# MisEty/RTG-SLAM

Hardware: AMD Instinct MI355X
Metric: hot_path_units_per_sec (higher is better)
Workload: dtype f32; 1 GPU; `value` counts UNITS, not SLAM frames (the SLAM frame rate by the reference's definition is `slam_frames_per_sec`, from the `slam_sequence` leg of --full).  One UNIT per step = 1 ICP track (3 levels x 5 GN iters, 1200x680, on a second HIP stream) + 1 map-optimisation iteration (raster fwd + masked L1 colour / gated depth loss + attach regulariser + raster bwd + fused Adam) over 1200000 random Gaus; gaussians=1200000, mode=single, parallelism=1 GPU

## Files before the change

include/rtgs_debug.h:

```cpp
#ifndef RTGS_DEBUG_H
#define RTGS_DEBUG_H
#include "rtgs_raster.h"
#ifdef __cplusplus
extern "C" {
#endif

void rtgs_raster_set_counters(void* counters);
void rtgs_raster_set_counters_ctx(rtgs_ctx* ctx, void* counters);

void rtgs_raster_set_profiling(int enable);
void rtgs_raster_set_profiling_ctx(rtgs_ctx* ctx, int enable);

void rtgs_raster_set_near_slice(int mode, int budget_per_tile);
void rtgs_raster_set_near_slice_ctx(rtgs_ctx* ctx, int mode, int budget_per_tile);

void rtgs_raster_force_sort_path(int enable);
void rtgs_raster_force_sort_path_ctx(rtgs_ctx* ctx, int enable);
int rtgs_raster_last_timings(float* ms12_host);
int rtgs_raster_last_timings_ctx(rtgs_ctx* ctx, float* ms12_host);

void rtgs_raster_set_bwd_walk_ctx(rtgs_ctx* ctx, int mode);
void rtgs_raster_set_onepass_ctx(rtgs_ctx* ctx, int on);
void rtgs_raster_set_fused_sort_ctx(rtgs_ctx* ctx, int on);
int rtgs_raster_fused_sort_stats_ctx(rtgs_ctx* ctx, int64_t* out18);
void rtgs_raster_set_tile_gather_ctx(rtgs_ctx* ctx, int mode);
int rtgs_raster_tile_gather_stats_ctx(rtgs_ctx* ctx, int64_t* out6);
void rtgs_raster_set_bwd_debug(int bits);
void rtgs_raster_set_bwd_stamps(void* dev);
void rtgs_raster_set_fwd_stamps(void* dev);
#define RTGS_ICP_STAMP_LAUNCHES 16
#define RTGS_ICP_STAMP_WGS 256
void rtgs_icp_set_stamps(void* dev);
void rtgs_tsdf_set_dense(int on);

#ifdef __cplusplus
}
#endif
#endif
```

rtg_slam_amd/csrc/map_ops.hip:

```cpp
#include "../../include/rtgs_raster.h"
#include <hip/hip_runtime.h>
#include <math.h>
#include <stdint.h>
#include "adam_common.h"
#include "activate_common.h"


namespace rtgs {

__global__ void __launch_bounds__(256) activate8_fwd_kernel(const float4* __restrict__ raw8, int64_t n,
                                                            float* __restrict__ opacity, float* __restrict__ scales,
                                                            float4* __restrict__ rots, float* __restrict__ normal) {
  for (int64_t i = (int64_t)blockIdx.x * blockDim.x + threadIdx.x; i < n; i += (int64_t)gridDim.x * blockDim.x)
    activate8_row_store(raw8[2 * i], raw8[2 * i + 1], i, opacity, scales, rots, normal);
}

__global__ void __launch_bounds__(256) activate8_bwd_kernel(const float4* __restrict__ raw8, int64_t n,
                                                            const float* __restrict__ g_op, const float* __restrict__ g_sc,
                                                            const float4* __restrict__ g_rot, const float* __restrict__ g_nrm,
                                                            const uint8_t* __restrict__ row_state,
                                                            float4* __restrict__ g_raw8) {
  for (int64_t i = (int64_t)blockIdx.x * blockDim.x + threadIdx.x; i < n; i += (int64_t)gridDim.x * blockDim.x) {
    if (row_state) {
      const uint8_t s = row_state[i];
      if (s == 0) continue;
      if (s == 2) { g_raw8[2 * i] = g_raw8[2 * i + 1] = make_float4(0.f, 0.f, 0.f, 0.f); continue; }
    }
    float4 lo, hi;
    activate8_bwd_row(raw8[2 * i], raw8[2 * i + 1], g_op[i], g_sc[i * 3], g_sc[i * 3 + 1], g_sc[i * 3 + 2], g_rot[i],
                      g_nrm[i * 3], g_nrm[i * 3 + 1], g_nrm[i * 3 + 2], lo, hi);
    g_raw8[2 * i] = lo;
    g_raw8[2 * i + 1] = hi;
  }
}

}

extern "C" int rtgs_map_activate8_forward(const float* raw8, int64_t n, float* opacity, float* scales, float* rotations,
                                          float* normal, void* stream) {
  if (n < 0 || (n > 0 && (!raw8 || !opacity || !scales || !rotations || !normal))) return -1;
  if (n == 0) return 0;
  int64_t blocks = (n + 255) / 256;
  if (blocks > 8192) blocks = 8192;
  hipLaunchKernelGGL(rtgs::activate8_fwd_kernel, dim3((unsigned)blocks), dim3(256), 0, (hipStream_t)stream,
                     (const float4*)raw8, n, opacity, scales, (float4*)rotations, normal);
  return hipGetLastError() == hipSuccess ? 0 : -2;
}

extern "C" int rtgs_map_activate8_backward(const float* raw8, int64_t n, const float* g_opacity, const float* g_scales,
                                           const float* g_rotations, const float* g_normal, float* g_raw8, void* stream) {
  if (n < 0 || (n > 0 && (!raw8 || !g_opacity || !g_scales || !g_rotations || !g_normal || !g_raw8))) return -1;
  if (n == 0) return 0;
  int64_t blocks = (n + 255) / 256;
  if (blocks > 8192) blocks = 8192;
  hipLaunchKernelGGL(rtgs::activate8_bwd_kernel, dim3((unsigned)blocks), dim3(256), 0, (hipStream_t)stream,
                     (const float4*)raw8, n, g_opacity, g_scales, (const float4*)g_rotations, g_normal,
                     (const uint8_t*)nullptr, (float4*)g_raw8);
  return hipGetLastError() == hipSuccess ? 0 : -2;
// ... 461 lines not shown
    const float4 t = *reinterpret_cast<const float4*>(p + i); v[0] = t.x; v[1] = t.y; v[2] = t.z; v[3] = t.w;
  }
  __device__ __forceinline__ void store(float* p, int64_t i) const { *reinterpret_cast<float4*>(p + i) = make_float4(v[0], v[1], v[2], v[3]); }
};
template <int V>
__device__ __forceinline__ void load_flags(const uint8_t* __restrict__ rmask, const int32_t* __restrict__ didx, int64_t i, bool (&m)[V],
                                           bool (&hit)[V]) {
  if constexpr (V == 4) {
    const uint32_t mm = rmask ? *reinterpret_cast<const uint32_t*>(rmask + i) : 0x01010101u;
    const int4 d = *reinterpret_cast<const int4*>(didx + i);
    m[0] = (mm & 0xffu) != 0; m[1] = (mm & 0xff00u) != 0; m[2] = (mm & 0xff0000u) != 0; m[3] = (mm & 0xff000000u) != 0;
    hit[0] = d.x != -1; hit[1] = d.y != -1; hit[2] = d.z != -1; hit[3] = d.w != -1;
  } else {
    m[0] = !rmask || rmask[i] != 0;
    hit[0] = didx[i] != -1;
  }
}

template <int V>
__global__ void __launch_bounds__(256) slam_loss_sums_kernel(const float* __restrict__ color, const float* __restrict__ depth,
                                                             const int32_t* __restrict__ didx, const float* __restrict__ gt_c,
                                                             const float* __restrict__ gt_d, const uint8_t* __restrict__ rmask,
                                                             int64_t hw, float depth_thr, float* __restrict__ sums) {
  float s_c = 0.f, s_d = 0.f, s_m = 0.f, s_n = 0.f;
  for (int64_t i = ((int64_t)blockIdx.x * blockDim.x + threadIdx.x) * V; i < hw; i += (int64_t)gridDim.x * blockDim.x * V) {
    bool m[V], hit[V];
    load_flags<V>(rmask, didx, i, m, hit);
    PixVec<V> c0, c1, c2, t0, t1, t2, dp, gd;
    c0.load(color, i); c1.load(color + hw, i); c2.load(color + 2 * hw, i);
    t0.load(gt_c, i); t1.load(gt_c + hw, i); t2.load(gt_c + 2 * hw, i);
    dp.load(depth, i); gd.load(gt_d, i);
#pragma unroll
    for (int k = 0; k < V; ++k) {
      if (!m[k]) continue;
      s_n += 1.f;
      s_c += fabsf(c0.v[k] - t0.v[k]) + fabsf(c1.v[k] - t1.v[k]) + fabsf(c2.v[k] - t2.v[k]);
      const float g = gd.v[k], e = dp.v[k] - g;
      if (hit[k] && g > 0.f && e < depth_thr) { s_d += fabsf(e); s_m += 1.f; }
    }
  }
  s_c = wave_sum_shfl(s_c); s_d = wave_sum_shfl(s_d); s_m = wave_sum_shfl(s_m); s_n = wave_sum_shfl(s_n);
  __shared__ float sh[4][4];
  const int lane = threadIdx.x & 63, w = threadIdx.x >> 6;
  if (lane == 0) { sh[0][w] = s_c; sh[1][w] = s_d; sh[2][w] = s_m; sh[3][w] = s_n; }
  __syncthreads();
  if (threadIdx.x < 4) {
    const float t = sh[threadIdx.x][0] + sh[threadIdx.x][1] + sh[threadIdx.x][2] + sh[threadIdx.x][3];
    unsafeAtomicAdd(&sums[threadIdx.x], t);
  }
}

__device__ __forceinline__ uint32_t sign_code(float d) { return d > 0.f ? 1u : (d < 0.f ? 2u : 0u); }

template <int V>
__global__ void __launch_bounds__(256) slam_loss_sums_signs_kernel(const float* __restrict__ color, const float* __restrict__ depth,
                                                                   const int32_t* __restrict__ didx, const float* __restrict__ gt_c,
                                                                   const float* __restrict__ gt_d, const uint8_t* __restrict__ rmask,
                                                                   int64_t hw, float depth_thr,
                                                                   float* __restrict__ sums, uint8_t* __restrict__ signs) {
  float s_c = 0.f, s_d = 0.f, s_m = 0.f, s_n = 0.f;
  for (int64_t i = ((int64_t)blockIdx.x * blockDim.x + threadIdx.x) * V; i < hw; i += (int64_t)gridDim.x * blockDim.x * V) {
    bool m[V], hit[V];
    load_flags<V>(rmask, didx, i, m, hit);
    PixVec<V> c0, c1, c2, t0, t1, t2, dp, gd;
    c0.load(color, i); c1.load(color + hw, i); c2.load(color + 2 * hw, i);
    t0.load(gt_c, i); t1.load(gt_c + hw, i); t2.load(gt_c + 2 * hw, i);
    dp.load(depth, i); gd.load(gt_d, i);
    uint32_t packed = 0u;
#pragma unroll
    for (int k = 0; k < V; ++k) {
      if (!m[k]) continue;
      const float d0 = c0.v[k] - t0.v[k], d1 = c1.v[k] - t1.v[k], d2 = c2.v[k] - t2.v[k];
      s_n += 1.f;
      s_c += fabsf(d0) + fabsf(d1) + fabsf(d2);
      uint32_t code = sign_code(d0) | (sign_code(d1) << 2) | (sign_code(d2) << 4);
      const float g = gd.v[k], e = dp.v[k] - g;
      if (hit[k] && g > 0.f && e < depth_thr) { s_d += fabsf(e); s_m += 1.f; code |= sign_code(e) << 6; }
      packed |= code << (8 * k);
    }
    if constexpr (V == 4) *reinterpret_cast<uint32_t*>(signs + i) = packed;
    else signs[i] = (uint8_t)packed;
  }
  s_c = wave_sum_shfl(s_c); s_d = wave_sum_shfl(s_d); s_m = wave_sum_shfl(s_m); s_n = wave_sum_shfl(s_n);
  __shared__ float sh[4][4];
  const int lane = threadIdx.x & 63, w = threadIdx.x >> 6;
  if (lane == 0) { sh[0][w] = s_c; sh[1][w] = s_d; sh[2][w] = s_m; sh[3][w] = s_n; }
  __syncthreads();
  if (threadIdx.x < 4) {
    const float t = sh[threadIdx.x][0] + sh[threadIdx.x][1] + sh[threadIdx.x][2] + sh[threadIdx.x][3];
    unsafeAtomicAdd(&sums[threadIdx.x], t);
  }
}

__global__ void slam_loss_values_kernel(const float* __restrict__ sums, float cw, float dw, float* __restrict__ loss4) {
  const float inv_c = 1.f / (3.f * fmaxf(sums[3], 1.f));
  const float inv_m = 1.f / fmaxf(sums[2], 1.f);
  const float lc = sums[0] * inv_c, ld = sums[1] * inv_m;
  loss4[1] = lc; loss4[2] = ld; loss4[3] = 0.f;
  loss4[0] = dw * ld + cw * lc;
}

struct SsimWin { float g[11]; };
constexpr int SS_R = 5, SS_T = 16 + 2 * SS_R;

__global__ void __launch_bounds__(256) ssim_fwd_kernel(const float* __restrict__ x1, const float* __restrict__ x2, int H, int W,
                                                       SsimWin win, float* __restrict__ dmaps, float* __restrict__ sums) {
  __shared__ float s_a[SS_T * SS_T], s_b[SS_T * SS_T];
  __shared__ float s_h[5][SS_T * 16];
  const int lx = threadIdx.x & 15, ly = threadIdx.x >> 4;
  const int px = blockIdx.x * 16 + lx, py = blockIdx.y * 16 + ly;
  const size_t HW = (size_t)H * W;
  float ssum = 0.f;
  for (int c = 0; c < 3; ++c) {
    __syncthreads();
// ... 133 lines not shown
}

}

extern "C" size_t rtgs_slam_loss_signs_offset(int32_t H, int32_t W, int32_t with_ssim) {
  const size_t front = 8 * sizeof(float) + (with_ssim ? (size_t)9 * (size_t)H * (size_t)W * sizeof(float) : 0);
  return (front + 15) & ~(size_t)15;
}
extern "C" size_t rtgs_slam_loss_scratch_bytes(int32_t H, int32_t W, int32_t with_ssim) {
  return rtgs_slam_loss_signs_offset(H, W, with_ssim) + (((size_t)H * (size_t)W + 15) & ~(size_t)15);
}

static void ssim_window(rtgs::SsimWin& win) {
  float gf[11], totf = 0.f;
  for (int i = 0; i < 11; ++i) { gf[i] = (float)exp(-(double)((i - 5) * (i - 5)) / (2.0 * 1.5 * 1.5)); totf += gf[i]; }
  for (int i = 0; i < 11; ++i) win.g[i] = gf[i] / totf;
}

extern "C" int rtgs_slam_loss_sums(const float* color, const float* depth, const int32_t* depth_index, const float* gt_color,
                                   const float* gt_depth, int32_t H, int32_t W, const rtgs_loss_cfg* cfg, void* scratch,
                                   void* stream) {
  if (!color || !depth || !depth_index || !gt_color || !gt_depth || !cfg || !scratch || H <= 0 || W <= 0) return -1;
  hipStream_t st = (hipStream_t)stream;
  const int64_t hw = (int64_t)H * W;
  float* sums = (float*)scratch;
  const bool ssim = cfg->render_mask == nullptr && cfg->ssim_weight != 0.f;
  if (!cfg->sums_zeroed && hipMemsetAsync(sums, 0, 8 * sizeof(float), st) != hipSuccess) return -2;
  int64_t blocks = (hw + 255) / 256;
  if (blocks > 192) blocks = 192;
  if (rtgs::loss_vec4_ok(hw, color, depth, depth_index, gt_color, gt_depth, cfg->render_mask, nullptr, nullptr))
    hipLaunchKernelGGL(rtgs::slam_loss_sums_kernel<4>, dim3((unsigned)blocks), dim3(256), 0, st, color, depth, depth_index,
                       gt_color, gt_depth, cfg->render_mask, hw, cfg->add_depth_thres, sums);
  else
    hipLaunchKernelGGL(rtgs::slam_loss_sums_kernel<1>, dim3((unsigned)blocks), dim3(256), 0, st, color, depth, depth_index,
                       gt_color, gt_depth, cfg->render_mask, hw, cfg->add_depth_thres, sums);
  if (ssim) {
    rtgs::SsimWin win;
    ssim_window(win);
    hipLaunchKernelGGL(rtgs::ssim_fwd_kernel, dim3((W + 15) / 16, (H + 15) / 16), dim3(256), 0, st, color, gt_color, H, W, win,
                       sums + 8, sums);
  }
  return hipGetLastError() == hipSuccess ? 0 : -2;
}

extern "C" int rtgs_slam_loss_values(const rtgs_loss_cfg* cfg, const void* scratch, float* loss_out4, void* stream) {
  if (!cfg || !scratch || !loss_out4 || (cfg->render_mask == nullptr && cfg->ssim_weight != 0.f)) return -1;
  hipLaunchKernelGGL(rtgs::slam_loss_values_kernel, dim3(1), dim3(1), 0, (hipStream_t)stream, (const float*)scratch,
                     cfg->color_weight, cfg->depth_weight, loss_out4);
  return hipGetLastError() == hipSuccess ? 0 : -2;
}
extern "C" int rtgs_slam_loss_sums_signs(const float* color, const float* depth, const int32_t* depth_index,
                                         const float* gt_color, const float* gt_depth, int32_t H, int32_t W,
                                         const rtgs_loss_cfg* cfg, void* scratch, float* loss_out4, void* stream) {
  if (!color || !depth || !depth_index || !gt_color || !gt_depth || !cfg || !scratch || H <= 0 || W <= 0) return -1;
  if (cfg->render_mask == nullptr && cfg->ssim_weight != 0.f) return -1;
  hipStream_t st = (hipStream_t)stream;
  const int64_t hw = (int64_t)H * W;
  float* sums = (float*)scratch;
  uint8_t* signs = (uint8_t*)scratch + rtgs_slam_loss_signs_offset(H, W, cfg->render_mask == nullptr);
  if (!cfg->sums_zeroed && hipMemsetAsync(sums, 0, 8 * sizeof(float), st) != hipSuccess) return -2;
  int64_t blocks = (hw + 255) / 256;
  if (blocks > 192) blocks = 192;
  if (rtgs::loss_vec4_ok(hw, color, depth, depth_index, gt_color, gt_depth, cfg->render_mask, nullptr, nullptr) &&
      ((uintptr_t)signs & 3u) == 0)
    hipLaunchKernelGGL(rtgs::slam_loss_sums_signs_kernel<4>, dim3((unsigned)blocks), dim3(256), 0, st, color, depth, depth_index,
                       gt_color, gt_depth, cfg->render_mask, hw, cfg->add_depth_thres, sums, signs);
  else
    hipLaunchKernelGGL(rtgs::slam_loss_sums_signs_kernel<1>, dim3((unsigned)blocks), dim3(256), 0, st, color, depth, depth_index,
                       gt_color, gt_depth, cfg->render_mask, hw, cfg->add_depth_thres, sums, signs);
  if (loss_out4) return rtgs_slam_loss_values(cfg, scratch, loss_out4, stream);
  return hipGetLastError() == hipSuccess ? 0 : -2;
}

extern "C" int rtgs_slam_loss_grads(const float* color, const float* depth, const int32_t* depth_index, const float* gt_color,
                                    const float* gt_depth, int32_t H, int32_t W, const rtgs_loss_cfg* cfg, void* scratch,
                                    float* loss_out4, float* g_color, float* g_depth, void* stream) {
  if (!color || !depth || !depth_index || !gt_color || !gt_depth || !cfg || !scratch || !loss_out4 || !g_color || !g_depth ||
      H <= 0 || W <= 0)
    return -1;
  hipStream_t st = (hipStream_t)stream;
  const int64_t hw = (int64_t)H * W;
  float* sums = (float*)scratch;
  const bool ssim = cfg->render_mask == nullptr && cfg->ssim_weight != 0.f;
  int64_t blocks = (hw + 255) / 256;
  if (blocks > 1024) blocks = 1024;
  if (rtgs::loss_vec4_ok(hw, color, depth, depth_index, gt_color, gt_depth, cfg->render_mask, g_color, g_depth)) {
    blocks = (hw / 4 + 255) / 256;
    if (blocks > 1024) blocks = 1024;
    hipLaunchKernelGGL(rtgs::slam_loss_grads_kernel<4>, dim3((unsigned)blocks), dim3(256), 0, st, color, depth, depth_index,
                       gt_color, gt_depth, cfg->render_mask, hw, cfg->color_weight, cfg->depth_weight,
                       ssim ? cfg->ssim_weight : 0.f, cfg->add_depth_thres, (const float*)sums, loss_out4, g_color, g_depth);
  } else {
    hipLaunchKernelGGL(rtgs::slam_loss_grads_kernel<1>, dim3((unsigned)blocks), dim3(256), 0, st, color, depth, depth_index,
                       gt_color, gt_depth, cfg->render_mask, hw, cfg->color_weight, cfg->depth_weight,
                       ssim ? cfg->ssim_weight : 0.f, cfg->add_depth_thres, (const float*)sums, loss_out4, g_color, g_depth);
  }
  if (ssim) {
    rtgs::SsimWin win;
    ssim_window(win);
    hipLaunchKernelGGL(rtgs::ssim_bwd_kernel, dim3((W + 15) / 16, (H + 15) / 16), dim3(256), 0, st, color, gt_color, H, W, win,
                       (const float*)(sums + 8), -cfg->ssim_weight / (3.f * (float)hw), g_color);
  }
  return hipGetLastError() == hipSuccess ? 0 : -2;
}

extern "C" int rtgs_slam_loss(const float* color, const float* depth, const int32_t* depth_index, const float* gt_color,
                              const float* gt_depth, int32_t H, int32_t W, const rtgs_loss_cfg* cfg, void* scratch,
                              float* loss_out4, float* g_color, float* g_depth, void* stream) {
  int rc = rtgs_slam_loss_sums(color, depth, depth_index, gt_color, gt_depth, H, W, cfg, scratch, stream);
  if (rc != 0) return rc;
  return rtgs_slam_loss_grads(color, depth, depth_index, gt_color, gt_depth, H, W, cfg, scratch, loss_out4, g_color, g_depth,
                              stream);
}


namespace rtgs {

__device__ __forceinline__ bool normal_pixel(const float* __restrict__ normal_w, const int32_t* __restrict__ didx,
                                             const float* __restrict__ gtn, const uint8_t* __restrict__ mask, int64_t i,
                                             int& owner, float (&n)[3], float (&g)[3]) {
  owner = didx[i];
  if (owner < 0 || (mask && mask[i] == 0)) return false;
// ... 104 lines not shown
```

rtg_slam_amd/csrc/map_step.hip:

```cpp
#include <hip/hip_runtime.h>

#include "../../include/rtgs_raster.h"

static int map_step_front(rtgs_ctx* ctx, const rtgs_map_step_args* a, int64_t* num_rendered_host, int32_t fwd_flags,
                          void* stream, bool walk_only = false) {
  if (!a || !num_rendered_host || !a->settings) return RTGS_E_INVALID;
  const int32_t P = a->P, M = a->sh_coeffs;
  if (P <= 0 || M != 16 || a->step < 1) return RTGS_E_INVALID;
  if (!a->xyz || !a->shs || !a->raw8 || !a->tile_mask || !a->gt_color || !a->gt_depth) return RTGS_E_INVALID;
  const int32_t H = a->settings->image_height, W = a->settings->image_width;
  int rc = 0;
  if (!a->activated_valid) {
    rc = rtgs_map_activate8_forward(a->raw8, P, a->opacity, a->scales, a->rotations, a->normal, stream);
    if (rc != 0) return RTGS_E_HIP;
  }
  if (!a->loss_scratch || !a->loss4) return RTGS_E_INVALID;
  rtgs_raster_set_aux_zero_ctx(ctx, a->loss_scratch);
  rc = rtgs_raster_forward_ctx(ctx, a->settings, P, M, a->xyz, a->opacity, a->shs, a->scales, a->rotations, a->normal,
                           a->tile_mask, a->out_color, a->out_depth, a->out_color_index, a->out_depth_index,
                           a->out_color_weight, a->out_depth_weight, a->out_T, a->out_radii, a->geom_resize,
                           a->geom_user, a->binning_resize, a->binning_user, a->image_resize, a->image_user,
                           num_rendered_host, fwd_flags, stream);
  if (rc != RTGS_OK) return rc;
  void* bufs[3];
  if (rtgs_raster_last_buffers_ctx(ctx, bufs) != RTGS_OK) return RTGS_E_ALLOC;
  void *geom = bufs[0], *bin = bufs[1], *img = bufs[2];
  rtgs_loss_cfg lcfg = a->loss;
  lcfg.sums_zeroed = P > 0 ? 1 : 0;
  const bool ssim_off = a->loss.render_mask != nullptr || a->loss.ssim_weight == 0.f;
  const bool signs = walk_only && ssim_off && rtgs_raster_signs_ok_ctx(ctx, geom) != 0;
  rtgs_raster_note_loss_path_ctx(ctx, signs ? 1 : 0);
  if (signs)
    rc = rtgs_slam_loss_sums_signs(a->out_color, a->out_depth, a->out_depth_index, a->gt_color, a->gt_depth, H, W, &lcfg,
                                   a->loss_scratch, nullptr, stream);
  else
    rc = rtgs_slam_loss(a->out_color, a->out_depth, a->out_depth_index, a->gt_color, a->gt_depth, H, W, &lcfg,
                        a->loss_scratch, a->loss4, a->dL_dcolor, a->dL_ddepth, stream);
  if (rc != 0) return RTGS_E_HIP;
  int32_t t0 = 0, t1 = P;
  if (a->train_begin != 0 || a->train_end != 0) { t0 = a->train_begin; t1 = a->train_end; }
  if (t0 < 0 || t1 > P || t1 < t0) return RTGS_E_INVALID;
  if (t1 == t0)
    return signs && rtgs_slam_loss_values(&lcfg, a->loss_scratch, a->loss4, stream) != 0 ? RTGS_E_HIP : RTGS_OK;
  if (signs) {
    const rtgs_loss_signs ls{reinterpret_cast<const uint8_t*>(a->loss_scratch) + rtgs_slam_loss_signs_offset(H, W, a->loss.render_mask == nullptr),
                             reinterpret_cast<const float*>(a->loss_scratch), a->loss.color_weight, a->loss.depth_weight, a->loss4};
    return rtgs_raster_backward_walk_signs_ctx(ctx, a->settings, P, M, *num_rendered_host, a->xyz, a->opacity, a->shs, a->scales,
                                               a->rotations, a->normal, geom, bin, img, a->out_color, a->out_T, a->out_depth_index,
                                               &ls, a->grad_scratch, a->row_state, t0, t1, stream);
  }
  rc = (walk_only ? rtgs_raster_backward_walk_ctx : rtgs_raster_backward_range_ctx)(
      ctx, a->settings, P, M, *num_rendered_host, a->xyz, a->opacity, a->shs, a->scales, a->rotations, a->normal, geom, bin, img,
      a->out_color, a->out_T, a->out_depth_index, a->dL_dcolor, a->dL_ddepth, a->d_xyz, a->d_opacity, a->d_shs, a->d_scales,
      a->d_rotations, a->d_normal, a->grad_scratch, a->row_state, t0, t1, stream);
  if (rc != RTGS_OK) return rc;
  if (a->normal_weight > 0.f && a->gt_normal) {
    rc = rtgs_slam_normal_loss_range(a->normal, a->out_depth_index, a->gt_normal, a->loss.render_mask, H, W, a->normal_weight,
                                     reinterpret_cast<float*>(a->loss_scratch) + 5, a->loss4, a->d_normal, a->row_state,
                                     rtgs_raster_spec_fail_ptr_ctx(ctx), t0, t1, stream);
    if (rc != 0) return RTGS_E_HIP;
  }
  return RTGS_OK;
}

extern "C" int rtgs_slam_map_step_front_ctx(rtgs_ctx* ctx, const rtgs_map_step_args* a, int64_t* num_rendered_host,
                                            void* stream) {
  return map_step_front(ctx, a, num_rendered_host, 0, stream);
}

extern "C" int rtgs_slam_map_step_front(const rtgs_map_step_args* a, int64_t* num_rendered_host, void* stream) {
  return rtgs_slam_map_step_front_ctx(nullptr, a, num_rendered_host, stream);
}

static int map_step_once(rtgs_ctx* ctx, const rtgs_map_step_args* a, int64_t* num_rendered_host, bool speculate, void* stream) {
  const bool fused = a->tail_mode == 0 && !(a->normal_weight > 0.f && a->gt_normal);
  rtgs_raster_set_map_epoch_ctx(ctx, speculate ? a->map_epoch : 0u);
  int rc = map_step_front(ctx, a, num_rendered_host, speculate ? RTGS_FWD_SPECULATE : 0, stream, fused);
  if (rc != RTGS_OK) return rc;
  if ((a->train_begin != 0 || a->train_end != 0) && a->train_end == a->train_begin) return RTGS_OK;
  if (fused) {
    void* bufs[3];
    if (rtgs_raster_last_buffers_ctx(ctx, bufs) != RTGS_OK) return RTGS_E_ALLOC;
    return rtgs_map_fused_tail_marked(a->settings, a, bufs[0], bufs[2], rtgs_raster_spec_fail_ptr_ctx(ctx), a->live_counts,
                                      rtgs_raster_last_listed_ctx(ctx), rtgs_raster_cull_marks_ctx(ctx), stream);
  }
  const int32_t P = a->P;
  int32_t t0 = 0, t1 = P;
  if (a->train_begin != 0 || a->train_end != 0) { t0 = a->train_begin; t1 = a->train_end; }
  const size_t o = (size_t)t0;
  const rtgs_activated act{a->opacity + o, a->scales + 3 * o, a->rotations + 4 * o, a->normal + 3 * o};
  uint8_t* const marks = rtgs_raster_cull_marks_ctx(ctx);
  rc = rtgs_map_tail_rows_marked(a->xyz + 3 * o, a->shs + 48 * o, a->raw8 + 8 * o, a->d_opacity + o, a->d_scales + 3 * o,
                          a->d_rotations + 4 * o, a->d_normal + 3 * o, a->d_xyz + 3 * o, a->d_shs + 48 * o, a->d_raw8 + 8 * o,
// ... 39 lines not shown
```

rtg_slam_amd/csrc/raster_api.hip:

```cpp
#include "../../include/rtgs_raster.h"
#include "../../include/rtgs_debug.h"
#include "raster_common.h"
#include "raster_launch.h"
#include <vector>

#include <rocprim/device/device_radix_sort.hpp>
#include <rocprim/device/device_scan.hpp>
#include <math.h>
#include <new>
#include <stdlib.h>
#include <string.h>

enum { EV_F0 = 0, EV_PRE, EV_SL_BIN, EV_SL_BLEND, EV_SCAN, EV_BIN0, EV_EMIT, EV_SORT, EV_RANGES, EV_BLEND0, EV_BLEND, EV_B0,
       EV_BWALK, EV_BBLEND, EV_BPRE, EV_N };
struct rtgs_ctx {
  int64_t stats[8] = {0};
  struct Switches {
    int slice_mode = 2;
    int slice_budget = 384;
    int bwd_walk = 0;
    bool onepass = true;
    bool fused_sort = true;
    bool speculation = true;
    bool plain_onepass = true;
    bool cull_cache = true, cull_check = false;
    bool loss_signs = true;
    int tile_gather = 1;
  } sw;
  int64_t gather_stats[4] = {0, 0, 0, 0};
  bool gather_blocked = false;
  int64_t loss_path_stats[2] = {0, 0};
  int64_t slice_stats[4] = {0};
  unsigned long long* counters = nullptr;
  uint32_t last_listed = 0;
  uint32_t* fsort_cls = nullptr;
  int32_t fsort_cap = 0, fsort_tiles = 0;
  bool prof = false;
  bool force_sort_path = false;
  bool ev_init = false;
  hipEvent_t ev[EV_N];
  bool ev_set[EV_N] = {false};
  uint32_t* info_host = nullptr;
  uint32_t seq = 0;
  const void* hint_geom = nullptr;
  bool hint_slice_lists = true, hint_main_lists = true;
  int hint_walk = -2;
  void *last_geom = nullptr, *last_bin = nullptr, *last_img = nullptr;
  uint32_t* aux_zero = nullptr;
  bool ask_first = false;
  struct Plan {
    bool valid = false;
    int32_t P = 0, H = 0, W = 0;
    int kind = -1;
    int slice_mode = 0, slice_budget = 0;
    uint32_t R = 0, R1 = 0, longest = 0, slots = 0, n_fin = 0;
    uint32_t R_hi = 0, longest_hi = 0, slots_hi = 0;
    uint32_t slice_longest_hi = 0;
    void note_slice(uint32_t l) { slice_longest_hi = l > slice_longest_hi - slice_longest_hi / 16 ? l : slice_longest_hi - slice_longest_hi / 16; }
    void note(uint32_t r, uint32_t l, uint32_t s) {
      R = r; longest = l; slots = s;
      R_hi = r > R_hi - R_hi / 16 ? r : R_hi - R_hi / 16;
      longest_hi = l > longest_hi - longest_hi / 16 ? l : longest_hi - longest_hi / 16;
      slots_hi = s > slots_hi - slots_hi / 16 ? s : slots_hi - slots_hi / 16;
    }
  } plan;
  struct Spec {
    bool pending = false;
    int kind = -1;
    bool gathered = false;
    uint32_t seq = 0, capR = 0, capL = 0, capS = 0;
    const void* geom = nullptr;
    const uint32_t* fail_dev = nullptr;
    void* stream = nullptr;
    int32_t ntiles = 0;
    int64_t G_total = 0, B_total = 0, I_total = 0;
  } spec;
  int64_t spec_stats[3] = {0, 0, 0};
  Plan plan_plain;
  Plan plan_plain0;
  int64_t plain_stats[2] = {0, 0};
  struct CullKey {
    const void *geom, *view, *means, *scales, *rots, *out_radii, *stream;
    uint64_t geom_bytes, epoch;
    int32_t P, H, W, kind, slice_mode, slice_budget;
    float fx, fy, cx, cy, tanfovx, tanfovy, scale_modifier, color_sigma;
  };
  struct CullCache {
    bool armed = false;
    CullKey key = {};
    uint8_t* marks = nullptr;
    uint64_t next_epoch = 0;
    int64_t stats[4] = {0, 0, 0, 0};
    char* scratch = nullptr;
    size_t scratch_bytes = 0;
    unsigned long long* mismatches = nullptr;
  } cull;
};

namespace rtgs {

static rtgs_ctx* default_ctx() {
  static rtgs_ctx* c = [] {
    rtgs_ctx* n = new rtgs_ctx();
    if (const char* e = getenv("RTGS_NEAR_SLICE")) n->sw.slice_mode = atoi(e);
    if (const char* e = getenv("RTGS_NEAR_SLICE_BUDGET")) { const int b = atoi(e); if (b > 0) n->sw.slice_budget = b; }
    if (const char* e = getenv("RTGS_SPECULATE")) n->sw.speculation = atoi(e) != 0;
    if (const char* e = getenv("RTGS_BIN_ONEPASS")) n->sw.onepass = atoi(e) != 0;
    if (const char* e = getenv("RTGS_FWD_SORT")) n->sw.fused_sort = atoi(e) != 0;
    if (const char* e = getenv("RTGS_PLAIN_ONEPASS")) n->sw.plain_onepass = atoi(e) != 0;
    if (const char* e = getenv("RTGS_BWD_WALK")) { const int m = atoi(e); n->sw.bwd_walk = (m >= 1 && m <= 4) ? m : 0; }
    if (const char* e = getenv("RTGS_CULL_CACHE")) n->sw.cull_cache = atoi(e) != 0;
    if (const char* e = getenv("RTGS_CULL_CACHE_CHECK")) n->sw.cull_check = atoi(e) != 0;
    if (const char* e = getenv("RTGS_LOSS_SIGNS")) n->sw.loss_signs = atoi(e) != 0;
    if (const char* e = getenv("RTGS_TILE_GATHER")) { const int m = atoi(e); n->sw.tile_gather = (m >= 0 && m <= 2) ? m : 1; }
    return n;
  }();
  return c;
}
static inline rtgs_ctx* use(rtgs_ctx* c) { return c ? c : default_ctx(); }

static void prof_mark(rtgs_ctx* c, int which, hipStream_t st) {
  if (!c->prof) return;
  if (!c->ev_init) {
    for (int i = 0; i < EV_N; ++i) (void)hipEventCreate(&c->ev[i]);
    c->ev_init = true;
  }
  (void)hipEventRecord(c->ev[which], st);
  c->ev_set[which] = true;
}

static int bits_for(uint32_t n) {
  int b = 0;
  while ((1ull << b) < (unsigned long long)n) ++b;
  return b < 1 ? 1 : b;
}

static int wait_published_words(uint32_t* info_host, uint32_t seq, hipStream_t st, uint32_t (&pub)[7]) {
  volatile uint32_t* h = info_host;
  auto snapshot_ok = [&]() -> bool {
    if (h[7] != seq) return false;
    __atomic_thread_fence(__ATOMIC_ACQUIRE);
    uint32_t w[7];
    for (int k = 0; k < 7; ++k) w[k] = h[k];
    if (h[8] != host_checksum(seq, w)) return false;
    for (int k = 0; k < 7; ++k) pub[k] = w[k];
    return true;
  };
  for (long spin = 0; spin < 4000000L; ++spin) {
    if (snapshot_ok()) return RTGS_OK;
    __builtin_ia32_pause();
  }
  if (hipStreamSynchronize(st) != hipSuccess) return RTGS_E_HIP;
  return snapshot_ok() ? RTGS_OK : RTGS_E_HIP;
}

static uint32_t sort_class_cap(uint32_t longest) {
  const uint64_t want = (uint64_t)longest + longest / 4 + 16;
  const uint32_t classes[5] = {256u, 1024u, 3072u, 8192u, 16384u};
  for (uint32_t c : classes) if (want <= c) return c;
  return 16384u;
}

__global__ void bwd_info_kernel(BwdInfo* dst, SplatGrad* slot_grads, uint32_t slots, uint32_t use_slots) {
  dst->slot_grads = slot_grads; dst->slots = slots; dst->use_slots = use_slots;
}

static int large_map_min() {
  static const int v = [] { const char* e = getenv("RTGS_LARGE_MAP_MIN"); const int x = e ? atoi(e) : 100000; return x > 0 ? x : 100000; }();
  return v;
}

static GeomLayout geom_layout(int32_t P, int gx, int gy, int budget) {
  GeomLayout L{};
  size_t off = 0;
  const size_t Pn = (size_t)(P > 0 ? P : 1);
  L.splats = off; off = align_up(off + Pn * sizeof(Splat));
  L.tiles_touched = off; off = align_up(off + Pn * sizeof(uint32_t));
  L.offsets = off; off = align_up(off + Pn * sizeof(uint32_t));
  L.radii = off; off = align_up(off + Pn * sizeof(int32_t));
  L.clamped = off; off = align_up(off + Pn);
  L.sat = off; off = align_up(off + (size_t)(gx + 1) * (gy + 1) * sizeof(int32_t));
  {
    const size_t nt = (size_t)gx * gy;
    L.zero_begin = L.tile_count = off;
    off += nt * sizeof(uint32_t);
    L.tile_count1 = off; off += nt * sizeof(uint32_t);
    L.ranges1_bwd = off; off += nt * sizeof(uint2);
    L.slice_ctr = off; off += 8 * sizeof(uint32_t);
    L.slot_count = off; off += Pn * sizeof(uint32_t);
    L.zero_end = off; off = align_up(off);
    L.cursor = off; off = align_up(off + nt * sizeof(uint32_t));
    L.info = off; off = align_up(off + 4 * sizeof(uint32_t));
    L.block_counts = off; off = align_up(off + bin_block_counts_bytes((int)Pn, gx * gy));
    L.zbin = off; off = align_up(off + Pn);
    L.cursor1 = off; off = align_up(off + nt * sizeof(uint32_t));
    L.ranges1 = off; off = align_up(off + nt * sizeof(uint2));
    L.mask2 = off; off = align_up(off + nt * sizeof(int32_t));
    L.uv = off; off = align_up(off + Pn * sizeof(float2));
    L.slice_hist = off; off += 2 * SLICE_BINS * sizeof(uint32_t);
    L.slice_cover = off; off = align_up(off + SLICE_BINS * sizeof(unsigned long long));
    L.cull_marks = off; off = align_up(off + Pn + 16);
    L.cull_view = off; off = align_up(off + 16 * sizeof(float));
    L.slice_cap = nt * (size_t)(budget > 0 ? budget : 1);
    L.slice_max_list = L.slice_cap < 65536 ? L.slice_cap : 65536;
// ... 71 lines not shown
  p.cy = s->cy > 0.f ? s->cy : 0.5f * (float)(p.H - 1);
  p.scale_modifier = s->scale_modifier;
  p.opaque_thr = s->opaque_threshold; p.depth_thr = s->depth_threshold; p.normal_thr = s->normal_threshold;
  p.color_sigma = s->color_sigma; p.T_thr = s->T_threshold;
  p.view = s->viewmatrix; p.campos = s->campos; p.bg = s->bg;
  p.spec_fail = nullptr;
  return RTGS_OK;
}

#define HIP_TRY(expr)                         \
  do {                                        \
    hipError_t e_ = (expr);                   \
    if (e_ != hipSuccess) return RTGS_E_HIP;  \
  } while (0)

static int dbg_sync(const rtgs_raster_settings* s, hipStream_t st) {
  if (s->debug) {
    HIP_TRY(hipStreamSynchronize(st));
    HIP_TRY(hipGetLastError());
  }
  return RTGS_OK;
}
#define DBG(s, st)                              \
  do {                                          \
    int r_ = dbg_sync(s, st);                   \
    if (r_ != RTGS_OK) return r_;               \
  } while (0)

struct FwdCall {
  rtgs_ctx* c;
  const rtgs_raster_settings* s;
  RasterParams p;
  hipStream_t st;
  int32_t flags;
  bool want_bwd, slice_auto;
  const float *means3D, *opacities, *shs, *scales, *rotations, *normal_w;
  const int32_t* tile_mask;
  float *out_color, *out_depth, *out_cw, *out_dw, *out_T;
  int32_t *out_cidx, *out_didx, *out_radii;
  rtgs_resize_fn geom_resize, binning_resize, image_resize;
  void *geom_user, *binning_user, *image_user;
  int64_t* num_rendered_host;
  GeomLayout G;
  ImgLayout I;
  char *geom, *img;
  uint32_t *tiles_touched, *offsets, *tile_count, *cursor, *info, *zero_words, *tile_count1, *slice_hist, *slice_ctr, *list1;
  Splat* splats; int32_t *radii, *sat, *mask2; uint8_t *clamped, *zbin; uint16_t* block_counts;
  uint2 *ranges, *ranges1, *ranges1_bwd; unsigned long long* slice_cover; float2* uv;
  uint32_t *n_contrib, *depth_pos, *tile_last, *tile_mode;
  int zero_n, ntiles;
  int fwd_walk;
  TileCache tcache;
  uint32_t seg1;
  uint32_t* aux_zero;
  uint64_t cull_epoch;
  bool cull_was_armed;
  uint32_t* info_host;
  uint32_t pub[7];
};

static inline void next_seq(rtgs_ctx* c) { if (++c->seq == 0u) c->seq = 1u; }
static inline int wait_published(FwdCall& f) { return wait_published_words(f.info_host, f.c->seq, f.st, f.pub); }

static void record_stats(rtgs_ctx* c, int64_t rendered, int ntiles, int64_t geom_bytes, int64_t bin_bytes, int64_t img_bytes,
                         bool tile_path, int64_t longest) {
  c->stats[0] = rendered; c->stats[1] = 32 + bits_for((uint32_t)ntiles); c->stats[2] = ntiles;
  c->stats[3] = geom_bytes; c->stats[4] = bin_bytes; c->stats[5] = img_bytes;
  c->stats[6] = tile_path ? 1 : 0; c->stats[7] = longest;
}

static void note_plan(rtgs_ctx::Plan& pl, const FwdCall& f, bool same, int kind, bool usable, int64_t R, uint32_t longest,
                      uint32_t slots) {
  same = same && pl.valid && pl.H == f.p.H && pl.W == f.p.W;
  pl.kind = kind;
  pl.valid = kind >= 0 && usable && R <= 0xffffffffll;
  pl.P = f.p.P; pl.H = f.p.H; pl.W = f.p.W; pl.slice_mode = f.c->sw.slice_mode; pl.slice_budget = f.c->sw.slice_budget;
  if (!same || !pl.valid) { pl.R_hi = pl.longest_hi = pl.slots_hi = 0; pl.slice_longest_hi = 0; }
  pl.note((uint32_t)R, longest, slots);
}

static SliceSel slice_sel(const FwdCall& f) {
  return SliceSel{1, f.zbin, f.slice_hist, (uint32_t)f.G.slice_cap, (uint32_t)f.G.slice_max_list, f.slice_ctr, nullptr, nullptr,
                  f.slice_cover, (uint32_t)f.ntiles * (uint32_t)(TILE * TILE), f.slice_auto ? 1 : 0};
}

static void preprocess_all(const FwdCall& f, const int32_t* sat, bool clear) {
  launch_preprocess_fwd(f.p, f.means3D, f.opacities, f.shs, f.scales, f.rotations, f.normal_w, sat, f.splats, f.tiles_touched,
                        f.radii, f.clamped, f.out_radii, clear ? f.zero_words : nullptr, clear ? f.zero_n : 0, nullptr, f.st);
}
static void shade(const FwdCall& f, const RasterParams& p, SliceList work, const SliceSel& sel, size_t max_list,
                  RowBands rb = RowBands{nullptr, nullptr, 0u}) {
  launch_preprocess_shade(p, f.means3D, f.opacities, f.shs, f.scales, f.rotations, f.normal_w, f.splats, f.radii, f.clamped,
                          f.uv, work, sel, max_list, f.st, rb);
}
static void blend(const FwdCall& f, const RasterParams& p, const uint2* ranges, const uint32_t* list, SlicePass pass,
                  uint32_t seg, FusedSort fs = FusedSort{nullptr, nullptr, nullptr, nullptr, nullptr},
                  TileGather tg = TileGather{nullptr, nullptr, 0u, nullptr, nullptr, nullptr}) {
  launch_blend_fwd(p, ranges, list, f.splats, f.out_color, f.out_depth, f.out_cidx, f.out_didx, f.out_cw, f.out_dw, f.out_T,
                   f.n_contrib, f.c->counters, pass, f.tile_mode, f.depth_pos, f.tile_last, f.fwd_walk, f.aux_zero, f.tcache,
                   seg, f.st, fs, tg);
}

static bool tile_gather_chosen(FwdCall& f, const rtgs_ctx::Plan& pl) {
  rtgs_ctx* const c = f.c; const GeomLayout& G = f.G;
  if (c->sw.tile_gather == 0 || !f.seg1 || !(c->sw.fused_sort && blend_fwd_fuses_sort() && blend_fwd_gathers())) return false;
  const size_t cap1 = (size_t)f.ntiles * G.slice_seg > G.slice_cap ? (size_t)f.ntiles * G.slice_seg : G.slice_cap;
  if (f.p.gx > 255 || f.p.gy > GATHER_ROWS_MAX || G.slice_max_list > 65536 ||
      (size_t)f.p.gy * G.slice_max_list * sizeof(uint32_t) > cap1 * sizeof(uint64_t)) { ++c->gather_stats[3]; return false; }
  const bool forced = c->sw.tile_gather == 2;
  if (c->gather_blocked && pl.slice_longest_hi <= (uint32_t)FSORT_CAP) c->gather_blocked = false;
  if (c->gather_blocked) { ++c->gather_stats[2]; return false; }
  if (!forced && c->last_listed > (uint32_t)G.slice_max_list) { ++c->gather_stats[1]; return false; }
  if (!forced && pl.slice_longest_hi > (uint32_t)(FSORT_CAP - FSORT_CAP / 8)) { ++c->gather_stats[2]; return false; }
  ++c->gather_stats[0];
  return true;
}

static int scan_slots(const FwdCall& f) {
  size_t tb = f.G.scan_temp_bytes;
  HIP_TRY(rocprim::exclusive_scan(f.geom + f.G.scan_temp, tb, f.tiles_touched, f.offsets, 0u, (size_t)f.p.P,
                                  rocprim::plus<uint32_t>(), f.st));
  return RTGS_OK;
}

static int fsort_class_words(FwdCall& f, uint32_t*& cls) {
  rtgs_ctx* const c = f.c;
  cls = nullptr;
  if (c->counters) {
    if (c->fsort_cap < f.ntiles) {
      if (c->fsort_cls) (void)hipFree(c->fsort_cls);
      c->fsort_cls = nullptr; c->fsort_cap = 0;
      HIP_TRY(hipMalloc((void**)&c->fsort_cls, (size_t)f.ntiles * sizeof(uint32_t)));
      c->fsort_cap = f.ntiles;
    }
    HIP_TRY(hipMemsetAsync(c->fsort_cls, 0xff, (size_t)f.ntiles * sizeof(uint32_t), f.st));
    c->fsort_tiles = f.ntiles;
    cls = c->fsort_cls;
  }
  return RTGS_OK;
}
static int sort_slice_lists(FwdCall& f, FusedSort& fs1) {
  rtgs_ctx* const c = f.c;
  const unsigned long long* bucket1 = (const unsigned long long*)(f.geom + f.G.bucket1);
  const uint32_t* cnt = f.seg1 ? f.tile_count1 : nullptr;
  if (!(c->sw.fused_sort && blend_fwd_fuses_sort())) {
    launch_bin_tilesort(f.ntiles, (uint32_t)SLICE_MAX_LIST, f.ranges1, bucket1, f.list1, nullptr, f.st, cnt, f.seg1,
                        f.seg1 ? f.ranges1 : nullptr);
    return RTGS_OK;
  }
  launch_bin_tilesort_long(f.ntiles, f.ranges1, bucket1, f.list1, nullptr, f.st, cnt, f.seg1);
  uint32_t* cls = nullptr;
  const int rc = fsort_class_words(f, cls);
  if (rc != RTGS_OK) return rc;
  fs1 = FusedSort{bucket1, cnt, f.seg1 ? f.ranges1 : nullptr, f.list1, cls};
  return RTGS_OK;
}

static int slice_pass1(FwdCall& f, uint32_t* guard, bool gather = false) {
  const RasterParams& p = f.p; const GeomLayout& G = f.G;
  const SliceSel sel1 = slice_sel(f);
  const SliceList work{(const uint32_t*)(f.geom + G.slice_ids), f.slice_ctr + 2};
  unsigned long long* const bucket1 = (unsigned long long*)(f.geom + G.bucket1);
  if (gather) {
    const RowBands rb{f.tile_count, (uint32_t*)bucket1, (uint32_t)G.slice_max_list};
    shade(f, p, work, sel1, G.slice_max_list, rb);
    uint32_t* cls = nullptr;
    const int rcc = fsort_class_words(f, cls);
    if (rcc != RTGS_OK) return rcc;
    DBG(f.s, f.st);
    prof_mark(f.c, EV_SL_BIN, f.st);
    blend(f, p, f.ranges1, f.list1, SlicePass{1, f.tile_mask, f.mask2, f.ranges1_bwd, f.ranges}, f.seg1,
          FusedSort{bucket1, f.tile_count1, f.ranges1, f.list1, cls},
          TileGather{rb.count, rb.entries, rb.stride, work.ids, f.radii, f.tile_count1});
    prof_mark(f.c, EV_SL_BLEND, f.st);
    launch_slice_publish(f.ntiles, f.tile_mask, f.mask2, f.info + 2, f.slice_ctr, f.info_host, f.c->seq, guard, f.st, f.tile_count1);
    DBG(f.s, f.st);
    return RTGS_OK;
  }
  shade(f, p, work, sel1, G.slice_max_list);
  if (f.seg1) {
    launch_bin_place(p, f.splats, f.radii, f.tile_mask, f.tile_count1, bucket1, f.seg1, nullptr, sel1, work, G.slice_max_list, f.st);
  } else {
    uint16_t* const block_counts1 = (uint16_t*)(f.geom + G.block_counts1);
    uint32_t* const cursor1 = (uint32_t*)(f.geom + G.cursor1);
    if (launch_bin_count(p, f.splats, f.radii, f.tile_mask, f.tile_count1, block_counts1, sel1, work, G.slice_max_list, f.st) != 0)
      return RTGS_E_HIP;
    launch_bin_tilescan(f.ntiles, f.tile_count1, f.ranges1, cursor1, f.info + 2, nullptr, nullptr, nullptr, nullptr, nullptr, 0u,
                        SpecCaps{nullptr, 0u, 0u, 0u, nullptr}, f.st);
    launch_bin_scatter(p, f.splats, f.radii, f.tile_mask, block_counts1, cursor1, bucket1, sel1, work, G.slice_max_list, f.st);
  }
  FusedSort fs1{nullptr, nullptr, nullptr, nullptr, nullptr};
  const int rc = sort_slice_lists(f, fs1);
  if (rc != RTGS_OK) return rc;
  DBG(f.s, f.st);
  prof_mark(f.c, EV_SL_BIN, f.st);
  blend(f, p, f.ranges1, f.list1, SlicePass{1, f.tile_mask, f.mask2, f.ranges1_bwd, f.ranges}, f.seg1, fs1);
  prof_mark(f.c, EV_SL_BLEND, f.st);
  launch_slice_publish(f.ntiles, f.tile_mask, f.mask2, f.info + 2, f.slice_ctr, f.info_host, f.c->seq, guard, f.st,
                       f.seg1 ? f.tile_count1 : nullptr);
  DBG(f.s, f.st);
  return RTGS_OK;
}

static int cull_self_check(FwdCall& f, uint32_t* fail) {
  rtgs_ctx::CullCache& cc = f.c->cull;
  const int32_t P = f.p.P; const size_t Pn = (size_t)P;
  const size_t o_tt = 0, o_rad = align_up(o_tt + Pn * 4), o_orad = align_up(o_rad + Pn * 4), o_zb = align_up(o_orad + Pn * 4),
               o_uv = align_up(o_zb + Pn), o_hist = align_up(o_uv + Pn * 8), need = align_up(o_hist + CULL_HIST_WORDS * 4);
  if (cc.scratch_bytes < need) {
    if (cc.scratch) (void)hipFree(cc.scratch);
    cc.scratch = nullptr; cc.scratch_bytes = 0;
    HIP_TRY(hipMalloc((void**)&cc.scratch, need));
    cc.scratch_bytes = need;
  }
  if (!cc.mismatches) {
    HIP_TRY(hipMalloc((void**)&cc.mismatches, sizeof(unsigned long long)));
    HIP_TRY(hipMemset(cc.mismatches, 0, sizeof(unsigned long long)));
  }
  char* sc = cc.scratch;
  HIP_TRY(hipMemcpyAsync(sc + o_uv, f.uv, Pn * 8, hipMemcpyDeviceToDevice, f.st));
  launch_preprocess_cull(f.p, f.means3D, f.scales, f.rotations, (uint32_t*)(sc + o_tt), (int32_t*)(sc + o_rad),
                         f.out_radii ? (int32_t*)(sc + o_orad) : nullptr, nullptr, 0, (uint8_t*)(sc + o_zb),
                         (float2*)(sc + o_uv), (uint32_t*)(sc + o_hist), f.st);
  launch_slice_hist(P, (const uint8_t*)(sc + o_zb), (const uint32_t*)(sc + o_tt), (const int32_t*)(sc + o_rad),
                    (uint32_t*)(sc + o_hist), (unsigned long long*)(sc + o_hist + 2 * SLICE_BINS * 4), f.st);
  launch_cull_check(P, f.tiles_touched, (const uint32_t*)(sc + o_tt), f.radii, (const int32_t*)(sc + o_rad), f.out_radii,
                    (const int32_t*)(sc + o_orad), f.zbin, (const uint8_t*)(sc + o_zb), f.uv, (const float2*)(sc + o_uv),
                    f.slice_hist, (const uint32_t*)(sc + o_hist), fail + 1, cc.mismatches, f.st);
  return RTGS_OK;
}

static int cull_stage(FwdCall& f, int kind, bool usable, uint32_t* fail, const BwdInfoInit& bi) {
  rtgs_ctx* const c = f.c; const RasterParams& p = f.p;
  rtgs_ctx::CullCache& cc = c->cull;
  rtgs_ctx::CullKey key;
  memset(&key, 0, sizeof(key));
  key.geom = f.geom; key.view = f.s->viewmatrix; key.means = f.means3D; key.scales = f.scales; key.rots = f.rotations;
  key.out_radii = f.out_radii; key.stream = (void*)f.st; key.geom_bytes = (uint64_t)f.G.total; key.epoch = f.cull_epoch;
  key.P = p.P; key.H = p.H; key.W = p.W; key.kind = kind; key.slice_mode = c->sw.slice_mode; key.slice_budget = c->sw.slice_budget;
  key.fx = p.fx; key.fy = p.fy; key.cx = p.cx; key.cy = p.cy; key.tanfovx = p.tanfovx; key.tanfovy = p.tanfovy;
  key.scale_modifier = p.scale_modifier; key.color_sigma = p.color_sigma;
  usable = usable && c->sw.cull_cache && f.cull_epoch != 0;
  uint8_t* const marks = (uint8_t*)(f.geom + f.G.cull_marks);
  float* const view_copy = (float*)(f.geom + f.G.cull_view);
  if (usable && f.cull_was_armed && memcmp(&key, &cc.key, sizeof(key)) == 0) {
    launch_recull_rows(p, f.means3D, f.scales, f.rotations, f.tiles_touched, f.radii, f.out_radii, f.zero_words, f.zero_n, f.zbin,
                       f.uv, f.slice_hist, f.slice_cover, marks, view_copy, (int)(fail - f.zero_words), bi, f.st);
    cc.armed = true;
    ++cc.stats[0]; --cc.stats[2];
    return c->sw.cull_check ? cull_self_check(f, fail) : RTGS_OK;
  }
  launch_preprocess_cull(p, f.means3D, f.scales, f.rotations, f.tiles_touched, f.radii, f.out_radii, f.zero_words, f.zero_n,
// ... 37 lines not shown
  f.tcache = f.want_bwd ? TileCache{(float4*)(img + I.tile_recs), (uint16_t*)(img + I.tile_masks), (float2*)(img + I.depth_aux)}
                        : TileCache{nullptr, nullptr, nullptr};
  f.fwd_walk = c->sw.bwd_walk == 0 || c->sw.bwd_walk == 3 ? 2 : (c->sw.bwd_walk == 4 ? -1 : c->sw.bwd_walk - 1);
  f.seg1 = c->sw.onepass ? (uint32_t)G.slice_seg : 0u;
  f.slice_auto = c->sw.slice_mode == 2;
  if (!c->info_host) {
    HIP_TRY(hipHostMalloc((void**)&c->info_host, HOST_WORDS * sizeof(uint32_t), hipHostMallocCoherent));
    memset(c->info_host, 0, HOST_WORDS * sizeof(uint32_t));
  }
  f.info_host = c->info_host;
  for (uint32_t& w : f.pub) w = 0;
  return RTGS_OK;
}

enum SpecOutcome { SPEC_RETURNED, SPEC_NOT_ELIGIBLE, SPEC_REDO };

static int forward_speculative(FwdCall& f, bool sort_path, bool sliced, SpecOutcome& outcome) {
  rtgs_ctx* const c = f.c;
  const RasterParams& p = f.p; const GeomLayout& G = f.G; const ImgLayout& I = f.I;
  const int32_t P = p.P; const int ntiles = f.ntiles; hipStream_t st = f.st;
  int rc;
  outcome = SPEC_RETURNED;
  rtgs_ctx::Plan& pp = sliced ? c->plan_plain : c->plan_plain0;
  const bool immediate = !(f.flags & RTGS_FWD_SPECULATE) && !f.want_bwd && c->sw.speculation && c->sw.plain_onepass && c->sw.onepass &&
                         P > 0 && !sort_path && !f.s->debug && pp.valid && (sliced ? (pp.kind == 2 && G.slice_seg) : pp.kind == 0) &&
                         pp.H == p.H && pp.W == p.W && pp.slice_mode == c->sw.slice_mode && pp.slice_budget == c->sw.slice_budget;
  const rtgs_ctx::Plan& pl = immediate ? pp : c->plan;
  const bool eligible = immediate ||
                        ((f.flags & RTGS_FWD_SPECULATE) && c->sw.speculation && f.want_bwd && P > 0 && !sort_path && !f.s->debug &&
                         pl.valid && pl.P == P && pl.H == p.H && pl.W == p.W && pl.slice_mode == c->sw.slice_mode &&
                         pl.slice_budget == c->sw.slice_budget && (pl.kind == 0 ? !sliced : (pl.kind == 1 || pl.kind == 2) && sliced));
  const uint32_t capR = pl.R_hi + pl.R_hi / 8u + 8192u, capL = sort_class_cap(pl.longest_hi),
                 capS = immediate ? 0u : pl.slots_hi + pl.slots_hi / 8u + 8192u;
  if (!(eligible && (pl.kind == 1 || capS <= SLOTS_MAX))) {
    if (f.flags & RTGS_FWD_SPECULATE) ++c->spec_stats[2];
    outcome = SPEC_NOT_ELIGIBLE;
    return RTGS_OK;
  }
  uint32_t* const fail = f.slice_ctr + 6;
  next_seq(c);
  const uint32_t sl = (uint32_t)G.slice_cap <= SLOTS_MAX ? (uint32_t)G.slice_cap : 0u;
  const uint32_t seg2 = (pl.kind != 1 && c->sw.onepass && ((pl.kind == 2 && G.slice_seg) || (immediate && pl.kind == 0))) ? capL : 0u;
  const bool seg_main = seg2 != 0u;
  const BinLayout B = pl.kind == 1 ? bin_layout(0, ntiles, false, (size_t)sl)
                                   : bin_layout(seg2 ? (int64_t)ntiles * (int64_t)seg2 : (int64_t)capR, ntiles, false, (size_t)capS);
  char* bin = (char*)f.binning_resize(f.binning_user, B.total);
  if (!bin) return RTGS_E_ALLOC;
  c->last_bin = bin;
  BwdInfo* const bwd_info = (BwdInfo*)(f.img + I.bwd_info);
  SplatGrad* const slot_grads = (SplatGrad*)(bin + B.slot_grads);
  if (pl.kind == 1) {
    if ((rc = cull_stage(f, pl.kind, !immediate, fail, BwdInfoInit{bwd_info, slot_grads, sl, sl ? 1u : 0u})) != RTGS_OK) return rc;
    prof_mark(c, EV_PRE, st);
    launch_slice_compact(P, slice_sel(f), (uint32_t*)(f.geom + G.slice_ids), f.slice_ctr + 2, f.tiles_touched, f.offsets,
                         f.slice_ctr + 4, nullptr, 0u, nullptr, st);
    c->spec.gathered = tile_gather_chosen(f, pl);
    if ((rc = slice_pass1(f, fail, c->spec.gathered)) != RTGS_OK) return rc;
    prof_mark(c, EV_BLEND0, st); prof_mark(c, EV_BLEND, st);
    c->hint_slice_lists = true; c->hint_main_lists = false;
    c->slice_stats[0] = 1; c->slice_stats[1] = pl.R1; c->slice_stats[2] = pl.n_fin; c->slice_stats[3] = 0;
  } else {
    unsigned long long* const keys_a = (unsigned long long*)(bin + B.keys_a);
    uint32_t* const vals_b = (uint32_t*)(bin + B.vals_b);
    RasterParams pg = p;
    pg.spec_fail = fail;
    SliceList vl{nullptr, nullptr};
    if (pl.kind == 2) {
      if ((rc = cull_stage(f, pl.kind, !immediate, fail, BwdInfoInit{bwd_info, slot_grads, capS, immediate ? 0u : 1u})) != RTGS_OK)
        return rc;
      prof_mark(c, EV_PRE, st);
      const SliceSel sel1 = slice_sel(f);
      vl = SliceList{(const uint32_t*)(f.geom + G.vis_ids), f.slice_ctr + 4};
      launch_visible_compact(P, f.zbin, (uint32_t*)(f.geom + G.vis_ids), f.slice_ctr + 4, f.tiles_touched, f.offsets, f.slice_ctr + 5,
                             fail, st, &sel1, (int32_t*)(f.slice_ctr + 3), fail);
      shade(f, pg, vl, sel1, (size_t)P);
    } else {
      preprocess_all(f, nullptr, true);
      if (!immediate && (rc = scan_slots(f)) != RTGS_OK) return rc;
      prof_mark(c, EV_PRE, st);
    }
    const SliceSel sel2{0, nullptr, nullptr, 0u, 0u, f.slice_ctr, nullptr, f.uv, nullptr, 0u, 0};
    const int32_t* const still_declined = pl.kind == 2 ? (const int32_t*)(f.slice_ctr + 3) : nullptr;
    if (seg2) {
      if (pl.kind != 2)
        hipLaunchKernelGGL(bwd_info_kernel, dim3(1), dim3(1), 0, st, bwd_info, slot_grads, capS, immediate ? 0u : 1u);
      launch_bin_place(pg, f.splats, f.radii, f.tile_mask, f.tile_count, keys_a, seg2, fail, sel2, vl, (size_t)P, st);
      prof_mark(c, EV_SCAN, st); prof_mark(c, EV_BIN0, st); prof_mark(c, EV_EMIT, st);
      const BinFinish fin{f.tile_count, ntiles, f.info, f.info_host, f.slice_ctr + 5, nullptr, f.slice_ctr + 4, c->seq,
                          SpecCaps{fail, 0xffffffffu, capL, immediate ? 0xffffffffu : capS, still_declined}};
      launch_bin_tilesort(ntiles, capL, f.ranges, keys_a, vals_b, fail, st, f.tile_count, seg2, f.ranges, &fin);
    } else {
      uint16_t* const counts = vl.ids ? (uint16_t*)(f.geom + G.block_counts_vis) : f.block_counts;
      if (launch_bin_count(pg, f.splats, f.radii, f.tile_mask, f.tile_count, counts, sel2, vl, (size_t)P, st) != 0)
        return RTGS_E_HIP;
      const SpecCaps caps{fail, capR, capL, immediate ? 0xffffffffu : capS, still_declined};
      launch_bin_tilescan(ntiles, f.tile_count, f.ranges, f.cursor, f.info, f.info_host, nullptr, nullptr,
                          vl.ids ? f.slice_ctr + 5 : f.offsets + (P - 1), vl.ids ? nullptr : f.tiles_touched + (P - 1), c->seq,
                          caps, st);
      prof_mark(c, EV_SCAN, st);
      if (pl.kind != 2) hipLaunchKernelGGL(bwd_info_kernel, dim3(1), dim3(1), 0, st, bwd_info, slot_grads, capS, 1u);
      prof_mark(c, EV_BIN0, st);
      launch_bin_scatter(pg, f.splats, f.radii, f.tile_mask, counts, f.cursor, keys_a, sel2, vl, (size_t)P, st);
      prof_mark(c, EV_EMIT, st);
      launch_bin_tilesort(ntiles, capL, f.ranges, keys_a, vals_b, fail, st);
    }
    prof_mark(c, EV_SORT, st);
    prof_mark(c, EV_BLEND0, st);
    blend(f, pg, f.ranges, vals_b, SlicePass{0, nullptr, nullptr, nullptr, nullptr}, seg2);
    prof_mark(c, EV_BLEND, st);
    c->hint_slice_lists = false; c->hint_main_lists = true;
// ... 200 lines not shown

const char* rtgs_version(void) { return "rtgs-hip 0.2.0 (gfx950)"; }

rtgs_ctx* rtgs_ctx_create(void) {
  rtgs_ctx* c = new (std::nothrow) rtgs_ctx();
  if (c) c->sw = default_ctx()->sw;
  return c;
}
void rtgs_ctx_destroy(rtgs_ctx* c) {
  if (!c || c == default_ctx()) return;
  if (c->ev_init) for (int i = 0; i < EV_N; ++i) (void)hipEventDestroy(c->ev[i]);
  if (c->info_host) (void)hipHostFree(c->info_host);
  if (c->cull.scratch) (void)hipFree(c->cull.scratch);
  if (c->cull.mismatches) (void)hipFree(c->cull.mismatches);
  if (c->fsort_cls) (void)hipFree(c->fsort_cls);
  delete c;
}

size_t rtgs_raster_geom_bytes_ctx(rtgs_ctx* c, int32_t P, int32_t H, int32_t W) {
  return geom_layout(P, (W + TILE - 1) / TILE, (H + TILE - 1) / TILE, use(c)->sw.slice_budget).total;
}
size_t rtgs_raster_geom_bytes(int32_t P, int32_t H, int32_t W) { return rtgs_raster_geom_bytes_ctx(nullptr, P, H, W); }
size_t rtgs_raster_binning_bytes(int64_t R, int32_t H, int32_t W) {
  const int gx = (W + TILE - 1) / TILE, gy = (H + TILE - 1) / TILE;
  return bin_layout(R, gx * gy, true, 0).total;
}
size_t rtgs_raster_image_bytes(int32_t H, int32_t W) {
  const int gx = (W + TILE - 1) / TILE, gy = (H + TILE - 1) / TILE;
  return img_layout(H, W, gx * gy).total;
}
size_t rtgs_raster_backward_scratch_bytes(int32_t P) {
  const size_t n = (size_t)(P > 0 ? P : 1);
  return align_up(n * sizeof(SplatGrad)) + align_up(n);
}

int rtgs_raster_last_stats_ctx(rtgs_ctx* c, int64_t* out) {
  if (!out) return RTGS_E_INVALID;
  memcpy(out, use(c)->stats, sizeof(use(c)->stats));
  return RTGS_OK;
}
void rtgs_raster_set_counters_ctx(rtgs_ctx* c, void* counters) { use(c)->counters = (unsigned long long*)counters; }

int rtgs_raster_forward_ctx(rtgs_ctx* ctx, const rtgs_raster_settings* s, int32_t P, int32_t M, const float* means3D,
                            const float* opacities, const float* shs, const float* scales, const float* rotations,
                            const float* normal_w, const int32_t* tile_mask, float* out_color, float* out_depth,
                            int32_t* out_cidx, int32_t* out_didx, float* out_cw, float* out_dw, float* out_T,
                            int32_t* out_radii, rtgs_resize_fn geom_resize, void* geom_user,
                            rtgs_resize_fn binning_resize, void* binning_user, rtgs_resize_fn image_resize,
                            void* image_user, int64_t* num_rendered_host, int32_t flags, void* stream) {
  rtgs_ctx* c = use(ctx);
  FwdCall f;
  f.c = c;
  f.aux_zero = c->aux_zero; c->aux_zero = nullptr;
  f.cull_epoch = c->cull.next_epoch; c->cull.next_epoch = 0;
  f.cull_was_armed = c->cull.armed; c->cull.armed = false;
  if (f.cull_was_armed) ++c->cull.stats[2];
  int rc = make_params(s, P, M, f.p);
  if (rc != RTGS_OK) return rc;
  if (P > 0 && (!means3D || !opacities || !shs || !scales || !rotations || !normal_w)) return RTGS_E_INVALID;
  if (!tile_mask || !out_color || !out_depth || !out_cidx || !out_didx || !out_cw || !out_dw || !out_T)
    return RTGS_E_INVALID;
  if (!geom_resize || !binning_resize || !image_resize || !num_rendered_host) return RTGS_E_INVALID;
  f.s = s; f.st = (hipStream_t)stream; f.flags = flags; f.want_bwd = !(flags & RTGS_FWD_NO_BACKWARD);
  f.means3D = means3D; f.opacities = opacities; f.shs = shs; f.scales = scales; f.rotations = rotations; f.normal_w = normal_w;
  f.tile_mask = tile_mask;
  f.out_color = out_color; f.out_depth = out_depth; f.out_cidx = out_cidx; f.out_didx = out_didx; f.out_cw = out_cw;
  f.out_dw = out_dw; f.out_T = out_T; f.out_radii = out_radii;
  f.geom_resize = geom_resize; f.geom_user = geom_user; f.binning_resize = binning_resize; f.binning_user = binning_user;
  f.image_resize = image_resize; f.image_user = image_user; f.num_rendered_host = num_rendered_host;
  if ((rc = forward_setup(f)) != RTGS_OK) return rc;
  if (c->spec.pending) return RTGS_E_INVALID;
  c->spec.geom = nullptr; c->spec.fail_dev = nullptr;
  const bool sort_path = (size_t)f.ntiles > bin_lds_limit_tiles() || c->force_sort_path;
  const bool sliced = !sort_path && P > 0 && (c->sw.slice_mode == 1 || (f.slice_auto && P >= large_map_min() && f.ntiles >= 256));
  SpecOutcome outcome;
  rc = forward_speculative(f, sort_path, sliced, outcome);
  if (outcome == SPEC_RETURNED) return rc;
  return forward_classic(f, sort_path, sliced);
}

static int backward_impl(rtgs_ctx* ctx, const rtgs_raster_settings* s, int32_t P, int32_t M, int64_t R, const float* means3D,
                         const float* opacities, const float* shs, const float* scales, const float* rotations,
                         const float* normal_w, void* geom_buffer, void* binning_buffer,
                         const void* image_buffer, const float* out_color, const float* out_T,
                         const int32_t* out_didx,
                         const float* dL_dcolor, const float* dL_ddepth, float* dL_dmeans3D, float* dL_dopacities,
                         float* dL_dshs, float* dL_dscales, float* dL_drotations, float* dL_dnormal_w,
                         void* grad_scratch, uint8_t* row_state, int32_t train_begin, int32_t train_end, void* stream,
                         bool walk_only = false, const rtgs_loss_signs* lsg = nullptr) {
  rtgs_ctx* c = use(ctx);
  RasterParams p;
  int rc = make_params(s, P, M, p);
  if (rc != RTGS_OK) return rc;
  if (P == 0) return RTGS_OK;
  if (c->spec.geom == geom_buffer && c->spec.fail_dev) p.spec_fail = c->spec.fail_dev;
  if (!means3D || !opacities || !shs || !scales || !rotations || !normal_w || !geom_buffer || !binning_buffer ||
      !image_buffer || !out_color || !out_T || !out_didx || (!lsg && (!dL_dcolor || !dL_ddepth)) || !grad_scratch || R < 0)
    return RTGS_E_INVALID;
  if (lsg && (!walk_only || !lsg->signs || !lsg->sums || c->hint_geom != geom_buffer || c->hint_walk != 2)) return RTGS_E_INVALID;
  const LossSigns lsd = lsg ? LossSigns{lsg->signs, lsg->sums, lsg->color_weight, lsg->depth_weight, lsg->loss_out4}
                            : LossSigns{nullptr, nullptr, 0.f, 0.f, nullptr};
  int entry_launches = 0;
  if (!walk_only && (!dL_dmeans3D || !dL_dopacities || !dL_dshs || !dL_dscales || !dL_drotations || !dL_dnormal_w)) return RTGS_E_INVALID;
  hipStream_t st = (hipStream_t)stream;
  const int ntiles = p.gx * p.gy;
  const GeomLayout G = geom_layout(P, p.gx, p.gy, 1);
  const BinLayout B = bin_layout(R, ntiles, false, 0);
  const ImgLayout I = img_layout(p.H, p.W, ntiles);
  const char* geom = (const char*)geom_buffer;
  const char* bin = (const char*)binning_buffer;
  const char* img = (const char*)image_buffer;
  SplatGrad* grads = (SplatGrad*)grad_scratch;
  for (int i = EV_B0; i < EV_N; ++i) c->ev_set[i] = false;
  prof_mark(c, EV_B0, st);
  uint8_t* touched = (uint8_t*)grad_scratch + align_up((size_t)P * sizeof(SplatGrad));
  if (!row_state) HIP_TRY(hipMemsetAsync(grads, 0, rtgs_raster_backward_scratch_bytes(P), st));
  const BwdInfo* binfo = (const BwdInfo*)(img + I.bwd_info);
  const uint32_t* gbase = (const uint32_t*)(geom + G.offsets);
  const int32_t* radii = (const int32_t*)(geom + G.radii);
  uint32_t* slot_count = (uint32_t*)(geom + G.slot_count);
  const uint32_t* tile_mode = (const uint32_t*)(img + I.tile_mode);
  if (R > 0) {
    const bool hinted = c->hint_geom == geom_buffer;
    const int which = !hinted ? 7 : (c->hint_walk == 2 ? 4 : (c->hint_walk == -1 ? 3 : (c->hint_walk == 0 ? 1 : 2)));
    if (train_begin < 0 || train_end > P || train_end < train_begin) return RTGS_E_INVALID;
    const uint32_t t0 = (uint32_t)train_begin, tn = (uint32_t)(train_end - train_begin);
    const uint32_t* depth_pos = (const uint32_t*)(img + I.depth_pos);
    for (int set = 0; set < 2; ++set) {
      if (hinted && !(set == 0 ? c->hint_slice_lists : c->hint_main_lists)) continue;
      const uint2* rg = set == 0 ? (const uint2*)(geom + G.ranges1_bwd) : (const uint2*)(img + I.ranges);
      const uint32_t* pl = set == 0 ? (const uint32_t*)(geom + G.list1) : (const uint32_t*)(bin + B.vals_b);
      if (which & 3)
        launch_blend_bwd(p, rg, pl, (const Splat*)(geom + G.splats), out_color, out_T, (const uint32_t*)(img + I.n_contrib),
                         out_didx, dL_dcolor, dL_ddepth, gbase, slot_count, binfo, grads, touched, tile_mode, which & 3, t0, tn, st);
      if (which & 4) ++entry_launches;
      if (which & 4)
        launch_blend_bwd_entry(p, rg, pl, (const Splat*)(geom + G.splats), out_color, (const uint32_t*)(img + I.n_contrib),
                               out_didx, depth_pos, (const uint32_t*)(img + I.tile_last), dL_dcolor, dL_ddepth, gbase, slot_count, binfo, grads,
                               touched, tile_mode, t0, tn,
                               TileCache{(float4*)(img + I.tile_recs), (uint16_t*)(img + I.tile_masks), (float2*)(img + I.depth_aux)},
                               set == 0 ? (uint32_t)(BLOCK / 4) : (uint32_t)BLOCK,
                               st, lsg ? &lsd : nullptr);
    }
    prof_mark(c, EV_BWALK, st);
    if (!walk_only) launch_grad_reduce(P, touched, gbase, slot_count, binfo, grads, p.spec_fail, st);
    DBG(s, st);
  }
// ... 51 lines not shown
                       image_buffer, out_color, out_T, out_didx, dL_dcolor, dL_ddepth, dL_dmeans3D, dL_dopacities,
                       dL_dshs, dL_dscales, dL_drotations, dL_dnormal_w, grad_scratch, row_state, train_begin, train_end, stream);
}

int rtgs_raster_backward_walk_ctx(rtgs_ctx* ctx, const rtgs_raster_settings* s, int32_t P, int32_t M, int64_t R,
                                   const float* means3D, const float* opacities, const float* shs, const float* scales,
                                   const float* rotations, const float* normal_w, void* geom_buffer,
                                   void* binning_buffer, const void* image_buffer, const float* out_color,
                                   const float* out_T, const int32_t* out_didx, const float* dL_dcolor,
                                   const float* dL_ddepth, float* dL_dmeans3D, float* dL_dopacities, float* dL_dshs,
                                   float* dL_dscales, float* dL_drotations, float* dL_dnormal_w, void* grad_scratch,
                                   uint8_t* row_state, int32_t train_begin, int32_t train_end, void* stream) {
  return backward_impl(ctx, s, P, M, R, means3D, opacities, shs, scales, rotations, normal_w, geom_buffer, binning_buffer,
                       image_buffer, out_color, out_T, out_didx, dL_dcolor, dL_ddepth, dL_dmeans3D, dL_dopacities,
                       dL_dshs, dL_dscales, dL_drotations, dL_dnormal_w, grad_scratch, row_state, train_begin, train_end, stream, true);
}

int rtgs_raster_backward_walk_signs_ctx(rtgs_ctx* ctx, const rtgs_raster_settings* s, int32_t P, int32_t M, int64_t R,
                                        const float* means3D, const float* opacities, const float* shs, const float* scales,
                                        const float* rotations, const float* normal_w, void* geom_buffer, void* binning_buffer,
                                        const void* image_buffer, const float* out_color, const float* out_T,
                                        const int32_t* out_didx, const rtgs_loss_signs* loss, void* grad_scratch,
                                        uint8_t* row_state, int32_t train_begin, int32_t train_end, void* stream) {
  if (!loss || (P > 0 && !row_state)) return RTGS_E_INVALID;
  return backward_impl(ctx, s, P, M, R, means3D, opacities, shs, scales, rotations, normal_w, geom_buffer, binning_buffer,
                       image_buffer, out_color, out_T, out_didx, nullptr, nullptr, nullptr, nullptr, nullptr, nullptr, nullptr,
                       nullptr, grad_scratch, row_state, train_begin, train_end, stream, true, loss);
}
int rtgs_raster_signs_ok_ctx(rtgs_ctx* ctx, const void* geom_buffer) {
  rtgs_ctx* c = use(ctx);
  return c->sw.loss_signs && geom_buffer && c->hint_geom == geom_buffer && c->hint_walk == 2 ? 1 : 0;
}
void rtgs_raster_set_loss_signs_ctx(rtgs_ctx* ctx, int enable) { use(ctx)->sw.loss_signs = enable != 0; }
int rtgs_raster_loss_signs_stats_ctx(rtgs_ctx* ctx, int64_t* out2) {
  if (!out2) return RTGS_E_INVALID;
  memcpy(out2, use(ctx)->loss_path_stats, sizeof(use(ctx)->loss_path_stats));
  return RTGS_OK;
}
void rtgs_raster_note_loss_path_ctx(rtgs_ctx* ctx, int signs) { ++use(ctx)->loss_path_stats[signs ? 0 : 1]; }

void rtgs_raster_set_profiling_ctx(rtgs_ctx* c, int enable) { use(c)->prof = enable != 0; }
void rtgs_raster_set_near_slice_ctx(rtgs_ctx* c, int mode, int budget_per_tile) {
  use(c)->sw.slice_mode = mode;
  if (budget_per_tile > 0) use(c)->sw.slice_budget = budget_per_tile;
}
int rtgs_raster_last_slice_stats_ctx(rtgs_ctx* c, int64_t* out) {
  if (!out) return RTGS_E_INVALID;
  memcpy(out, use(c)->slice_stats, sizeof(use(c)->slice_stats));
  return RTGS_OK;
}
void rtgs_raster_force_sort_path_ctx(rtgs_ctx* c, int enable) { use(c)->force_sort_path = enable != 0; }
int rtgs_raster_forward_verify_ctx(rtgs_ctx* ctx, int64_t* num_rendered_host) {
  rtgs_ctx* c = use(ctx);
  if (!c->spec.pending) return 0;
  c->spec.pending = false;
  uint32_t pub[7] = {0, 0, 0, 0, 0, 0, 0};
  const int rc = wait_published_words(c->info_host, c->spec.seq, (hipStream_t)c->spec.stream, pub);
  if (rc != RTGS_OK) { c->plan.valid = false; return rc; }
  rtgs_ctx::Plan& pl = c->plan;
  bool ok;
  if (c->spec.kind == 1) {
    const uint32_t n_left = pub[2];
    ok = n_left == 0u && pub[5] == 0u;
    if (pub[5] != 0u) ++c->cull.stats[3];
    pl.R1 = pub[4]; pl.n_fin = pub[3]; pl.R = 0; pl.longest = 0;
    pl.note_slice(pub[1]);
    if (c->spec.gathered && pub[1] > (uint32_t)FSORT_CAP) c->gather_blocked = true;
    c->last_listed = pub[0];
    c->slice_stats[1] = pub[4]; c->slice_stats[2] = pub[3]; c->slice_stats[3] = n_left;
  } else {
    ok = pub[0] <= c->spec.capR && pub[1] <= c->spec.capL && pub[5] <= c->spec.capS && (c->spec.kind != 2 || (int32_t)pub[6] < 0) &&
         pub[4] == 0u;
    if (pub[4] != 0u) ++c->cull.stats[3];
    pl.note(pub[0], pub[1], pub[5]); pl.R1 = 0;
    c->last_listed = pub[2];
  }
  record_stats(c, (int64_t)pl.R + (int64_t)pl.R1, c->spec.ntiles, c->spec.G_total, c->spec.B_total, c->spec.I_total, true,
               (int64_t)pl.longest);
  if (num_rendered_host) *num_rendered_host = c->stats[0] > 0 ? c->stats[0] : 1;
  if (!ok) { pl.valid = false; ++c->spec_stats[1]; }
  return ok ? 0 : 1;
}
const uint32_t* rtgs_raster_spec_fail_ptr_ctx(rtgs_ctx* ctx) {
  rtgs_ctx* c = use(ctx);
  return c->spec.pending ? c->spec.fail_dev : nullptr;
}
void rtgs_raster_set_speculation_ctx(rtgs_ctx* ctx, int enable) {
  rtgs_ctx* c = use(ctx);
  c->sw.speculation = enable != 0;
  c->plan = rtgs_ctx::Plan();
}
int rtgs_raster_speculation_stats_ctx(rtgs_ctx* ctx, int64_t* out3) {
  if (!out3) return RTGS_E_INVALID;
  memcpy(out3, use(ctx)->spec_stats, sizeof(use(ctx)->spec_stats));
  return RTGS_OK;
}
int rtgs_raster_plain_stats_ctx(rtgs_ctx* ctx, int64_t* out2) {
  if (!out2) return RTGS_E_INVALID;
  memcpy(out2, use(ctx)->plain_stats, sizeof(use(ctx)->plain_stats));
  return RTGS_OK;
}
void rtgs_raster_set_plain_onepass_ctx(rtgs_ctx* ctx, int enable) {
  rtgs_ctx* c = use(ctx);
  c->sw.plain_onepass = enable != 0;
  c->plan_plain = rtgs_ctx::Plan();
  c->plan_plain0 = rtgs_ctx::Plan();
}
uint32_t rtgs_raster_last_listed_ctx(rtgs_ctx* c) { return use(c)->last_listed; }
void rtgs_raster_set_cull_cache_ctx(rtgs_ctx* ctx, int enable) {
  rtgs_ctx* c = use(ctx);
  c->sw.cull_cache = enable != 0;
  c->cull.armed = false;
}
void rtgs_raster_set_cull_cache_check_ctx(rtgs_ctx* ctx, int enable) { use(ctx)->sw.cull_check = enable != 0; }
void rtgs_raster_set_map_epoch_ctx(rtgs_ctx* ctx, uint64_t epoch) { use(ctx)->cull.next_epoch = epoch; }
uint8_t* rtgs_raster_cull_marks_ctx(rtgs_ctx* ctx) {
  rtgs_ctx* c = use(ctx);
  return c->cull.armed ? c->cull.marks : nullptr;
}
int rtgs_raster_cull_cache_stats_ctx(rtgs_ctx* ctx, int64_t* out5) {
  rtgs_ctx* c = use(ctx);
  if (!out5) return RTGS_E_INVALID;
  memcpy(out5, c->cull.stats, sizeof(c->cull.stats));
  unsigned long long bad = 0;
  if (c->cull.mismatches) HIP_TRY(hipMemcpy(&bad, c->cull.mismatches, sizeof(bad), hipMemcpyDeviceToHost));
  out5[4] = (int64_t)bad;
  return RTGS_OK;
}
void rtgs_raster_set_bwd_debug(int bits) { rtgs::set_bwd_debug(bits); }
void rtgs_raster_set_bwd_stamps(void* dev) { rtgs::set_bwd_stamps(dev); }
void rtgs_raster_set_fwd_stamps(void* dev) { rtgs::set_fwd_stamps(dev); }
void rtgs_raster_set_onepass_ctx(rtgs_ctx* c, int on) { use(c)->sw.onepass = on != 0; use(c)->plan.valid = false; }
void rtgs_raster_set_fused_sort_ctx(rtgs_ctx* c, int on) { use(c)->sw.fused_sort = on != 0; use(c)->plan.valid = false; }
int rtgs_raster_fused_sort_stats_ctx(rtgs_ctx* ctx, int64_t* out18) {
  rtgs_ctx* c = use(ctx);
  if (!out18) return RTGS_E_INVALID;
  for (int k = 0; k < 3 * FSORT_CLASSES; ++k) out18[k] = 0;
  if (!c->fsort_cls || c->fsort_tiles <= 0) return RTGS_OK;
  std::vector<uint32_t> w((size_t)c->fsort_tiles);
  HIP_TRY(hipMemcpy(w.data(), c->fsort_cls, w.size() * sizeof(uint32_t), hipMemcpyDeviceToHost));
  for (uint32_t v : w) {
    if (v == 0xffffffffu) continue;
    const int cls = (int)(v >> 28);
    const int64_t len = (int64_t)(v & 0x0fffffffu);
    if (cls >= FSORT_CLASSES) continue;
    int64_t* o = out18 + 3 * cls;
    o[1] = o[0] == 0 ? len : (len < o[1] ? len : o[1]);
    o[2] = len > o[2] ? len : o[2];
    ++o[0];
  }
  return RTGS_OK;
}
void rtgs_raster_set_tile_gather_ctx(rtgs_ctx* c, int mode) {
  use(c)->sw.tile_gather = (mode >= 0 && mode <= 2) ? mode : 1; use(c)->plan.valid = false; use(c)->gather_blocked = false;
}
int rtgs_raster_tile_gather_stats_ctx(rtgs_ctx* ctx, int64_t* out6) {
  if (!out6) return RTGS_E_INVALID;
  memcpy(out6, use(ctx)->gather_stats, sizeof(use(ctx)->gather_stats));
  out6[4] = GATHER_CHUNK; out6[5] = GATHER_CAND;
  return RTGS_OK;
}
void rtgs_raster_set_bwd_walk_ctx(rtgs_ctx* c, int mode) { use(c)->sw.bwd_walk = (mode >= 1 && mode <= 4) ? mode : 0; }
void rtgs_raster_set_aux_zero_ctx(rtgs_ctx* ctx, void* eight_words) { use(ctx)->aux_zero = (uint32_t*)eight_words; }
int rtgs_raster_last_buffers_ctx(rtgs_ctx* ctx, void** out3) {
  rtgs_ctx* c = use(ctx);
  if (!out3 || !c->last_geom || !c->last_bin || !c->last_img) return RTGS_E_INVALID;
  out3[0] = c->last_geom; out3[1] = c->last_bin; out3[2] = c->last_img;
  return RTGS_OK;
}
int rtgs_raster_backward_buffers(int32_t P, int32_t H, int32_t W, size_t* out) {
  if (!out || P < 0 || H <= 0 || W <= 0) return RTGS_E_INVALID;
  const int gx = (W + TILE - 1) / TILE, gy = (H + TILE - 1) / TILE;
  const GeomLayout G = geom_layout(P, gx, gy, 1);
  const ImgLayout I = img_layout(H, W, gx * gy);
  out[0] = G.clamped; out[1] = G.offsets; out[2] = G.slot_count; out[3] = I.bwd_info;
  out[4] = align_up((size_t)(P > 0 ? P : 1) * sizeof(SplatGrad)); out[5] = G.radii; out[6] = G.cull_marks; out[7] = 0;
  return RTGS_OK;
}
int rtgs_raster_image_offsets(int32_t H, int32_t W, size_t* out) {
  if (!out || H <= 0 || W <= 0) return RTGS_E_INVALID;
  const int gx = (W + TILE - 1) / TILE, gy = (H + TILE - 1) / TILE;
  const ImgLayout I = img_layout(H, W, gx * gy);
  out[0] = I.ranges; out[1] = I.n_contrib; out[2] = I.bwd_info; out[3] = I.tile_mode; out[4] = I.total; out[5] = I.depth_pos;
  return RTGS_OK;
}

int rtgs_raster_last_timings_ctx(rtgs_ctx* ctx, float* ms) {
  rtgs_ctx* c = use(ctx);
  if (!ms) return RTGS_E_INVALID;
  for (int i = 0; i < 12; ++i) ms[i] = -1.f;
  if (!c->ev_init) return RTGS_OK;
  const int pre_end = c->ev_set[EV_SL_BLEND] ? EV_SL_BLEND : EV_PRE;
  const int pairs[11][2] = {{EV_F0, EV_PRE}, {pre_end, EV_SCAN}, {EV_BIN0, EV_EMIT}, {EV_EMIT, EV_SORT},
                            {EV_SORT, EV_RANGES}, {EV_BLEND0, EV_BLEND}, {EV_B0, EV_BWALK}, {EV_BBLEND, EV_BPRE},
                            {EV_PRE, EV_SL_BIN}, {EV_SL_BIN, EV_SL_BLEND}, {EV_BWALK, EV_BBLEND}};
  for (int i = 0; i < 11; ++i) {
    const int a = pairs[i][0], b = pairs[i][1];
    if (!c->ev_set[a] || !c->ev_set[b]) continue;
    if (hipEventSynchronize(c->ev[b]) != hipSuccess) return RTGS_E_HIP;
    float t = 0.f;
    if (hipEventElapsedTime(&t, c->ev[a], c->ev[b]) == hipSuccess) ms[i] = t;
  }
  return RTGS_OK;
}

int rtgs_raster_forward(const rtgs_raster_settings* s, int32_t P, int32_t M, const float* means3D,
                        const float* opacities, const float* shs, const float* scales, const float* rotations,
                        const float* normal_w, const int32_t* tile_mask, float* out_color, float* out_depth,
// ... 42 lines not shown
```

rtg_slam_amd/csrc/raster_common.h:

```cpp
#pragma once
#include <hip/hip_runtime.h>
#include <stdint.h>
#include <stddef.h>

namespace rtgs {

constexpr int TILE = 16;
constexpr int BLOCK = TILE * TILE;
constexpr int WAVE = 64;
#ifndef RTGS_BWD_BATCH
#define RTGS_BWD_BATCH 128
#endif
constexpr int BATCH = RTGS_BWD_BATCH;

struct __attribute__((aligned(16))) Splat {
  float u, v;
  float ca, cb, cc;
  float o;
  float r, g, b;
  float nx, ny, nz;
  float pd;
  float z;
  float hx, hy;
};
// ... 256 lines not shown

#define RTGS_SH_C0 0.28209479177387814f
#define RTGS_SH_C1 0.4886025119029199f
#define RTGS_SH_C2_0 1.0925484305920792f
#define RTGS_SH_C2_1 -1.0925484305920792f
#define RTGS_SH_C2_2 0.31539156525252005f
#define RTGS_SH_C2_3 -1.0925484305920792f
#define RTGS_SH_C2_4 0.5462742152960396f
#define RTGS_SH_C3_0 -0.5900435899266435f
#define RTGS_SH_C3_1 2.890611442640554f
#define RTGS_SH_C3_2 -0.4570457994644658f
#define RTGS_SH_C3_3 0.3731763325901154f
#define RTGS_SH_C3_4 -0.4570457994644658f
#define RTGS_SH_C3_5 1.445305721320277f
#define RTGS_SH_C3_6 -0.5900435899266435f

__device__ __forceinline__ uint32_t wave_max_u32(uint32_t x) {
  const auto r = __builtin_amdgcn_permlane32_swap(x, x, false, false);
  x = max(r[0], r[1]);
  const auto q = __builtin_amdgcn_permlane16_swap(x, x, false, false);
  x = max(q[0], q[1]);
  x = max(x, (uint32_t)__builtin_amdgcn_update_dpp(0, (int)x, 0x128, 0xf, 0xf, false));
  x = max(x, (uint32_t)__builtin_amdgcn_update_dpp(0, (int)x, 0x124, 0xf, 0xf, false));
  x = max(x, (uint32_t)__builtin_amdgcn_update_dpp(0, (int)x, 0x122, 0xf, 0xf, false));
  x = max(x, (uint32_t)__builtin_amdgcn_update_dpp(0, (int)x, 0x121, 0xf, 0xf, false));
  return x;
}

__device__ __forceinline__ float splat_power(float ca, float cb, float cc, float dx, float dy) {
  float q = __fmaf_rn(ca * dx, dx, (cc * dy) * dy);
  return __fmaf_rn(-0.5f, q, -(cb * dx) * dy);
}

__device__ __forceinline__ float splat_exp(float x) {
  return __builtin_amdgcn_exp2f(__fmul_rn(x, 1.4426950408889634f));
}

constexpr int HOST_WORDS = 16;
__host__ __device__ __forceinline__ uint32_t host_checksum(uint32_t seq, const uint32_t (&w)[7]) {
  uint32_t h = seq * 2654435761u;
#pragma unroll
  for (int k = 0; k < 7; ++k) h = (h ^ w[k]) * 16777619u;
  return h;
}
__device__ __forceinline__ void publish_to_host(uint32_t* host, const uint32_t (&w)[7], uint32_t seq) {
#pragma unroll
  for (int k = 0; k < 7; ++k) host[k] = w[k];
  host[8] = host_checksum(seq, w);
  __builtin_amdgcn_fence(__ATOMIC_RELEASE, "");
  asm volatile("s_waitcnt vmcnt(0)" ::: "memory");
  __hip_atomic_store(&host[7], seq, __ATOMIC_RELAXED, __HIP_MEMORY_SCOPE_SYSTEM);
}

__device__ __forceinline__ int slice_cut(const SliceSel& sel) {
  __shared__ uint32_t s_wsum[2][BLOCK / 64];
  const int tid = threadIdx.x, lane = tid & 63, w = tid >> 6;
  uint32_t incl = sel.hist[tid], incl_n = sel.hist[SLICE_BINS + tid];
#pragma unroll
  for (int off = 1; off < 64; off <<= 1) {
    const uint32_t o = (uint32_t)__shfl_up((int)incl, off), on = (uint32_t)__shfl_up((int)incl_n, off);
    if (lane >= off) { incl += o; incl_n += on; }
  }
  if (lane == 63) { s_wsum[0][w] = incl; s_wsum[1][w] = incl_n; }
  __syncthreads();
  unsigned long long cum = incl, cum_n = incl_n;
  for (int k = 0; k < w; ++k) { cum += s_wsum[0][k]; cum_n += s_wsum[1][k]; }
  const int n_ok = __syncthreads_count(cum <= (unsigned long long)sel.cap && cum_n <= (unsigned long long)sel.max_list);
  const int cut = n_ok - 1;
  if (!sel.decide || cut < 0) return cut;
  __shared__ float s_dec[3][BLOCK / 64];
  float cov = tid <= cut ? (float)sel.cover[tid] : 0.f;
  float ins = tid <= cut ? (float)sel.hist[tid] : 0.f;
  float tot = (float)sel.hist[tid];
#pragma unroll
  for (int off = 32; off > 0; off >>= 1) { cov += __shfl_xor(cov, off); ins += __shfl_xor(ins, off); tot += __shfl_xor(tot, off); }
  if (lane == 0) { s_dec[0][w] = cov; s_dec[1][w] = ins; s_dec[2][w] = tot; }
  __syncthreads();
  cov = (s_dec[0][0] + s_dec[0][1]) + (s_dec[0][2] + s_dec[0][3]);
  ins = (s_dec[1][0] + s_dec[1][1]) + (s_dec[1][2] + s_dec[1][3]);
  tot = (s_dec[2][0] + s_dec[2][1]) + (s_dec[2][2] + s_dec[2][3]);
  const bool use = cov >= SLICE_MIN_COVER * (float)sel.npix && tot >= SLICE_MIN_RATIO * ins;
  return use ? cut : -1;
}

}
```

rtg_slam_amd/csrc/raster_fwd.hip:

```cpp
#include "raster_common.h"
#include "raster_launch.h"
#include "raster_tilesort.h"
#include <stdlib.h>

namespace rtgs {

constexpr int SAT_LDS = 12288;
__global__ void __launch_bounds__(256) mask_sat_kernel(const int32_t* __restrict__ mask, int gx, int gy,
                                                       int32_t* __restrict__ sat) {
  __shared__ int32_t s_sat[SAT_LDS];
  const int sw = gx + 1, n = (gy + 1) * sw;
  int32_t* const w = n <= SAT_LDS ? s_sat : sat;
  for (int i = threadIdx.x; i < n; i += blockDim.x) {
    int y = i / sw, x = i % sw;
    w[i] = (y == 0 || x == 0) ? 0 : (mask[(y - 1) * gx + (x - 1)] != 0);
  }
  __syncthreads();
  for (int y = 1 + threadIdx.x; y <= gy; y += blockDim.x) {
    int acc = 0;
    for (int x = 1; x <= gx; ++x) { acc += w[y * sw + x]; w[y * sw + x] = acc; }
  }
  __syncthreads();
  for (int x = 1 + threadIdx.x; x <= gx; x += blockDim.x) {
    int acc = 0;
// ... 35 lines not shown
  const float S01 = M00 * M10 + M01 * M11 + M02 * M12;
  const float S02 = M00 * M20 + M01 * M21 + M02 * M22;
  const float S11 = M10 * M10 + M11 * M11 + M12 * M12;
  const float S12 = M10 * M20 + M11 * M21 + M12 * M22;
  const float S22 = M20 * M20 + M21 * M21 + M22 * M22;

  const float limx = 1.3f * p.tanfovx, limy = 1.3f * p.tanfovy;
  const float txtz = pcx / pcz, tytz = pcy / pcz;
  const float tx = fminf(limx, fmaxf(-limx, txtz)) * pcz;
  const float ty = fminf(limy, fmaxf(-limy, tytz)) * pcz;
  const float iz = 1.f / pcz;
  const float J00 = p.fx * iz, J02 = -p.fx * tx * iz * iz;
  const float J11 = p.fy * iz, J12 = -p.fy * ty * iz * iz;
  const float T00 = J00 * V[0] + J02 * V[2], T01 = J00 * V[4] + J02 * V[6], T02 = J00 * V[8] + J02 * V[10];
  const float T10 = J11 * V[1] + J12 * V[2], T11 = J11 * V[5] + J12 * V[6], T12 = J11 * V[9] + J12 * V[10];
  const float a0 = S00 * T00 + S01 * T01 + S02 * T02;
  const float a1 = S01 * T00 + S11 * T01 + S12 * T02;
  const float a2 = S02 * T00 + S12 * T01 + S22 * T02;
  const float b0 = S00 * T10 + S01 * T11 + S02 * T12;
  const float b1 = S01 * T10 + S11 * T11 + S12 * T12;
  const float b2 = S02 * T10 + S12 * T11 + S22 * T12;
  const float ca = T00 * a0 + T01 * a1 + T02 * a2 + 0.3f;
  const float cb = T00 * b0 + T01 * b1 + T02 * b2;
  const float cc = T10 * b0 + T11 * b1 + T12 * b2 + 0.3f;
  const float det = ca * cc - cb * cb;
  if (det == 0.f) return false;
  const float idet = 1.f / det;
  const float mid = 0.5f * (ca + cc);
  const float lam = mid + sqrtf(fmaxf(0.1f, mid * mid - det));
  const int radius = (int)ceilf(p.color_sigma * sqrtf(lam));
  const float u = p.fx * pcx / pcz + p.cx;
  const float v = p.fy * pcy / pcz + p.cy;
  int touched = 0;
  if constexpr (RECT) {
    int x0, y0, x1, y1;
    tile_rect_of(u, v, radius, p.gx, p.gy, x0, y0, x1, y1);
    if ((x1 - x0) * (y1 - y0) == 0) return false;
    const int sw = p.gx + 1;
    touched = sat ? sat[y1 * sw + x1] - sat[y0 * sw + x1] - sat[y1 * sw + x0] + sat[y0 * sw + x0]
                  : (x1 - x0) * (y1 - y0);
  }
  o.mx = mx; o.my = my; o.mz = mz; o.pcx = pcx; o.pcy = pcy; o.pcz = pcz;
  o.ca = ca; o.cb = cb; o.cc = cc; o.idet = idet; o.u = u; o.v = v; o.radius = radius; o.touched = touched;
  return true;
}
__device__ __forceinline__ void cull_store(const CullGeom& g, int i, uint32_t* __restrict__ tiles_touched,
                                           int32_t* __restrict__ radii, int32_t* __restrict__ out_radii,
                                           uint8_t* __restrict__ zbin, float2* __restrict__ uv) {
  radii[i] = g.radius;
  if (out_radii) out_radii[i] = g.radius;
  tiles_touched[i] = (uint32_t)g.touched;
  zbin[i] = (uint8_t)slice_bin_of(g.pcz);
  uv[i] = make_float2(g.u, g.v);
}

template <int MODE>
__global__ void __launch_bounds__(256) preprocess_fwd_kernel(
    RasterParams p, const float* __restrict__ means, const float* __restrict__ opac,
    const float* __restrict__ shs, const float* __restrict__ scales, const float* __restrict__ rots,
    const float* __restrict__ normal_w, const int32_t* __restrict__ sat,
    Splat* __restrict__ splats, uint32_t* __restrict__ tiles_touched, int32_t* __restrict__ radii,
    uint8_t* __restrict__ clamped, int32_t* __restrict__ out_radii, uint32_t* __restrict__ zero_words, int zero_n,
    uint8_t* __restrict__ zbin, float2* __restrict__ uv, SliceList list, SliceSel sel,
    uint32_t* __restrict__ zero2, int zero2_n, RowBands rb) {
#pragma clang fp contract(off)
  int i = blockIdx.x * blockDim.x + threadIdx.x;
  if constexpr (MODE != 2) {
    for (int t = i; t < zero_n; t += gridDim.x * blockDim.x) zero_words[t] = 0u;
    for (int t = i; t < zero2_n; t += gridDim.x * blockDim.x) zero2[t] = 0u;
    if (i >= p.P) return;
    tiles_touched[i] = 0;
    radii[i] = 0;
    if (out_radii) out_radii[i] = 0;
    if (zbin) zbin[i] = 255;
  } else {
    if (spec_failed(p.spec_fail)) return;
    if (list.ids) {
      const int n_list = (int)*list.count;
      if (rb.count) {
        if ((int)(blockIdx.x * blockDim.x) >= n_list) return;
        __shared__ uint32_t s_rows[GATHER_ROWS_MAX], s_rbase[GATHER_ROWS_MAX];
        for (int y = threadIdx.x; y < GATHER_ROWS_MAX; y += blockDim.x) s_rows[y] = 0u;
        __syncthreads();
        int x0 = 0, y0 = 0, x1 = 0, y1 = 0;
        if (i < n_list) {
          const int id = (int)list.ids[i];
          const int rad = radii[id];
          if (rad > 0 && opac[id] >= 1.f / 255.f) {
            const float2 c = uv[id];
            tile_rect_of(c.x, c.y, rad, p.gx, p.gy, x0, y0, x1, y1);
            if ((x1 - x0) * (y1 - y0) <= 0) y1 = y0;
          }
        }
        for (int y = y0; y < y1; ++y) atomicAdd(&s_rows[y], 1u);
        __syncthreads();
        for (int y = threadIdx.x; y < p.gy; y += blockDim.x) {
          const uint32_t c = s_rows[y];
          s_rbase[y] = c ? atomicAdd(&rb.count[y], c) : 0u;
          s_rows[y] = 0u;
        }
        __syncthreads();
        const uint32_t word = (uint32_t)x0 | ((uint32_t)x1 << 8) | ((uint32_t)i << 16);
        for (int y = y0; y < y1; ++y) {
          const uint32_t slot = s_rbase[y] + atomicAdd(&s_rows[y], 1u);
          if (slot < rb.stride) rb.entries[(size_t)y * rb.stride + slot] = word;
        }
      }
      if (i >= n_list) return;
      i = (int)list.ids[i];
    } else {
      if (sel.ctr && sel.ctr[0] == 0u) return;
      const int cut = slice_cut(sel);
      if (i >= p.P) return;
      const int zb = (int)sel.zbin[i];
      if (zb == 255 || zb <= cut) return;
      if (sel.sat) {
        const float2 c = uv[i];
        int x0, y0, x1, y1;
        tile_rect_of(c.x, c.y, radii[i], p.gx, p.gy, x0, y0, x1, y1);
        if (sat_count(sel.sat, p.gx, x0, y0, x1, y1) == 0) return;
      }
    }
  }

  CullGeom cg;
  if (!cull_geom<MODE != 2>(p, means, scales, rots, sat, i, cg)) return;
  const float* V = p.view;
  const float mx = cg.mx, my = cg.my, mz = cg.mz, pcx = cg.pcx, pcy = cg.pcy, pcz = cg.pcz;
  const float ca = cg.ca, cb = cg.cb, cc = cg.cc, idet = cg.idet;
  float u = cg.u, v = cg.v;
  int radius = cg.radius;
  const int touched = cg.touched;
  if constexpr (MODE == 2) {
    const float2 t = uv[i];
    u = t.x; v = t.y; radius = radii[i];
  }
  if constexpr (MODE == 1) {
    cull_store(cg, i, tiles_touched, radii, out_radii, zbin, uv);
    return;
  }

  float dxw = mx - p.campos[0], dyw = my - p.campos[1], dzw = mz - p.campos[2];
  const float il = 1.f / sqrtf(dxw * dxw + dyw * dyw + dzw * dzw);
  dxw *= il; dyw *= il; dzw *= il;
  float shv[48];
  if (p.M == 16) {
    const float4* sh4 = reinterpret_cast<const float4*>(shs + (size_t)i * 48);
#pragma unroll
    for (int q = 0; q < 12; ++q) {
      const float4 t = sh4[q];
      shv[4 * q] = t.x; shv[4 * q + 1] = t.y; shv[4 * q + 2] = t.z; shv[4 * q + 3] = t.w;
    }
  } else {
    const float* shp = shs + (size_t)i * p.M * 3;
#pragma unroll
    for (int q = 0; q < 48; ++q) shv[q] = (q < p.M * 3) ? shp[q] : 0.f;
  }
  const float* sh = shv;
  float col[3];
#pragma unroll
  for (int c = 0; c < 3; ++c) {
    float r = RTGS_SH_C0 * sh[c];
    if (p.deg > 0) {
      r = r - RTGS_SH_C1 * dyw * sh[3 + c] + RTGS_SH_C1 * dzw * sh[6 + c] - RTGS_SH_C1 * dxw * sh[9 + c];
      if (p.deg > 1) {
        const float xx = dxw * dxw, yy = dyw * dyw, zz = dzw * dzw, xy = dxw * dyw, yz = dyw * dzw, xz = dxw * dzw;
        r = r + RTGS_SH_C2_0 * xy * sh[12 + c] + RTGS_SH_C2_1 * yz * sh[15 + c] +
            RTGS_SH_C2_2 * (2.f * zz - xx - yy) * sh[18 + c] + RTGS_SH_C2_3 * xz * sh[21 + c] +
            RTGS_SH_C2_4 * (xx - yy) * sh[24 + c];
        if (p.deg > 2) {
          r = r + RTGS_SH_C3_0 * dyw * (3.f * xx - yy) * sh[27 + c] + RTGS_SH_C3_1 * xy * dzw * sh[30 + c] +
              RTGS_SH_C3_2 * dyw * (4.f * zz - xx - yy) * sh[33 + c] +
              RTGS_SH_C3_3 * dzw * (2.f * zz - 3.f * xx - 3.f * yy) * sh[36 + c] +
              RTGS_SH_C3_4 * dxw * (4.f * zz - xx - yy) * sh[39 + c] + RTGS_SH_C3_5 * dzw * (xx - yy) * sh[42 + c] +
              RTGS_SH_C3_6 * dxw * (xx - 3.f * yy) * sh[45 + c];
        }
      }
    }
    col[c] = r + 0.5f;
  }
  uint8_t cl = 0;
#pragma unroll
  for (int c = 0; c < 3; ++c) {
    if (col[c] < 0.f) { cl |= (uint8_t)(1u << c); col[c] = 0.f; }
  }

  const float nwx = normal_w[3 * i], nwy = normal_w[3 * i + 1], nwz = normal_w[3 * i + 2];
  const float ncx = V[0] * nwx + V[4] * nwy + V[8] * nwz;
  const float ncy = V[1] * nwx + V[5] * nwy + V[9] * nwz;
  const float ncz = V[2] * nwx + V[6] * nwy + V[10] * nwz;

  Splat s;
  s.u = u; s.v = v;
  s.ca = cc * idet; s.cb = -cb * idet; s.cc = ca * idet;
  s.o = opac[i];
  s.r = col[0]; s.g = col[1]; s.b = col[2];
  s.nx = ncx; s.ny = ncy; s.nz = ncz;
  s.pd = ncx * pcx + ncy * pcy + ncz * pcz;
  s.z = pcz;
  {
    const float thr = 2.f * __logf(255.f * fmaxf(opac[i], 1e-12f));
    const float m = fmaxf(thr, 0.f) * 1.01f;
    s.hx = sqrtf(m * ca) + 0.5f;
    s.hy = sqrtf(m * cc) + 0.5f;
  }
  float4* dst = reinterpret_cast<float4*>(splats + i);
  const float4* src = reinterpret_cast<const float4*>(&s);
  dst[0] = src[0]; dst[1] = src[1]; dst[2] = src[2]; dst[3] = src[3];
  clamped[i] = cl;
  if constexpr (MODE == 0) {
    radii[i] = radius;
    if (out_radii) out_radii[i] = radius;
    tiles_touched[i] = (uint32_t)touched;
    if (zbin) zbin[i] = (uint8_t)slice_bin_of(pcz);
  }
}

__global__ void __launch_bounds__(256) emit_keys_kernel(
    RasterParams p, const Splat* __restrict__ splats, const int32_t* __restrict__ radii,
    const uint32_t* __restrict__ offsets, const int32_t* __restrict__ mask,
    uint64_t* __restrict__ keys, uint32_t* __restrict__ vals) {
  const int i = blockIdx.x * blockDim.x + threadIdx.x;
  if (i >= p.P) return;
  const int radius = radii[i];
  if (radius <= 0) return;
  uint32_t off = (i == 0) ? 0u : offsets[i - 1];
  const uint32_t end = offsets[i];
  if (off == end) return;
  const float u = splats[i].u, v = splats[i].v;
  const uint32_t zbits = __float_as_uint(splats[i].z);
  int x0, y0, x1, y1;
  tile_rect_of(u, v, radius, p.gx, p.gy, x0, y0, x1, y1);
  for (int y = y0; y < y1; ++y)
    for (int x = x0; x < x1; ++x) {
      const int t = y * p.gx + x;
      if (mask[t] != 0) {
        keys[off] = ((uint64_t)(uint32_t)t << 32) | zbits;
        vals[off] = (uint32_t)i;
        ++off;
      }
    }
}

__global__ void __launch_bounds__(256) tile_ranges_kernel(int64_t R, const uint64_t* __restrict__ keys,
                                                          uint2* __restrict__ ranges) {
  const int64_t i = (int64_t)blockIdx.x * blockDim.x + threadIdx.x;
  if (i >= R) return;
  const uint32_t t = (uint32_t)(keys[i] >> 32);
  if (i == 0) ranges[t].x = 0;
  else {
    const uint32_t tp = (uint32_t)(keys[i - 1] >> 32);
    if (tp != t) { ranges[tp].y = (uint32_t)i; ranges[t].x = (uint32_t)i; }
  }
  if (i == R - 1) ranges[t].y = (uint32_t)R;
}

constexpr int FWD_BATCH = BLOCK;
constexpr int FWD_CHUNKS = FWD_BATCH / 32;

typedef float f4v __attribute__((ext_vector_type(4)));
typedef float f2v __attribute__((ext_vector_type(2)));

template <bool STAMP, bool COUNT, bool ASMW, bool FSORT, bool GATHER>
__device__ __forceinline__ void blend_fwd_body(
    RasterParams p, const uint2* __restrict__ ranges, const uint32_t* __restrict__ point_list,
    const Splat* __restrict__ splats, float* __restrict__ out_color, float* __restrict__ out_depth,
    int32_t* __restrict__ out_cidx, int32_t* __restrict__ out_didx, float* __restrict__ out_cw,
// ... 466 lines not shown
__global__ void __launch_bounds__(256, OCC) blend_fwd_gather_kernel(
    RasterParams p, const uint2* __restrict__ ranges, const uint32_t* __restrict__ point_list,
    const Splat* __restrict__ splats, float* __restrict__ out_color, float* __restrict__ out_depth,
    int32_t* __restrict__ out_cidx, int32_t* __restrict__ out_didx, float* __restrict__ out_cw,
    float* __restrict__ out_dw, float* __restrict__ out_T, uint32_t* __restrict__ n_contrib,
    unsigned long long* __restrict__ counters, SlicePass sp, uint32_t* __restrict__ tile_mode,
    uint32_t* __restrict__ depth_pos, uint32_t* __restrict__ tile_last, int walk, uint32_t* __restrict__ aux_zero,
    TileCache tc, unsigned long long* __restrict__ stamps, uint32_t seg, FusedSort fs, TileGather tg) {
  blend_fwd_body<false, COUNT, true, true, true>(
      p, ranges, point_list, splats, out_color, out_depth, out_cidx, out_didx, out_cw, out_dw, out_T, n_contrib, counters, sp, tile_mode,
      depth_pos, tile_last, walk, aux_zero, tc, stamps, seg, fs, tg);
}


static int g_f1_occ = [] { const char* e = getenv("RTGS_F1_OCC"); const int v = e ? atoi(e) : 6; return v == 5 ? 5 : 6; }();
static int g_f1_asm = [] { const char* e = getenv("RTGS_F1_ASM"); return e ? atoi(e) : 1; }();
static unsigned long long* g_fwd_stamps = nullptr;
void set_fwd_stamps(void* dev) { g_fwd_stamps = (unsigned long long*)dev; }

void launch_mask_sat(const int32_t* mask, int gx, int gy, int32_t* sat, hipStream_t st) {
  hipLaunchKernelGGL(mask_sat_kernel, dim3(1), dim3(256), 0, st, mask, gx, gy, sat);
}
void launch_preprocess_fwd(const RasterParams& p, const float* means, const float* opac, const float* shs,
                           const float* scales, const float* rots, const float* normal_w, const int32_t* sat,
                           Splat* splats, uint32_t* tiles_touched, int32_t* radii, uint8_t* clamped,
                           int32_t* out_radii, uint32_t* zero_words, int zero_n, uint8_t* zbin, hipStream_t st) {
  if (p.P == 0) return;
  hipLaunchKernelGGL(preprocess_fwd_kernel<0>, dim3((p.P + 255) / 256), dim3(256), 0, st, p, means, opac, shs, scales,
                     rots, normal_w, sat, splats, tiles_touched, radii, clamped, out_radii, zero_words, zero_n, zbin,
                     (float2*)nullptr, SliceList{nullptr, nullptr}, SliceSel{0, nullptr, nullptr, 0u, 0u, nullptr, nullptr, nullptr},
                     (uint32_t*)nullptr, 0, RowBands{nullptr, nullptr, 0u});
}
void launch_preprocess_cull(const RasterParams& p, const float* means, const float* scales, const float* rots,
                            uint32_t* tiles_touched, int32_t* radii, int32_t* out_radii, uint32_t* zero_words, int zero_n,
                            uint8_t* zbin, float2* uv, uint32_t* hist_words, hipStream_t st) {
  if (p.P == 0) return;
  hipLaunchKernelGGL(preprocess_fwd_kernel<1>, dim3((p.P + 255) / 256), dim3(256), 0, st, p, means, (const float*)nullptr,
                     (const float*)nullptr, scales, rots, (const float*)nullptr, (const int32_t*)nullptr, (Splat*)nullptr,
                     tiles_touched, radii, (uint8_t*)nullptr, out_radii, zero_words, zero_n, zbin, uv,
                     SliceList{nullptr, nullptr}, SliceSel{0, nullptr, nullptr, 0u, 0u, nullptr, nullptr, nullptr},
                     hist_words, hist_words ? CULL_HIST_WORDS : 0, RowBands{nullptr, nullptr, 0u});
}
void launch_preprocess_shade(const RasterParams& p, const float* means, const float* opac, const float* shs,
                             const float* scales, const float* rots, const float* normal_w, Splat* splats,
                             int32_t* radii, uint8_t* clamped, float2* uv, SliceList list, SliceSel sel, size_t max_items,
                             hipStream_t st, RowBands rb) {
  if (p.P == 0) return;
  const size_t n = list.ids ? (max_items < (size_t)p.P ? max_items : (size_t)p.P) : (size_t)p.P;
  hipLaunchKernelGGL(preprocess_fwd_kernel<2>, dim3((unsigned)((n + 255) / 256)), dim3(256), 0, st, p, means, opac, shs,
                     scales, rots, normal_w, (const int32_t*)nullptr, splats, (uint32_t*)nullptr, radii, clamped,
                     (int32_t*)nullptr, (uint32_t*)nullptr, 0, (uint8_t*)nullptr, uv, list, sel, (uint32_t*)nullptr, 0,
                     list.ids ? rb : RowBands{nullptr, nullptr, 0u});
}
constexpr int RECULL_ROWS = 1024;
struct RecullArgs {
  RasterParams p;
  const float *means, *scales, *rots;
  uint32_t* tiles_touched; int32_t* radii; int32_t* out_radii; uint8_t* zbin; float2* uv;
  uint32_t* hist; unsigned long long* cover;
  uint8_t* marks;
  const float* view_copy;
  uint32_t* zero_words; int zero_n;
  int fail_idx;
  BwdInfoInit bi;
};
__global__ void __launch_bounds__(256) recull_rows_kernel(RecullArgs a) {
  __shared__ uint32_t s_h[SLICE_BINS], s_c[SLICE_BINS], s_r[SLICE_BINS];
  __shared__ uint16_t s_list[RECULL_ROWS];
  __shared__ uint32_t s_n;
  const int tid = threadIdx.x;
  const bool differs = tid < 16 && __float_as_uint(a.p.view[tid]) != __float_as_uint(a.view_copy[tid]);
  s_h[tid] = 0; s_c[tid] = 0; s_r[tid] = 0;
  if (tid == 0) s_n = 0;
  const uint32_t moved = __syncthreads_or(differs ? 1 : 0) ? 1u : 0u;
  if (a.bi.dst && blockIdx.x == 0 && tid == 0) {
    a.bi.dst->slot_grads = a.bi.slot_grads; a.bi.dst->slots = a.bi.slots; a.bi.dst->use_slots = a.bi.use_slots;
  }
  {
    const int nv = a.zero_n >> 2, stride = (int)gridDim.x * 256;
    uint4* z4 = reinterpret_cast<uint4*>(a.zero_words);
    for (int t = (int)blockIdx.x * 256 + tid; t < nv; t += stride) {
      uint4 w = make_uint4(0u, 0u, 0u, 0u);
      const int d = a.fail_idx - 4 * t;
      if (d >= -1 && d < 4) {
        if (d == 0 || d == -1) w.x = moved;
        if (d == 1 || d == 0) w.y = moved;
        if (d == 2 || d == 1) w.z = moved;
        if (d == 3 || d == 2) w.w = moved;
      }
      z4[t] = w;
    }
    for (int t = 4 * nv + (int)blockIdx.x * 256 + tid; t < a.zero_n; t += stride)
      a.zero_words[t] = (t == a.fail_idx || t == a.fail_idx + 1) ? moved : 0u;
  }
  if (moved) return;
  const int P = a.p.P;
  const int row0 = (int)blockIdx.x * RECULL_ROWS + tid * 4;
  if (row0 < P) {
    uint32_t* m4 = reinterpret_cast<uint32_t*>(a.marks + row0);
    const uint32_t m = *m4;
    if (m != 0u) {
      uint32_t bits = 0;
#pragma unroll
      for (int k = 0; k < 4; ++k) bits |= (((m >> (8 * k)) & 0xffu) != 0u ? 1u : 0u) << k;
      uint32_t at = atomicAdd(&s_n, (uint32_t)__popc(bits));
      while (bits) {
// ... 44 lines not shown
}

struct CullCheckArgs {
  int P;
  const uint32_t *tt_a, *tt_b; const int32_t *rad_a, *rad_b, *orad_a, *orad_b; const uint8_t *zb_a, *zb_b;
  const uint2 *uv_a, *uv_b; const uint32_t *hist_a, *hist_b;
  const uint32_t* skip;
  unsigned long long* mismatches;
};
__global__ void __launch_bounds__(256) cull_check_kernel(CullCheckArgs a) {
  if (*a.skip != 0u) return;
  uint32_t bad = 0;
  const int stride = (int)gridDim.x * 256;
  for (int i = (int)blockIdx.x * 256 + (int)threadIdx.x; i < a.P; i += stride) {
    bad += a.tt_a[i] != a.tt_b[i]; bad += a.rad_a[i] != a.rad_b[i]; bad += a.zb_a[i] != a.zb_b[i];
    if (a.orad_a) bad += a.orad_a[i] != a.orad_b[i];
    const uint2 x = a.uv_a[i], y = a.uv_b[i];
    bad += x.x != y.x; bad += x.y != y.y;
  }
  if (blockIdx.x == 0)
    for (int t = (int)threadIdx.x; t < CULL_HIST_WORDS; t += 256) bad += a.hist_a[t] != a.hist_b[t];
#pragma unroll
  for (int off = 32; off > 0; off >>= 1) bad += (uint32_t)__shfl_xor((int)bad, off);
  if ((threadIdx.x & 63) == 0 && bad) atomicAdd(a.mismatches, (unsigned long long)bad);
}
void launch_cull_check(int P, const uint32_t* tt_a, const uint32_t* tt_b, const int32_t* rad_a, const int32_t* rad_b,
                       const int32_t* orad_a, const int32_t* orad_b, const uint8_t* zb_a, const uint8_t* zb_b,
                       const float2* uv_a, const float2* uv_b, const uint32_t* hist_a, const uint32_t* hist_b,
                       const uint32_t* skip, unsigned long long* mismatches, hipStream_t st) {
  if (P == 0) return;
  int blocks = (P + 255) / 256;
  if (blocks > 1024) blocks = 1024;
  const CullCheckArgs a{P, tt_a, tt_b, rad_a, rad_b, orad_a, orad_b, zb_a, zb_b, (const uint2*)uv_a, (const uint2*)uv_b,
                        hist_a, hist_b, skip, mismatches};
  hipLaunchKernelGGL(cull_check_kernel, dim3(blocks), dim3(256), 0, st, a);
}

void launch_emit_keys(const RasterParams& p, const Splat* splats, const int32_t* radii, const uint32_t* offsets,
                      const int32_t* mask, uint64_t* keys, uint32_t* vals, hipStream_t st) {
  if (p.P == 0) return;
  hipLaunchKernelGGL(emit_keys_kernel, dim3((p.P + 255) / 256), dim3(256), 0, st, p, splats, radii, offsets, mask,
                     keys, vals);
}
void launch_tile_ranges(int64_t R, const uint64_t* keys, uint2* ranges, hipStream_t st) {
  if (R == 0) return;
  hipLaunchKernelGGL(tile_ranges_kernel, dim3((unsigned)((R + 255) / 256)), dim3(256), 0, st, R, keys, ranges);
}
__global__ void __launch_bounds__(256) slice_publish_kernel(int ntiles, const int32_t* __restrict__ user_mask,
                                                            const int32_t* __restrict__ mask2,
                                                            const uint32_t* __restrict__ r1, uint32_t* __restrict__ ctr,
                                                            uint32_t* __restrict__ host, uint32_t seq,
                                                            uint32_t* __restrict__ spec_fail,
                                                            const uint32_t* __restrict__ seg_count) {
  int left = 0, fin = 0, inst = 0, lmax = 0;
  constexpr int PUB_IT = 16;
  if (ntiles <= 256 * PUB_IT) {
    int32_t um[PUB_IT], m2[PUB_IT];
    uint32_t sc[PUB_IT];
    const uint32_t* const sc_src = seg_count ? seg_count : reinterpret_cast<const uint32_t*>(mask2);
#pragma unroll
    for (int j = 0; j < PUB_IT; ++j) {
      const int t = max(min((int)threadIdx.x + 256 * j, ntiles - 1), 0);
      um[j] = user_mask[t];
      m2[j] = mask2[t];
      sc[j] = sc_src[t];
    }
#pragma unroll
    for (int j = 0; j < PUB_IT; ++j) {
      const bool in = (int)threadIdx.x + 256 * j < ntiles;
      const bool on = in && um[j] != 0, l = in && m2[j] != 0;
      left += l ? 1 : 0;
      fin += (on && !l) ? 1 : 0;
      inst += (in && seg_count) ? (int)sc[j] : 0;
      lmax = max(lmax, (in && seg_count) ? (int)sc[j] : 0);
    }
  } else {
    for (int t = threadIdx.x; t < ntiles; t += 256) {
      const bool on = user_mask[t] != 0, l = mask2[t] != 0;
      left += l ? 1 : 0;
      fin += (on && !l) ? 1 : 0;
      if (seg_count) { inst += (int)seg_count[t]; lmax = max(lmax, (int)seg_count[t]); }
    }
  }
  __shared__ int s_l[4], s_f[4], s_i[4], s_m[4];
#pragma unroll
  for (int off = 32; off > 0; off >>= 1) {
    left += __shfl_xor(left, off); fin += __shfl_xor(fin, off); inst += __shfl_xor(inst, off); lmax = max(lmax, __shfl_xor(lmax, off));
  }
  if ((threadIdx.x & 63) == 0) { s_l[threadIdx.x >> 6] = left; s_f[threadIdx.x >> 6] = fin; s_i[threadIdx.x >> 6] = inst; s_m[threadIdx.x >> 6] = lmax; }
  __syncthreads();
  if (threadIdx.x == 0) {
    const uint32_t L = (uint32_t)(s_l[0] + s_l[1] + s_l[2] + s_l[3]), F = (uint32_t)(s_f[0] + s_f[1] + s_f[2] + s_f[3]);
    ctr[0] = L; ctr[1] = F;
    if (spec_fail) *spec_fail = (L != 0u || *spec_fail != 0u) ? 1u : 0u;
    const uint32_t R1 = seg_count ? (uint32_t)(s_i[0] + s_i[1] + s_i[2] + s_i[3]) : r1[0];
    const uint32_t LM = (uint32_t)max(max(s_m[0], s_m[1]), max(s_m[2], s_m[3]));
    const uint32_t w[7] = {ctr[2], LM, L, F, R1, ctr[7], 0u};
    publish_to_host(host, w, seq);
  }
}
void launch_slice_publish(int ntiles, const int32_t* user_mask, const int32_t* mask2, const uint32_t* r1, uint32_t* ctr,
                          uint32_t* host, uint32_t seq, uint32_t* spec_fail, hipStream_t st, const uint32_t* seg_count) {
  hipLaunchKernelGGL(slice_publish_kernel, dim3(1), dim3(256), 0, st, ntiles, user_mask, mask2, r1, ctr, host, seq, spec_fail,
                     seg_count);
}

void launch_blend_fwd(const RasterParams& p, const uint2* ranges, const uint32_t* point_list, const Splat* splats,
                      float* out_color, float* out_depth, int32_t* out_cidx, int32_t* out_didx, float* out_cw,
                      float* out_dw, float* out_T, uint32_t* n_contrib, unsigned long long* counters,
                      SlicePass sp, uint32_t* tile_mode, uint32_t* depth_pos, uint32_t* tile_last, int walk, uint32_t* aux_zero,
                      TileCache tc, uint32_t seg, hipStream_t st, FusedSort fs, TileGather tg) {
#define RTGS_FWD1F(OCC, STAMP, COUNT, ASMW, FS) hipLaunchKernelGGL((blend_fwd_kernel<OCC, STAMP, COUNT, ASMW, FS>), dim3(p.gx, p.gy), dim3(BLOCK), 0, st, p, ranges, point_list, splats, \
                       out_color, out_depth, out_cidx, out_didx, out_cw, out_dw, out_T, n_contrib, counters, sp, tile_mode, \
                       depth_pos, tile_last, walk, aux_zero, tc, g_fwd_stamps, seg, fs)
#define RTGS_FWD1G(OCC, COUNT) hipLaunchKernelGGL((blend_fwd_gather_kernel<OCC, COUNT>), dim3(p.gx, p.gy), dim3(BLOCK), 0, st, p, ranges, point_list, splats, \
                       out_color, out_depth, out_cidx, out_didx, out_cw, out_dw, out_T, n_contrib, counters, sp, tile_mode, \
                       depth_pos, tile_last, walk, aux_zero, tc, g_fwd_stamps, seg, fs, tg)
#define RTGS_FWD1(OCC, STAMP, COUNT, ASMW) do { if (fs.bucket && tg.band_count && !STAMP) RTGS_FWD1G(OCC, COUNT); \
    else if (fs.bucket) RTGS_FWD1F(OCC, STAMP, COUNT, ASMW, true); else RTGS_FWD1F(OCC, STAMP, COUNT, ASMW, false); } while (0)
  if (fs.bucket && (g_f1_asm == 0 || sp.mode != 1)) abort();
  if (tg.band_count && (!(fs.bucket && fs.count && seg != 0u) || g_fwd_stamps)) abort();
  if (g_f1_asm == 0) RTGS_FWD1F(6, false, true, false, false);
  else if (counters) RTGS_FWD1(6, false, true, true);
  else if (g_fwd_stamps) RTGS_FWD1(6, true, false, true);
  else if (g_f1_occ == 5) RTGS_FWD1(5, false, false, true); else RTGS_FWD1(6, false, false, true);
#undef RTGS_FWD1
#undef RTGS_FWD1F
#undef RTGS_FWD1G
}
bool blend_fwd_fuses_sort() { return g_f1_asm != 0; }
bool blend_fwd_gathers() { return g_f1_asm != 0 && g_fwd_stamps == nullptr; }

}
```

rtg_slam_amd/csrc/raster_launch.h:

```cpp
#pragma once
#include "raster_common.h"

namespace rtgs {

void set_fwd_stamps(void* dev);
void launch_mask_sat(const int32_t* mask, int gx, int gy, int32_t* sat, hipStream_t st);
void launch_preprocess_fwd(const RasterParams& p, const float* means, const float* opac, const float* shs, const float* scales,
                           const float* rots, const float* normal_w, const int32_t* sat, Splat* splats, uint32_t* tiles_touched,
                           int32_t* radii, uint8_t* clamped, int32_t* out_radii, uint32_t* zero_words, int zero_n, uint8_t* zbin,
                           hipStream_t st);
void launch_preprocess_cull(const RasterParams& p, const float* means, const float* scales, const float* rots,
                            uint32_t* tiles_touched, int32_t* radii, int32_t* out_radii, uint32_t* zero_words, int zero_n,
                            uint8_t* zbin, float2* uv, uint32_t* hist_words, hipStream_t st);
void launch_preprocess_shade(const RasterParams& p, const float* means, const float* opac, const float* shs, const float* scales,
                             const float* rots, const float* normal_w, Splat* splats, int32_t* radii, uint8_t* clamped, float2* uv,
                             SliceList list, SliceSel sel, size_t max_items, hipStream_t st,
                             RowBands rb = RowBands{nullptr, nullptr, 0u});
void launch_recull_rows(const RasterParams& p, const float* means, const float* scales, const float* rots, uint32_t* tiles_touched,
                        int32_t* radii, int32_t* out_radii, uint32_t* zero_words, int zero_n, uint8_t* zbin, float2* uv,
                        uint32_t* hist, unsigned long long* cover, uint8_t* marks, const float* view_copy, int fail_idx,
                        BwdInfoInit bi, hipStream_t st);
void launch_cull_check(int P, const uint32_t* tt_a, const uint32_t* tt_b, const int32_t* rad_a, const int32_t* rad_b,
                       const int32_t* orad_a, const int32_t* orad_b, const uint8_t* zb_a, const uint8_t* zb_b, const float2* uv_a,
                       const float2* uv_b, const uint32_t* hist_a, const uint32_t* hist_b, const uint32_t* skip,
                       unsigned long long* mismatches, hipStream_t st);
void launch_emit_keys(const RasterParams& p, const Splat* splats, const int32_t* radii, const uint32_t* offsets,
                      const int32_t* mask, uint64_t* keys, uint32_t* vals, hipStream_t st);
void launch_tile_ranges(int64_t R, const uint64_t* keys, uint2* ranges, hipStream_t st);
void launch_slice_publish(int ntiles, const int32_t* user_mask, const int32_t* mask2, const uint32_t* r1, uint32_t* ctr,
                          uint32_t* host, uint32_t seq, uint32_t* spec_fail, hipStream_t st, const uint32_t* seg_count = nullptr);
void launch_blend_fwd(const RasterParams& p, const uint2* ranges, const uint32_t* point_list, const Splat* splats, float* out_color,
                      float* out_depth, int32_t* out_cidx, int32_t* out_didx, float* out_cw, float* out_dw, float* out_T,
                      uint32_t* n_contrib, unsigned long long* counters, SlicePass sp, uint32_t* tile_mode, uint32_t* depth_pos,
                      uint32_t* tile_last, int walk, uint32_t* aux_zero, TileCache tc, uint32_t seg, hipStream_t st,
                      FusedSort fs = FusedSort{nullptr, nullptr, nullptr, nullptr, nullptr},
                      TileGather tg = TileGather{nullptr, nullptr, 0u, nullptr, nullptr, nullptr});
bool blend_fwd_fuses_sort();
bool blend_fwd_gathers();

void launch_blend_bwd(const RasterParams& p, const uint2* ranges, const uint32_t* point_list, const Splat* splats,
                      const float* out_color, const float* final_T, const uint32_t* n_contrib, const int32_t* depth_index,
                      const float* dL_dcolor, const float* dL_ddepth, const uint32_t* gbase, uint32_t* slot_count,
                      const BwdInfo* info, SplatGrad* grads, uint8_t* touched, const uint32_t* tile_mode, int which, uint32_t t0,
                      uint32_t tn, hipStream_t st);
void launch_grad_reduce(int P, const uint8_t* touched, const uint32_t* gbase, uint32_t* count, const BwdInfo* info,
                        SplatGrad* grads, const uint32_t* spec_fail, hipStream_t st);
void launch_preprocess_bwd(const RasterParams& p, const float* means, const float* opac, const float* shs, const float* scales,
                           const float* rots, const float* normal_w, const int32_t* radii, const uint8_t* clamped,
                           SplatGrad* grads, uint8_t* touched, uint8_t* row_state, float* d_means, float* d_opac, float* d_shs,
                           float* d_scales, float* d_rots, float* d_normal, hipStream_t st);

void set_bwd_debug(int bits);
void set_bwd_stamps(void* dev);
void launch_blend_bwd_entry(const RasterParams& p, const uint2* ranges, const uint32_t* point_list, const Splat* splats,
                            const float* out_color, const uint32_t* n_contrib, const int32_t* depth_index,
                            const uint32_t* depth_pos, const uint32_t* tile_last, const float* dL_dcolor, const float* dL_ddepth,
                            const uint32_t* gbase, uint32_t* slot_count, const BwdInfo* info, SplatGrad* grads, uint8_t* touched,
                            const uint32_t* tile_mode, uint32_t t0, uint32_t tn, TileCache tc, uint32_t pre, hipStream_t st,
                            const LossSigns* signs = nullptr);

size_t bin_lds_limit_tiles();
int bin_sort_capacity();
size_t bin_block_counts_bytes(int P, int ntiles);
size_t bin_slice_block_counts_bytes(int P, size_t max_list, int ntiles);
size_t bin_list_block_counts_bytes(int P, int ntiles);
void launch_slice_hist(int P, const uint8_t* zbin, const uint32_t* rect_area, const int32_t* radii, uint32_t* hist,
                       unsigned long long* cover, hipStream_t st, BwdInfoInit bi = BwdInfoInit{nullptr, nullptr, 0u, 0u});
void launch_slice_compact(int P, SliceSel sel, uint32_t* ids, uint32_t* n_list, const uint32_t* rect_area, uint32_t* gbase,
                          uint32_t* slot_cursor, uint32_t* host, uint32_t seq, uint32_t* fail_if_taken, hipStream_t st);
void launch_visible_compact(int P, const uint8_t* zbin, uint32_t* ids, uint32_t* n_list, const uint32_t* rect_area,
// ... 21 lines not shown
```

rtg_slam_amd/rasterizer.py:

```python
from __future__ import annotations

import ctypes as C
import threading
from typing import NamedTuple, Optional

import torch
import torch.nn as nn

from . import _lib


class GaussianRasterizationSettings(NamedTuple):
    image_height: int
    image_width: int
    tanfovx: float
    tanfovy: float
    bg: torch.Tensor
    scale_modifier: float
    viewmatrix: torch.Tensor
    projmatrix: torch.Tensor
    sh_degree: int
    campos: torch.Tensor
    opaque_threshold: float
    depth_threshold: float
# ... 10 lines not shown

    def __init__(self, handle=None, owned=False):
        self.handle = handle
        self._owned = owned

    @classmethod
    def create(cls) -> "RasterContext":
        h = _lib.load().rtgs_ctx_create()
        if not h:
            raise RuntimeError("rtgs_ctx_create failed")
        return cls(h, owned=True)

    def __del__(self):
        try:
            if self._owned and self.handle:
                _lib.load().rtgs_ctx_destroy(C.c_void_p(self.handle))
                self.handle = None
        except Exception:
            pass

    @property
    def ptr(self):
        return C.c_void_p(self.handle)

    def set_near_slice(self, mode: int, budget_per_tile: int = 0):
        _lib.load().rtgs_raster_set_near_slice_ctx(self.ptr, int(mode), int(budget_per_tile))

    def force_sort_path(self, enable: bool):
        _lib.load().rtgs_raster_force_sort_path_ctx(self.ptr, int(bool(enable)))

    def set_bwd_walk(self, mode: int):
        _lib.load().rtgs_raster_set_bwd_walk_ctx(self.ptr, int(mode))

    def set_onepass(self, enable: bool):
        _lib.load().rtgs_raster_set_onepass_ctx(self.ptr, int(bool(enable)))

    def set_fused_sort(self, enable: bool):
        _lib.load().rtgs_raster_set_fused_sort_ctx(self.ptr, int(bool(enable)))

    def fused_sort_stats(self):
        out = (C.c_int64 * 18)()
        _lib.check(_lib.load().rtgs_raster_fused_sort_stats_ctx(self.ptr, out), "rtgs_raster_fused_sort_stats")
        names = ("empty", "single", "bitonic", "radix", "launch", "pass2")
        return {n: dict(tiles=int(out[3 * k]), shortest=int(out[3 * k + 1]), longest=int(out[3 * k + 2])) for k, n in enumerate(names)}

    def set_tile_gather(self, mode: int):
        _lib.load().rtgs_raster_set_tile_gather_ctx(self.ptr, int(mode))

    def tile_gather_stats(self):
        out = (C.c_int64 * 6)()
        _lib.check(_lib.load().rtgs_raster_tile_gather_stats_ctx(self.ptr, out), "rtgs_raster_tile_gather_stats")
        return dict(gathered=int(out[0]), fell_back_listed=int(out[1]), fell_back_longest=int(out[2]), fell_back_layout=int(out[3]),
                    chunk=int(out[4]), capacity=int(out[5]))

    def set_loss_signs(self, enable: bool):
        _lib.load().rtgs_raster_set_loss_signs_ctx(self.ptr, int(bool(enable)))

    def loss_signs_stats(self):
        out = (C.c_int64 * 2)()
        _lib.check(_lib.load().rtgs_raster_loss_signs_stats_ctx(self.ptr, out), "rtgs_raster_loss_signs_stats")
        return dict(signs=int(out[0]), floats=int(out[1]))

    def set_speculation(self, enable: bool):
        _lib.load().rtgs_raster_set_speculation_ctx(self.ptr, int(bool(enable)))

    def speculation_stats(self):
        out = (C.c_int64 * 3)()
        _lib.check(_lib.load().rtgs_raster_speculation_stats_ctx(self.ptr, out), "rtgs_raster_speculation_stats")
        return dict(speculative=int(out[0]), failed=int(out[1]), not_eligible=int(out[2]))

    def set_cull_cache(self, enable: bool):
        _lib.load().rtgs_raster_set_cull_cache_ctx(self.ptr, int(bool(enable)))

    def set_cull_cache_check(self, enable: bool):
        _lib.load().rtgs_raster_set_cull_cache_check_ctx(self.ptr, int(bool(enable)))

    def cull_cache_stats(self):
        out = (C.c_int64 * 5)()
        _lib.check(_lib.load().rtgs_raster_cull_cache_stats_ctx(self.ptr, out), "rtgs_raster_cull_cache_stats")
        return dict(hits=int(out[0]), full=int(out[1]), disarmed=int(out[2]), view_redos=int(out[3]), check_mismatches=int(out[4]))

    def set_plain_onepass(self, enable: bool):
        _lib.load().rtgs_raster_set_plain_onepass_ctx(self.ptr, int(bool(enable)))

    def plain_stats(self):
        out = (C.c_int64 * 2)()
        _lib.check(_lib.load().rtgs_raster_plain_stats_ctx(self.ptr, out), "rtgs_raster_plain_stats")
        return dict(onepass=int(out[0]), redone=int(out[1]))

    def set_profiling(self, enable: bool):
        _lib.load().rtgs_raster_set_profiling_ctx(self.ptr, int(bool(enable)))

    def set_counters(self, counters: Optional[torch.Tensor]):
        _lib.load().rtgs_raster_set_counters_ctx(self.ptr, C.c_void_p(counters.data_ptr() if counters is not None else 0))

    def last_stats(self):
        out = (C.c_int64 * 8)()
        _lib.check(_lib.load().rtgs_raster_last_stats_ctx(self.ptr, out), "rtgs_raster_last_stats")
        return [int(v) for v in out]

    def last_slice_stats(self):
        out = (C.c_int64 * 4)()
        _lib.check(_lib.load().rtgs_raster_last_slice_stats_ctx(self.ptr, out), "rtgs_raster_last_slice_stats")
        return dict(used=int(out[0]), instances=int(out[1]), tiles_finished=int(out[2]), tiles_left_to_pass2=int(out[3]))

    def last_timings(self):
# ... 270 lines not shown
```

Baseline: 3109 units/s.

## Fuse slice compact with shading and fold slice publish into loss kernel

```diff
diff --git a/include/rtgs_debug.h b/include/rtgs_debug.h
--- a/include/rtgs_debug.h
+++ b/include/rtgs_debug.h
@@ -25,6 +25,10 @@
 int rtgs_raster_fused_sort_stats_ctx(rtgs_ctx* ctx, int64_t* out18);
 void rtgs_raster_set_tile_gather_ctx(rtgs_ctx* ctx, int mode);
 int rtgs_raster_tile_gather_stats_ctx(rtgs_ctx* ctx, int64_t* out6);
+void rtgs_raster_set_slice_shade_ctx(rtgs_ctx* ctx, int on);
+int rtgs_raster_slice_shade_stats_ctx(rtgs_ctx* ctx, int64_t* out3);
+void rtgs_raster_set_loss_publish_ctx(rtgs_ctx* ctx, int on);
+int rtgs_raster_loss_publish_stats_ctx(rtgs_ctx* ctx, int64_t* out3);
 void rtgs_raster_set_bwd_debug(int bits);
 void rtgs_raster_set_bwd_stamps(void* dev);
 void rtgs_raster_set_fwd_stamps(void* dev);
diff --git a/rtg_slam_amd/csrc/map_ops.hip b/rtg_slam_amd/csrc/map_ops.hip
--- a/rtg_slam_amd/csrc/map_ops.hip
+++ b/rtg_slam_amd/csrc/map_ops.hip
@@ -4,6 +4,7 @@
 #include <stdint.h>
 #include "adam_common.h"
 #include "activate_common.h"
+#include "raster_publish.h"
 
 
 namespace rtgs {
@@ -571,14 +572,22 @@
 
 __device__ __forceinline__ uint32_t sign_code(float d) { return d > 0.f ? 1u : (d < 0.f ? 2u : 0u); }
 
-template <int V>
+template <int V, bool JOB>
 __global__ void __launch_bounds__(256) slam_loss_sums_signs_kernel(const float* __restrict__ color, const float* __restrict__ depth,
                                                                    const int32_t* __restrict__ didx, const float* __restrict__ gt_c,
                                                                    const float* __restrict__ gt_d, const uint8_t* __restrict__ rmask,
                                                                    int64_t hw, float depth_thr,
-                                                                   float* __restrict__ sums, uint8_t* __restrict__ signs) {
+                                                                   float* __restrict__ sums, uint8_t* __restrict__ signs,
+                                                                   PublishJob job) {
+  const unsigned img_blocks = gridDim.x - (JOB ? 1u : 0u);
+  if constexpr (JOB) {
+    if (blockIdx.x >= img_blocks) {
+      slice_publish_body(job.ntiles, job.user_mask, job.mask2, job.r1, job.ctr, job.host, job.seq, job.spec_fail, job.seg_count);
+      return;
+    }
+  }
   float s_c = 0.f, s_d = 0.f, s_m = 0.f, s_n = 0.f;
-  for (int64_t i = ((int64_t)blockIdx.x * blockDim.x + threadIdx.x) * V; i < hw; i += (int64_t)gridDim.x * blockDim.x * V) {
+  for (int64_t i = ((int64_t)blockIdx.x * blockDim.x + threadIdx.x) * V; i < hw; i += (int64_t)img_blocks * blockDim.x * V) {
     bool m[V], hit[V];
     load_flags<V>(rmask, didx, i, m, hit);
     PixVec<V> c0, c1, c2, t0, t1, t2, dp, gd;
@@ -818,6 +827,13 @@
 extern "C" int rtgs_slam_loss_sums_signs(const float* color, const float* depth, const int32_t* depth_index,
                                          const float* gt_color, const float* gt_depth, int32_t H, int32_t W,
                                          const rtgs_loss_cfg* cfg, void* scratch, float* loss_out4, void* stream) {
+  return rtgs::loss_sums_signs_publish(color, depth, depth_index, gt_color, gt_depth, H, W, cfg, scratch, loss_out4,
+                                       rtgs::PublishJob{0, nullptr, nullptr, nullptr, nullptr, nullptr, 0u, nullptr, nullptr}, nullptr, stream);
+}
+int rtgs::loss_sums_signs_publish(const float* color, const float* depth, const int32_t* depth_index, const float* gt_color,
+                                  const float* gt_depth, int32_t H, int32_t W, const rtgs_loss_cfg* cfg, void* scratch,
+                                  float* loss_out4, const PublishJob& job, bool* job_launched, void* stream) {
+  if (job_launched) *job_launched = false;
   if (!color || !depth || !depth_index || !gt_color || !gt_depth || !cfg || !scratch || H <= 0 || W <= 0) return -1;
   if (cfg->render_mask == nullptr && cfg->ssim_weight != 0.f) return -1;
   hipStream_t st = (hipStream_t)stream;
@@ -827,13 +843,16 @@
   if (!cfg->sums_zeroed && hipMemsetAsync(sums, 0, 8 * sizeof(float), st) != hipSuccess) return -2;
   int64_t blocks = (hw + 255) / 256;
   if (blocks > 192) blocks = 192;
-  if (rtgs::loss_vec4_ok(hw, color, depth, depth_index, gt_color, gt_depth, cfg->render_mask, nullptr, nullptr) &&
-      ((uintptr_t)signs & 3u) == 0)
-    hipLaunchKernelGGL(rtgs::slam_loss_sums_signs_kernel<4>, dim3((unsigned)blocks), dim3(256), 0, st, color, depth, depth_index,
-                       gt_color, gt_depth, cfg->render_mask, hw, cfg->add_depth_thres, sums, signs);
-  else
-    hipLaunchKernelGGL(rtgs::slam_loss_sums_signs_kernel<1>, dim3((unsigned)blocks), dim3(256), 0, st, color, depth, depth_index,
-                       gt_color, gt_depth, cfg->render_mask, hw, cfg->add_depth_thres, sums, signs);
+  const bool with_job = job.ntiles != 0;
+  const dim3 grid((unsigned)blocks + (with_job ? 1u : 0u));
+  const bool vec4 = rtgs::loss_vec4_ok(hw, color, depth, depth_index, gt_color, gt_depth, cfg->render_mask, nullptr, nullptr) &&
+                    ((uintptr_t)signs & 3u) == 0;
+#define RTGS_LOSS_SIGNS(V, JOB) hipLaunchKernelGGL((rtgs::slam_loss_sums_signs_kernel<V, JOB>), grid, dim3(256), 0, st, color, depth, \
+                       depth_index, gt_color, gt_depth, cfg->render_mask, hw, cfg->add_depth_thres, sums, signs, job)
+  if (vec4) { if (with_job) RTGS_LOSS_SIGNS(4, true); else RTGS_LOSS_SIGNS(4, false); }
+  else { if (with_job) RTGS_LOSS_SIGNS(1, true); else RTGS_LOSS_SIGNS(1, false); }
+#undef RTGS_LOSS_SIGNS
+  if (job_launched) *job_launched = with_job;
   if (loss_out4) return rtgs_slam_loss_values(cfg, scratch, loss_out4, stream);
   return hipGetLastError() == hipSuccess ? 0 : -2;
 }
diff --git a/rtg_slam_amd/csrc/map_step.hip b/rtg_slam_amd/csrc/map_step.hip
--- a/rtg_slam_amd/csrc/map_step.hip
+++ b/rtg_slam_amd/csrc/map_step.hip
@@ -1,6 +1,7 @@
 #include <hip/hip_runtime.h>
 
 #include "../../include/rtgs_raster.h"
+#include "raster_publish.h"
 
 static int map_step_front(rtgs_ctx* ctx, const rtgs_map_step_args* a, int64_t* num_rendered_host, int32_t fwd_flags,
                           void* stream, bool walk_only = false) {
@@ -16,6 +17,7 @@
   }
   if (!a->loss_scratch || !a->loss4) return RTGS_E_INVALID;
   rtgs_raster_set_aux_zero_ctx(ctx, a->loss_scratch);
+  if (fwd_flags & RTGS_FWD_SPECULATE) rtgs::publish_defer_request(ctx);
   rc = rtgs_raster_forward_ctx(ctx, a->settings, P, M, a->xyz, a->opacity, a->shs, a->scales, a->rotations, a->normal,
                            a->tile_mask, a->out_color, a->out_depth, a->out_color_index, a->out_depth_index,
                            a->out_color_weight, a->out_depth_weight, a->out_T, a->out_radii, a->geom_resize,
@@ -30,15 +32,24 @@
   const bool ssim_off = a->loss.render_mask != nullptr || a->loss.ssim_weight == 0.f;
   const bool signs = walk_only && ssim_off && rtgs_raster_signs_ok_ctx(ctx, geom) != 0;
   rtgs_raster_note_loss_path_ctx(ctx, signs ? 1 : 0);
-  if (signs)
-    rc = rtgs_slam_loss_sums_signs(a->out_color, a->out_depth, a->out_depth_index, a->gt_color, a->gt_depth, H, W, &lcfg,
-                                   a->loss_scratch, nullptr, stream);
-  else
+  int32_t t0 = 0, t1 = P;
+  if (a->train_begin != 0 || a->train_end != 0) { t0 = a->train_begin; t1 = a->train_end; }
+  rtgs::PublishJob job{0, nullptr, nullptr, nullptr, nullptr, nullptr, 0u, nullptr, nullptr};
+  const bool carry = signs && t0 >= 0 && t1 <= P && t1 > t0 && rtgs::publish_take(ctx, &job);
+  if (!carry && rtgs::publish_discharge(ctx) != RTGS_OK) return RTGS_E_HIP;
+  if (signs) {
+    bool launched = false;
+    rc = rtgs::loss_sums_signs_publish(a->out_color, a->out_depth, a->out_depth_index, a->gt_color, a->gt_depth, H, W, &lcfg,
+                                       a->loss_scratch, nullptr, job, &launched, stream);
+    if (carry && launched) rtgs::publish_note_in_loss(ctx);
+    else if (carry) {
+      rtgs::publish_put_back(ctx, job);
+      if (rtgs::publish_discharge(ctx) != RTGS_OK) return RTGS_E_HIP;
+    }
+  } else
     rc = rtgs_slam_loss(a->out_color, a->out_depth, a->out_depth_index, a->gt_color, a->gt_depth, H, W, &lcfg,
                         a->loss_scratch, a->loss4, a->dL_dcolor, a->dL_ddepth, stream);
   if (rc != 0) return RTGS_E_HIP;
-  int32_t t0 = 0, t1 = P;
-  if (a->train_begin != 0 || a->train_end != 0) { t0 = a->train_begin; t1 = a->train_end; }
   if (t0 < 0 || t1 > P || t1 < t0) return RTGS_E_INVALID;
   if (t1 == t0)
     return signs && rtgs_slam_loss_values(&lcfg, a->loss_scratch, a->loss4, stream) != 0 ? RTGS_E_HIP : RTGS_OK;
diff --git a/rtg_slam_amd/csrc/raster_api.hip b/rtg_slam_amd/csrc/raster_api.hip
--- a/rtg_slam_amd/csrc/raster_api.hip
+++ b/rtg_slam_amd/csrc/raster_api.hip
@@ -2,6 +2,7 @@
 #include "../../include/rtgs_debug.h"
 #include "raster_common.h"
 #include "raster_launch.h"
+#include "raster_publish.h"
 #include <vector>
 
 #include <rocprim/device/device_radix_sort.hpp>
@@ -26,7 +27,16 @@
     bool cull_cache = true, cull_check = false;
     bool loss_signs = true;
     int tile_gather = 1;
+    bool slice_shade = true;
+    bool loss_publish = true;
   } sw;
+  bool publish_defer = false;
+  bool publish_pending = false;
+  rtgs::PublishJob publish_job = {};
+  hipStream_t publish_stream = nullptr;
+  int64_t loss_publish_stats[2] = {0, 0};
+  int64_t host_wait_fallbacks = 0;
+  int64_t slice_shade_stats[2] = {0, 0};
   int64_t gather_stats[4] = {0, 0, 0, 0};
   bool gather_blocked = false;
   int64_t loss_path_stats[2] = {0, 0};
@@ -113,11 +123,37 @@
     if (const char* e = getenv("RTGS_CULL_CACHE_CHECK")) n->sw.cull_check = atoi(e) != 0;
     if (const char* e = getenv("RTGS_LOSS_SIGNS")) n->sw.loss_signs = atoi(e) != 0;
     if (const char* e = getenv("RTGS_TILE_GATHER")) { const int m = atoi(e); n->sw.tile_gather = (m >= 0 && m <= 2) ? m : 1; }
+    if (const char* e = getenv("RTGS_SLICE_SHADE")) n->sw.slice_shade = atoi(e) != 0;
+    if (const char* e = getenv("RTGS_LOSS_PUBLISH")) n->sw.loss_publish = atoi(e) != 0;
     return n;
   }();
   return c;
 }
 static inline rtgs_ctx* use(rtgs_ctx* c) { return c ? c : default_ctx(); }
+
+void publish_defer_request(rtgs_ctx* ctx) { use(ctx)->publish_defer = true; }
+bool publish_take(rtgs_ctx* ctx, PublishJob* out) {
+  rtgs_ctx* const c = use(ctx);
+  if (!c->publish_pending || !out) return false;
+  *out = c->publish_job;
+  c->publish_pending = false;
+  return true;
+}
+void publish_put_back(rtgs_ctx* ctx, const PublishJob& job) {
+  rtgs_ctx* const c = use(ctx);
+  c->publish_job = job; c->publish_pending = true;
+}
+int publish_discharge(rtgs_ctx* ctx) {
+  rtgs_ctx* const c = use(ctx);
+  if (!c->publish_pending) return RTGS_OK;
+  c->publish_pending = false;
+  const PublishJob& j = c->publish_job;
+  if (!c->spec.pending || c->spec.seq != j.seq) return RTGS_OK;
+  launch_slice_publish(j.ntiles, j.user_mask, j.mask2, j.r1, j.ctr, j.host, j.seq, j.spec_fail, c->publish_stream, j.seg_count);
+  ++c->loss_publish_stats[1];
+  return hipGetLastError() == hipSuccess ? RTGS_OK : RTGS_E_HIP;
+}
+void publish_note_in_loss(rtgs_ctx* ctx) { ++use(ctx)->loss_publish_stats[0]; }
 
 static void prof_mark(rtgs_ctx* c, int which, hipStream_t st) {
   if (!c->prof) return;
@@ -135,7 +171,7 @@
   return b < 1 ? 1 : b;
 }
 
-static int wait_published_words(uint32_t* info_host, uint32_t seq, hipStream_t st, uint32_t (&pub)[7]) {
+static int wait_published_words(uint32_t* info_host, uint32_t seq, hipStream_t st, uint32_t (&pub)[7], int64_t* fallbacks = nullptr) {
   volatile uint32_t* h = info_host;
   auto snapshot_ok = [&]() -> bool {
     if (h[7] != seq) return false;
@@ -150,6 +186,7 @@
     if (snapshot_ok()) return RTGS_OK;
     __builtin_ia32_pause();
   }
+  if (fallbacks) ++*fallbacks;
   if (hipStreamSynchronize(st) != hipSuccess) return RTGS_E_HIP;
   return snapshot_ok() ? RTGS_OK : RTGS_E_HIP;
 }
@@ -327,6 +364,7 @@
   int fwd_walk;
   TileCache tcache;
   uint32_t seg1;
+  bool publish_defer = false;
   uint32_t* aux_zero;
   uint64_t cull_epoch;
   bool cull_was_armed;
@@ -335,7 +373,7 @@
 };
 
 static inline void next_seq(rtgs_ctx* c) { if (++c->seq == 0u) c->seq = 1u; }
-static inline int wait_published(FwdCall& f) { return wait_published_words(f.info_host, f.c->seq, f.st, f.pub); }
+static inline int wait_published(FwdCall& f) { return wait_published_words(f.info_host, f.c->seq, f.st, f.pub, &f.c->host_wait_fallbacks); }
 
 static void record_stats(rtgs_ctx* c, int64_t rendered, int ntiles, int64_t geom_bytes, int64_t bin_bytes, int64_t img_bytes,
                          bool tile_path, int64_t longest) {
@@ -431,14 +469,24 @@
   return RTGS_OK;
 }
 
-static int slice_pass1(FwdCall& f, uint32_t* guard, bool gather = false) {
+static void publish_slice(FwdCall& f, uint32_t* guard, const uint32_t* seg_count, bool defer) {
+  rtgs_ctx* const c = f.c;
+  if (!defer) {
+    launch_slice_publish(f.ntiles, f.tile_mask, f.mask2, f.info + 2, f.slice_ctr, f.info_host, c->seq, guard, f.st, seg_count);
+    return;
+  }
+  c->publish_job = PublishJob{f.ntiles, f.tile_mask, f.mask2, f.info + 2, f.slice_ctr, f.info_host, c->seq, guard, seg_count};
+  c->publish_stream = f.st;
+  c->publish_pending = true;
+}
+static int slice_pass1(FwdCall& f, uint32_t* guard, bool gather = false, bool shaded = false, bool defer = false) {
   const RasterParams& p = f.p; const GeomLayout& G = f.G;
   const SliceSel sel1 = slice_sel(f);
   const SliceList work{(const uint32_t*)(f.geom + G.slice_ids), f.slice_ctr + 2};
   unsigned long long* const bucket1 = (unsigned long long*)(f.geom + G.bucket1);
   if (gather) {
     const RowBands rb{f.tile_count, (uint32_t*)bucket1, (uint32_t)G.slice_max_list};
-    shade(f, p, work, sel1, G.slice_max_list, rb);
+    if (!shaded) shade(f, p, work, sel1, G.slice_max_list, rb);
     uint32_t* cls = nullptr;
     const int rcc = fsort_class_words(f, cls);
     if (rcc != RTGS_OK) return rcc;
@@ -448,11 +496,11 @@
           FusedSort{bucket1, f.tile_count1, f.ranges1, f.list1, cls},
           TileGather{rb.count, rb.entries, rb.stride, work.ids, f.radii, f.tile_count1});
     prof_mark(f.c, EV_SL_BLEND, f.st);
-    launch_slice_publish(f.ntiles, f.tile_mask, f.mask2, f.info + 2, f.slice_ctr, f.info_host, f.c->seq, guard, f.st, f.tile_count1);
+    publish_slice(f, guard, f.tile_count1, defer);
     DBG(f.s, f.st);
     return RTGS_OK;
   }
-  shade(f, p, work, sel1, G.slice_max_list);
+  if (!shaded) shade(f, p, work, sel1, G.slice_max_list);
   if (f.seg1) {
     launch_bin_place(p, f.splats, f.radii, f.tile_mask, f.tile_count1, bucket1, f.seg1, nullptr, sel1, work, G.slice_max_list, f.st);
   } else {
@@ -471,8 +519,7 @@
   prof_mark(f.c, EV_SL_BIN, f.st);
   blend(f, p, f.ranges1, f.list1, SlicePass{1, f.tile_mask, f.mask2, f.ranges1_bwd, f.ranges}, f.seg1, fs1);
   prof_mark(f.c, EV_SL_BLEND, f.st);
-  launch_slice_publish(f.ntiles, f.tile_mask, f.mask2, f.info + 2, f.slice_ctr, f.info_host, f.c->seq, guard, f.st,
-                       f.seg1 ? f.tile_count1 : nullptr);
+  publish_slice(f, guard, f.seg1 ? f.tile_count1 : nullptr, defer);
   DBG(f.s, f.st);
   return RTGS_OK;
 }
@@ -616,10 +663,20 @@
   if (pl.kind == 1) {
     if ((rc = cull_stage(f, pl.kind, !immediate, fail, BwdInfoInit{bwd_info, slot_grads, sl, sl ? 1u : 0u})) != RTGS_OK) return rc;
     prof_mark(c, EV_PRE, st);
-    launch_slice_compact(P, slice_sel(f), (uint32_t*)(f.geom + G.slice_ids), f.slice_ctr + 2, f.tiles_touched, f.offsets,
-                         f.slice_ctr + 4, nullptr, 0u, nullptr, st);
     c->spec.gathered = tile_gather_chosen(f, pl);
-    if ((rc = slice_pass1(f, fail, c->spec.gathered)) != RTGS_OK) return rc;
+    const bool fused = c->sw.slice_shade;
+    ++c->slice_shade_stats[fused ? 0 : 1];
+    if (fused) {
+      const RowBands rb = c->spec.gathered ? RowBands{f.tile_count, (uint32_t*)(f.geom + G.bucket1), (uint32_t)G.slice_max_list}
+                                           : RowBands{nullptr, nullptr, 0u};
+      launch_slice_shade(p, f.means3D, f.opacities, f.shs, f.scales, f.rotations, f.normal_w, f.splats, f.radii, f.clamped, f.uv,
+                         slice_sel(f), (uint32_t*)(f.geom + G.slice_ids), f.slice_ctr + 2, f.tiles_touched, f.offsets,
+                         f.slice_ctr + 4, rb, st);
+    } else {
+      launch_slice_compact(P, slice_sel(f), (uint32_t*)(f.geom + G.slice_ids), f.slice_ctr + 2, f.tiles_touched, f.offsets,
+                           f.slice_ctr + 4, nullptr, 0u, nullptr, st);
+    }
+    if ((rc = slice_pass1(f, fail, c->spec.gathered, fused, f.publish_defer && !immediate)) != RTGS_OK) return rc;
     prof_mark(c, EV_BLEND0, st); prof_mark(c, EV_BLEND, st);
     c->hint_slice_lists = true; c->hint_main_lists = false;
     c->slice_stats[0] = 1; c->slice_stats[1] = pl.R1; c->slice_stats[2] = pl.n_fin; c->slice_stats[3] = 0;
@@ -926,6 +983,8 @@
   FwdCall f;
   f.c = c;
   f.aux_zero = c->aux_zero; c->aux_zero = nullptr;
+  f.publish_defer = c->publish_defer && c->sw.loss_publish; c->publish_defer = false;
+  if (!c->spec.pending) c->publish_pending = false;
   f.cull_epoch = c->cull.next_epoch; c->cull.next_epoch = 0;
   f.cull_was_armed = c->cull.armed; c->cull.armed = false;
   if (f.cull_was_armed) ++c->cull.stats[2];
@@ -967,6 +1026,7 @@
   int rc = make_params(s, P, M, p);
   if (rc != RTGS_OK) return rc;
   if (P == 0) return RTGS_OK;
+  if (publish_discharge(c) != RTGS_OK) return RTGS_E_HIP;
   if (c->spec.geom == geom_buffer && c->spec.fail_dev) p.spec_fail = c->spec.fail_dev;
   if (!means3D || !opacities || !shs || !scales || !rotations || !normal_w || !geom_buffer || !binning_buffer ||
       !image_buffer || !out_color || !out_T || !out_didx || (!lsg && (!dL_dcolor || !dL_ddepth)) || !grad_scratch || R < 0)
@@ -1124,10 +1184,11 @@
 void rtgs_raster_force_sort_path_ctx(rtgs_ctx* c, int enable) { use(c)->force_sort_path = enable != 0; }
 int rtgs_raster_forward_verify_ctx(rtgs_ctx* ctx, int64_t* num_rendered_host) {
   rtgs_ctx* c = use(ctx);
+  if (publish_discharge(c) != RTGS_OK) { c->spec.pending = false; c->plan.valid = false; return RTGS_E_HIP; }
   if (!c->spec.pending) return 0;
   c->spec.pending = false;
   uint32_t pub[7] = {0, 0, 0, 0, 0, 0, 0};
-  const int rc = wait_published_words(c->info_host, c->spec.seq, (hipStream_t)c->spec.stream, pub);
+  const int rc = wait_published_words(c->info_host, c->spec.seq, (hipStream_t)c->spec.stream, pub, &c->host_wait_fallbacks);
   if (rc != RTGS_OK) { c->plan.valid = false; return rc; }
   rtgs_ctx::Plan& pl = c->plan;
   bool ok;
@@ -1226,6 +1287,18 @@
 void rtgs_raster_set_tile_gather_ctx(rtgs_ctx* c, int mode) {
   use(c)->sw.tile_gather = (mode >= 0 && mode <= 2) ? mode : 1; use(c)->plan.valid = false; use(c)->gather_blocked = false;
 }
+void rtgs_raster_set_loss_publish_ctx(rtgs_ctx* c, int on) { use(c)->sw.loss_publish = on != 0; }
+int rtgs_raster_loss_publish_stats_ctx(rtgs_ctx* ctx, int64_t* out3) {
+  if (!out3) return RTGS_E_INVALID;
+  out3[0] = use(ctx)->loss_publish_stats[0]; out3[1] = use(ctx)->loss_publish_stats[1]; out3[2] = use(ctx)->host_wait_fallbacks;
+  return RTGS_OK;
+}
+void rtgs_raster_set_slice_shade_ctx(rtgs_ctx* c, int on) { use(c)->sw.slice_shade = on != 0; use(c)->plan.valid = false; }
+int rtgs_raster_slice_shade_stats_ctx(rtgs_ctx* ctx, int64_t* out3) {
+  if (!out3) return RTGS_E_INVALID;
+  out3[0] = use(ctx)->slice_shade_stats[0]; out3[1] = use(ctx)->slice_shade_stats[1]; out3[2] = slice_shade_chunk();
+  return RTGS_OK;
+}
 int rtgs_raster_tile_gather_stats_ctx(rtgs_ctx* ctx, int64_t* out6) {
   if (!out6) return RTGS_E_INVALID;
   memcpy(out6, use(ctx)->gather_stats, sizeof(use(ctx)->gather_stats));
diff --git a/rtg_slam_amd/csrc/raster_common.h b/rtg_slam_amd/csrc/raster_common.h
--- a/rtg_slam_amd/csrc/raster_common.h
+++ b/rtg_slam_amd/csrc/raster_common.h
@@ -332,6 +332,69 @@
   __hip_atomic_store(&host[7], seq, __ATOMIC_RELAXED, __HIP_MEMORY_SCOPE_SYSTEM);
 }
 
+struct PublishJob {
+  int ntiles;
+  const int32_t* user_mask;
+  const int32_t* mask2;
+  const uint32_t* r1;
+  uint32_t* ctr;
+  uint32_t* host;
+  uint32_t seq;
+  uint32_t* spec_fail;
+  const uint32_t* seg_count;
+};
+__device__ __forceinline__ void slice_publish_body(int ntiles, const int32_t* __restrict__ user_mask,
+                                                   const int32_t* __restrict__ mask2, const uint32_t* __restrict__ r1,
+                                                   uint32_t* __restrict__ ctr, uint32_t* __restrict__ host, uint32_t seq,
+                                                   uint32_t* __restrict__ spec_fail, const uint32_t* __restrict__ seg_count) {
+  int left = 0, fin = 0, inst = 0, lmax = 0;
+  constexpr int PUB_IT = 16;
+  if (ntiles <= 256 * PUB_IT) {
+    int32_t um[PUB_IT], m2[PUB_IT];
+    uint32_t sc[PUB_IT];
+    const uint32_t* const sc_src = seg_count ? seg_count : reinterpret_cast<const uint32_t*>(mask2);
+#pragma unroll
+    for (int j = 0; j < PUB_IT; ++j) {
+      const int t = max(min((int)threadIdx.x + 256 * j, ntiles - 1), 0);
+      um[j] = user_mask[t];
+      m2[j] = mask2[t];
+      sc[j] = sc_src[t];
+    }
+#pragma unroll
+    for (int j = 0; j < PUB_IT; ++j) {
+      const bool in = (int)threadIdx.x + 256 * j < ntiles;
+      const bool on = in && um[j] != 0, l = in && m2[j] != 0;
+      left += l ? 1 : 0;
+      fin += (on && !l) ? 1 : 0;
+      inst += (in && seg_count) ? (int)sc[j] : 0;
+      lmax = max(lmax, (in && seg_count) ? (int)sc[j] : 0);
+    }
+  } else {
+    for (int t = threadIdx.x; t < ntiles; t += 256) {
+      const bool on = user_mask[t] != 0, l = mask2[t] != 0;
+      left += l ? 1 : 0;
+      fin += (on && !l) ? 1 : 0;
+      if (seg_count) { inst += (int)seg_count[t]; lmax = max(lmax, (int)seg_count[t]); }
+    }
+  }
+  __shared__ int s_l[4], s_f[4], s_i[4], s_m[4];
+#pragma unroll
+  for (int off = 32; off > 0; off >>= 1) {
+    left += __shfl_xor(left, off); fin += __shfl_xor(fin, off); inst += __shfl_xor(inst, off); lmax = max(lmax, __shfl_xor(lmax, off));
+  }
+  if ((threadIdx.x & 63) == 0) { s_l[threadIdx.x >> 6] = left; s_f[threadIdx.x >> 6] = fin; s_i[threadIdx.x >> 6] = inst; s_m[threadIdx.x >> 6] = lmax; }
+  __syncthreads();
+  if (threadIdx.x == 0) {
+    const uint32_t L = (uint32_t)(s_l[0] + s_l[1] + s_l[2] + s_l[3]), F = (uint32_t)(s_f[0] + s_f[1] + s_f[2] + s_f[3]);
+    ctr[0] = L; ctr[1] = F;
+    if (spec_fail) *spec_fail = (L != 0u || *spec_fail != 0u) ? 1u : 0u;
+    const uint32_t R1 = seg_count ? (uint32_t)(s_i[0] + s_i[1] + s_i[2] + s_i[3]) : r1[0];
+    const uint32_t LM = (uint32_t)max(max(s_m[0], s_m[1]), max(s_m[2], s_m[3]));
+    const uint32_t w[7] = {ctr[2], LM, L, F, R1, ctr[7], 0u};
+    publish_to_host(host, w, seq);
+  }
+}
+
 __device__ __forceinline__ int slice_cut(const SliceSel& sel) {
   __shared__ uint32_t s_wsum[2][BLOCK / 64];
   const int tid = threadIdx.x, lane = tid & 63, w = tid >> 6;
diff --git a/rtg_slam_amd/csrc/raster_fwd.hip b/rtg_slam_amd/csrc/raster_fwd.hip
--- a/rtg_slam_amd/csrc/raster_fwd.hip
+++ b/rtg_slam_amd/csrc/raster_fwd.hip
@@ -111,6 +111,108 @@
   tiles_touched[i] = (uint32_t)g.touched;
   zbin[i] = (uint8_t)slice_bin_of(g.pcz);
   uv[i] = make_float2(g.u, g.v);
+}
+
+template <int MODE>
+__device__ __forceinline__ void preprocess_row(
+    const RasterParams& p, const float* __restrict__ means, const float* __restrict__ opac,
+    const float* __restrict__ shs, const float* __restrict__ scales, const float* __restrict__ rots,
+    const float* __restrict__ normal_w, const int32_t* __restrict__ sat,
+    Splat* __restrict__ splats, uint32_t* __restrict__ tiles_touched, int32_t* __restrict__ radii,
+    uint8_t* __restrict__ clamped, int32_t* __restrict__ out_radii, uint8_t* __restrict__ zbin, float2* __restrict__ uv,
+    const int i) {
+#pragma clang fp contract(off)
+  CullGeom cg;
+  if (!cull_geom<MODE != 2>(p, means, scales, rots, sat, i, cg)) return;
+  const float* V = p.view;
+  const float mx = cg.mx, my = cg.my, mz = cg.mz, pcx = cg.pcx, pcy = cg.pcy, pcz = cg.pcz;
+  const float ca = cg.ca, cb = cg.cb, cc = cg.cc, idet = cg.idet;
+  float u = cg.u, v = cg.v;
+  int radius = cg.radius;
+  const int touched = cg.touched;
+  if constexpr (MODE == 2) {
+    const float2 t = uv[i];
+    u = t.x; v = t.y; radius = radii[i];
+  }
+  if constexpr (MODE == 1) {
+    cull_store(cg, i, tiles_touched, radii, out_radii, zbin, uv);
+    return;
+  }
+
+  float dxw = mx - p.campos[0], dyw = my - p.campos[1], dzw = mz - p.campos[2];
+  const float il = 1.f / sqrtf(dxw * dxw + dyw * dyw + dzw * dzw);
+  dxw *= il; dyw *= il; dzw *= il;
+  float shv[48];
+  if (p.M == 16) {
+    const float4* sh4 = reinterpret_cast<const float4*>(shs + (size_t)i * 48);
+#pragma unroll
+    for (int q = 0; q < 12; ++q) {
+      const float4 t = sh4[q];
+      shv[4 * q] = t.x; shv[4 * q + 1] = t.y; shv[4 * q + 2] = t.z; shv[4 * q + 3] = t.w;
+    }
+  } else {
+    const float* shp = shs + (size_t)i * p.M * 3;
+#pragma unroll
+    for (int q = 0; q < 48; ++q) shv[q] = (q < p.M * 3) ? shp[q] : 0.f;
+  }
+  const float* sh = shv;
+  float col[3];
+#pragma unroll
+  for (int c = 0; c < 3; ++c) {
+    float r = RTGS_SH_C0 * sh[c];
+    if (p.deg > 0) {
+      r = r - RTGS_SH_C1 * dyw * sh[3 + c] + RTGS_SH_C1 * dzw * sh[6 + c] - RTGS_SH_C1 * dxw * sh[9 + c];
+      if (p.deg > 1) {
+        const float xx = dxw * dxw, yy = dyw * dyw, zz = dzw * dzw, xy = dxw * dyw, yz = dyw * dzw, xz = dxw * dzw;
+        r = r + RTGS_SH_C2_0 * xy * sh[12 + c] + RTGS_SH_C2_1 * yz * sh[15 + c] +
+            RTGS_SH_C2_2 * (2.f * zz - xx - yy) * sh[18 + c] + RTGS_SH_C2_3 * xz * sh[21 + c] +
+            RTGS_SH_C2_4 * (xx - yy) * sh[24 + c];
+        if (p.deg > 2) {
+          r = r + RTGS_SH_C3_0 * dyw * (3.f * xx - yy) * sh[27 + c] + RTGS_SH_C3_1 * xy * dzw * sh[30 + c] +
+              RTGS_SH_C3_2 * dyw * (4.f * zz - xx - yy) * sh[33 + c] +
+              RTGS_SH_C3_3 * dzw * (2.f * zz - 3.f * xx - 3.f * yy) * sh[36 + c] +
+              RTGS_SH_C3_4 * dxw * (4.f * zz - xx - yy) * sh[39 + c] + RTGS_SH_C3_5 * dzw * (xx - yy) * sh[42 + c] +
+              RTGS_SH_C3_6 * dxw * (xx - 3.f * yy) * sh[45 + c];
+        }
+      }
+    }
+    col[c] = r + 0.5f;
+  }
+  uint8_t cl = 0;
+#pragma unroll
+  for (int c = 0; c < 3; ++c) {
+    if (col[c] < 0.f) { cl |= (uint8_t)(1u << c); col[c] = 0.f; }
+  }
+
+  const float nwx = normal_w[3 * i], nwy = normal_w[3 * i + 1], nwz = normal_w[3 * i + 2];
+  const float ncx = V[0] * nwx + V[4] * nwy + V[8] * nwz;
+  const float ncy = V[1] * nwx + V[5] * nwy + V[9] * nwz;
+  const float ncz = V[2] * nwx + V[6] * nwy + V[10] * nwz;
+
+  Splat s;
+  s.u = u; s.v = v;
+  s.ca = cc * idet; s.cb = -cb * idet; s.cc = ca * idet;
+  s.o = opac[i];
+  s.r = col[0]; s.g = col[1]; s.b = col[2];
+  s.nx = ncx; s.ny = ncy; s.nz = ncz;
+  s.pd = ncx * pcx + ncy * pcy + ncz * pcz;
+  s.z = pcz;
+  {
+    const float thr = 2.f * __logf(255.f * fmaxf(opac[i], 1e-12f));
+    const float m = fmaxf(thr, 0.f) * 1.01f;
+    s.hx = sqrtf(m * ca) + 0.5f;
+    s.hy = sqrtf(m * cc) + 0.5f;
+  }
+  float4* dst = reinterpret_cast<float4*>(splats + i);
+  const float4* src = reinterpret_cast<const float4*>(&s);
+  dst[0] = src[0]; dst[1] = src[1]; dst[2] = src[2]; dst[3] = src[3];
+  clamped[i] = cl;
+  if constexpr (MODE == 0) {
+    radii[i] = radius;
+    if (out_radii) out_radii[i] = radius;
+    tiles_touched[i] = (uint32_t)touched;
+    if (zbin) zbin[i] = (uint8_t)slice_bin_of(pcz);
+  }
 }
 
 template <int MODE>
@@ -182,96 +284,130 @@
     }
   }
 
-  CullGeom cg;
-  if (!cull_geom<MODE != 2>(p, means, scales, rots, sat, i, cg)) return;
-  const float* V = p.view;
-  const float mx = cg.mx, my = cg.my, mz = cg.mz, pcx = cg.pcx, pcy = cg.pcy, pcz = cg.pcz;
-  const float ca = cg.ca, cb = cg.cb, cc = cg.cc, idet = cg.idet;
-  float u = cg.u, v = cg.v;
-  int radius = cg.radius;
-  const int touched = cg.touched;
-  if constexpr (MODE == 2) {
-    const float2 t = uv[i];
-    u = t.x; v = t.y; radius = radii[i];
-  }
-  if constexpr (MODE == 1) {
-    cull_store(cg, i, tiles_touched, radii, out_radii, zbin, uv);
-    return;
-  }
-
-  float dxw = mx - p.campos[0], dyw = my - p.campos[1], dzw = mz - p.campos[2];
-  const float il = 1.f / sqrtf(dxw * dxw + dyw * dyw + dzw * dzw);
-  dxw *= il; dyw *= il; dzw *= il;
-  float shv[48];
-  if (p.M == 16) {
-    const float4* sh4 = reinterpret_cast<const float4*>(shs + (size_t)i * 48);
-#pragma unroll
-    for (int q = 0; q < 12; ++q) {
-      const float4 t = sh4[q];
-      shv[4 * q] = t.x; shv[4 * q + 1] = t.y; shv[4 * q + 2] = t.z; shv[4 * q + 3] = t.w;
-    }
-  } else {
-    const float* shp = shs + (size_t)i * p.M * 3;
-#pragma unroll
-    for (int q = 0; q < 48; ++q) shv[q] = (q < p.M * 3) ? shp[q] : 0.f;
-  }
-  const float* sh = shv;
-  float col[3];
-#pragma unroll
-  for (int c = 0; c < 3; ++c) {
-    float r = RTGS_SH_C0 * sh[c];
-    if (p.deg > 0) {
-      r = r - RTGS_SH_C1 * dyw * sh[3 + c] + RTGS_SH_C1 * dzw * sh[6 + c] - RTGS_SH_C1 * dxw * sh[9 + c];
-      if (p.deg > 1) {
-        const float xx = dxw * dxw, yy = dyw * dyw, zz = dzw * dzw, xy = dxw * dyw, yz = dyw * dzw, xz = dxw * dzw;
-        r = r + RTGS_SH_C2_0 * xy * sh[12 + c] + RTGS_SH_C2_1 * yz * sh[15 + c] +
-            RTGS_SH_C2_2 * (2.f * zz - xx - yy) * sh[18 + c] + RTGS_SH_C2_3 * xz * sh[21 + c] +
-            RTGS_SH_C2_4 * (xx - yy) * sh[24 + c];
-        if (p.deg > 2) {
-          r = r + RTGS_SH_C3_0 * dyw * (3.f * xx - yy) * sh[27 + c] + RTGS_SH_C3_1 * xy * dzw * sh[30 + c] +
-              RTGS_SH_C3_2 * dyw * (4.f * zz - xx - yy) * sh[33 + c] +
-              RTGS_SH_C3_3 * dzw * (2.f * zz - 3.f * xx - 3.f * yy) * sh[36 + c] +
-              RTGS_SH_C3_4 * dxw * (4.f * zz - xx - yy) * sh[39 + c] + RTGS_SH_C3_5 * dzw * (xx - yy) * sh[42 + c] +
-              RTGS_SH_C3_6 * dxw * (xx - 3.f * yy) * sh[45 + c];
+  preprocess_row<MODE>(p, means, opac, shs, scales, rots, normal_w, sat, splats, tiles_touched, radii, clamped, out_radii, zbin, uv,
+                       i);
+}
+
+constexpr int SLICE_SHADE_CHUNK = 8192;
+__global__ void __launch_bounds__(256) slice_shade_kernel(
+    RasterParams p, const float* __restrict__ means, const float* __restrict__ opac,
+    const float* __restrict__ shs, const float* __restrict__ scales, const float* __restrict__ rots,
+    const float* __restrict__ normal_w, Splat* __restrict__ splats, int32_t* __restrict__ radii,
+    uint8_t* __restrict__ clamped, float2* __restrict__ uv, SliceSel sel, uint32_t* __restrict__ ids,
+    uint32_t* __restrict__ n_list, const uint32_t* __restrict__ rect_area, uint32_t* __restrict__ gbase,
+    uint32_t* __restrict__ slot_cursor, RowBands rb) {
+  constexpr int WORDS = SLICE_SHADE_CHUNK / 1024;
+  static_assert(SLICE_SHADE_CHUNK % 1024 == 0 && WORDS * 4 <= 32, "one flag bit per row of a thread; 16-bit row offsets");
+  static_assert(GATHER_ROWS_MAX == 256, "one row counter per thread");
+  __shared__ uint16_t s_loc[SLICE_SHADE_CHUNK];
+  __shared__ uint32_t s_rel[SLICE_SHADE_CHUNK];
+  __shared__ uint32_t s_w[4], s_base, s_gb;
+  __shared__ uint32_t s_rows[GATHER_ROWS_MAX], s_rbase[GATHER_ROWS_MAX];
+  const int tid = threadIdx.x, lane = tid & 63, w = tid >> 6;
+  const int begin = blockIdx.x * SLICE_SHADE_CHUNK;
+  uint32_t zall[WORDS];
+#pragma unroll
+  for (int j = 0; j < WORDS; ++j) {
+    const int i = begin + j * 1024 + tid * 4;
+    const bool whole = i + 4 <= p.P;
+    const uint32_t zb4 = *reinterpret_cast<const uint32_t*>(sel.zbin + (whole ? i : 0));
+    zall[j] = whole ? zb4 : 0xffffffffu;
+  }
+#pragma unroll
+  for (int j = 0; j < WORDS; ++j) {
+    const int i = begin + j * 1024 + tid * 4;
+    if (i < p.P && i + 4 > p.P)
+      for (int k = 0; k < 4; ++k) if (i + k < p.P) zall[j] = (zall[j] & ~(0xffu << (8 * k))) | ((uint32_t)sel.zbin[i + k] << (8 * k));
+  }
+  const int cut = slice_cut(sel);
+  if (blockIdx.x == 0 && tid == 0) reinterpret_cast<int32_t*>(n_list)[1] = cut;
+  uint32_t flags = 0u;
+#pragma unroll
+  for (int j = 0; j < WORDS; ++j)
+#pragma unroll
+    for (int k = 0; k < 4; ++k) {
+      const int zb = (int)((zall[j] >> (8 * k)) & 0xffu);
+      if (zb != 255 && zb <= cut) flags |= 1u << (j * 4 + k);
+    }
+  const uint32_t cnt = (uint32_t)__popc(flags);
+  uint32_t incl = cnt;
+#pragma unroll
+  for (int off = 1; off < 64; off <<= 1) {
+    const uint32_t t = (uint32_t)__shfl_up((int)incl, off);
+    if (lane >= off) incl += t;
+  }
+  if (lane == 63) s_w[w] = incl;
+  __syncthreads();
+  const uint32_t n = (s_w[0] + s_w[1]) + (s_w[2] + s_w[3]);
+  {
+    uint32_t at = incl - cnt;
+    for (int q = 0; q < w; ++q) at += s_w[q];
+    for (uint32_t f = flags; f != 0u; f &= f - 1u) {
+      const int b = __ffs((int)f) - 1;
+      s_loc[at++] = (uint16_t)((b >> 2) * 1024 + tid * 4 + (b & 3));
+    }
+  }
+  __syncthreads();
+  if (n == 0u) return;
+  uint32_t run = 0u;
+  for (uint32_t k0 = 0; k0 < n; k0 += 256) {
+    const uint32_t k = k0 + (uint32_t)tid;
+    const uint32_t a = k < n ? rect_area[begin + (int)s_loc[k]] : 0u;
+    uint32_t ia = a;
+#pragma unroll
+    for (int off = 1; off < 64; off <<= 1) {
+      const uint32_t t = (uint32_t)__shfl_up((int)ia, off);
+      if (lane >= off) ia += t;
+    }
+    if (lane == 63) s_w[w] = ia;
+    __syncthreads();
+    uint32_t pre = run;
+    for (int q = 0; q < w; ++q) pre += s_w[q];
+    if (k < n) s_rel[k] = pre + ia - a;
+    run += (s_w[0] + s_w[1]) + (s_w[2] + s_w[3]);
+    __syncthreads();
+  }
+  if (tid == 0) s_base = atomicAdd(n_list, n);
+  if (tid == 64) s_gb = atomicAdd(slot_cursor, run);
+  __syncthreads();
+  const uint32_t base = s_base, gb = s_gb;
+  const bool go = !spec_failed(p.spec_fail);
+  for (uint32_t k0 = 0; k0 < n; k0 += 256) {
+    const uint32_t k = k0 + (uint32_t)tid;
+    const bool mine = k < n;
+    const int id = mine ? begin + (int)s_loc[k] : 0;
+    const uint32_t pos = base + k;
+    if (mine) { ids[pos] = (uint32_t)id; gbase[id] = gb + s_rel[k]; }
+    if (!go) continue;
+    if (rb.count) {
+      s_rows[tid] = 0u;
+      __syncthreads();
+      int x0 = 0, y0 = 0, x1 = 0, y1 = 0;
+      if (mine) {
+        const int rad = radii[id];
+        if (rad > 0 && opac[id] >= 1.f / 255.f) {
+          const float2 c = uv[id];
+          tile_rect_of(c.x, c.y, rad, p.gx, p.gy, x0, y0, x1, y1);
+          if ((x1 - x0) * (y1 - y0) <= 0) y1 = y0;
         }
       }
-    }
-    col[c] = r + 0.5f;
-  }
-  uint8_t cl = 0;
-#pragma unroll
-  for (int c = 0; c < 3; ++c) {
-    if (col[c] < 0.f) { cl |= (uint8_t)(1u << c); col[c] = 0.f; }
-  }
-
-  const float nwx = normal_w[3 * i], nwy = normal_w[3 * i + 1], nwz = normal_w[3 * i + 2];
-  const float ncx = V[0] * nwx + V[4] * nwy + V[8] * nwz;
-  const float ncy = V[1] * nwx + V[5] * nwy + V[9] * nwz;
-  const float ncz = V[2] * nwx + V[6] * nwy + V[10] * nwz;
-
-  Splat s;
-  s.u = u; s.v = v;
-  s.ca = cc * idet; s.cb = -cb * idet; s.cc = ca * idet;
-  s.o = opac[i];
-  s.r = col[0]; s.g = col[1]; s.b = col[2];
-  s.nx = ncx; s.ny = ncy; s.nz = ncz;
-  s.pd = ncx * pcx + ncy * pcy + ncz * pcz;
-  s.z = pcz;
-  {
-    const float thr = 2.f * __logf(255.f * fmaxf(opac[i], 1e-12f));
-    const float m = fmaxf(thr, 0.f) * 1.01f;
-    s.hx = sqrtf(m * ca) + 0.5f;
-    s.hy = sqrtf(m * cc) + 0.5f;
-  }
-  float4* dst = reinterpret_cast<float4*>(splats + i);
-  const float4* src = reinterpret_cast<const float4*>(&s);
-  dst[0] = src[0]; dst[1] = src[1]; dst[2] = src[2]; dst[3] = src[3];
-  clamped[i] = cl;
-  if constexpr (MODE == 0) {
-    radii[i] = radius;
-    if (out_radii) out_radii[i] = radius;
-    tiles_touched[i] = (uint32_t)touched;
-    if (zbin) zbin[i] = (uint8_t)slice_bin_of(pcz);
+      for (int y = y0; y < y1; ++y) atomicAdd(&s_rows[y], 1u);
+      __syncthreads();
+      for (int y = tid; y < p.gy; y += 256) {
+        const uint32_t c = s_rows[y];
+        s_rbase[y] = c ? atomicAdd(&rb.count[y], c) : 0u;
+        s_rows[y] = 0u;
+      }
+      __syncthreads();
+      const uint32_t word = (uint32_t)x0 | ((uint32_t)x1 << 8) | (pos << 16);
+      for (int y = y0; y < y1; ++y) {
+        const uint32_t slot = s_rbase[y] + atomicAdd(&s_rows[y], 1u);
+        if (slot < rb.stride) rb.entries[(size_t)y * rb.stride + slot] = word;
+      }
+      __syncthreads();
+    }
+    if (mine)
+      preprocess_row<2>(p, means, opac, shs, scales, rots, normal_w, nullptr, splats, nullptr, radii, clamped, nullptr, nullptr, uv, id);
   }
 }
 
@@ -844,6 +980,15 @@
                      (int32_t*)nullptr, (uint32_t*)nullptr, 0, (uint8_t*)nullptr, uv, list, sel, (uint32_t*)nullptr, 0,
                      list.ids ? rb : RowBands{nullptr, nullptr, 0u});
 }
+void launch_slice_shade(const RasterParams& p, const float* means, const float* opac, const float* shs, const float* scales,
+                        const float* rots, const float* normal_w, Splat* splats, int32_t* radii, uint8_t* clamped, float2* uv,
+                        SliceSel sel, uint32_t* ids, uint32_t* n_list, const uint32_t* rect_area, uint32_t* gbase,
+                        uint32_t* slot_cursor, RowBands rb, hipStream_t st) {
+  if (p.P == 0) return;
+  hipLaunchKernelGGL(slice_shade_kernel, dim3((p.P + SLICE_SHADE_CHUNK - 1) / SLICE_SHADE_CHUNK), dim3(256), 0, st, p, means, opac,
+                     shs, scales, rots, normal_w, splats, radii, clamped, uv, sel, ids, n_list, rect_area, gbase, slot_cursor, rb);
+}
+int slice_shade_chunk() { return SLICE_SHADE_CHUNK; }
 constexpr int RECULL_ROWS = 1024;
 struct RecullArgs {
   RasterParams p;
@@ -994,52 +1139,7 @@
                                                             uint32_t* __restrict__ host, uint32_t seq,
                                                             uint32_t* __restrict__ spec_fail,
                                                             const uint32_t* __restrict__ seg_count) {
-  int left = 0, fin = 0, inst = 0, lmax = 0;
-  constexpr int PUB_IT = 16;
-  if (ntiles <= 256 * PUB_IT) {
-    int32_t um[PUB_IT], m2[PUB_IT];
-    uint32_t sc[PUB_IT];
-    const uint32_t* const sc_src = seg_count ? seg_count : reinterpret_cast<const uint32_t*>(mask2);
-#pragma unroll
-    for (int j = 0; j < PUB_IT; ++j) {
-      const int t = max(min((int)threadIdx.x + 256 * j, ntiles - 1), 0);
-      um[j] = user_mask[t];
-      m2[j] = mask2[t];
-      sc[j] = sc_src[t];
-    }
-#pragma unroll
-    for (int j = 0; j < PUB_IT; ++j) {
-      const bool in = (int)threadIdx.x + 256 * j < ntiles;
-      const bool on = in && um[j] != 0, l = in && m2[j] != 0;
-      left += l ? 1 : 0;
-      fin += (on && !l) ? 1 : 0;
-      inst += (in && seg_count) ? (int)sc[j] : 0;
-      lmax = max(lmax, (in && seg_count) ? (int)sc[j] : 0);
-    }
-  } else {
-    for (int t = threadIdx.x; t < ntiles; t += 256) {
-      const bool on = user_mask[t] != 0, l = mask2[t] != 0;
-      left += l ? 1 : 0;
-      fin += (on && !l) ? 1 : 0;
-      if (seg_count) { inst += (int)seg_count[t]; lmax = max(lmax, (int)seg_count[t]); }
-    }
-  }
-  __shared__ int s_l[4], s_f[4], s_i[4], s_m[4];
-#pragma unroll
-  for (int off = 32; off > 0; off >>= 1) {
-    left += __shfl_xor(left, off); fin += __shfl_xor(fin, off); inst += __shfl_xor(inst, off); lmax = max(lmax, __shfl_xor(lmax, off));
-  }
-  if ((threadIdx.x & 63) == 0) { s_l[threadIdx.x >> 6] = left; s_f[threadIdx.x >> 6] = fin; s_i[threadIdx.x >> 6] = inst; s_m[threadIdx.x >> 6] = lmax; }
-  __syncthreads();
-  if (threadIdx.x == 0) {
-    const uint32_t L = (uint32_t)(s_l[0] + s_l[1] + s_l[2] + s_l[3]), F = (uint32_t)(s_f[0] + s_f[1] + s_f[2] + s_f[3]);
-    ctr[0] = L; ctr[1] = F;
-    if (spec_fail) *spec_fail = (L != 0u || *spec_fail != 0u) ? 1u : 0u;
-    const uint32_t R1 = seg_count ? (uint32_t)(s_i[0] + s_i[1] + s_i[2] + s_i[3]) : r1[0];
-    const uint32_t LM = (uint32_t)max(max(s_m[0], s_m[1]), max(s_m[2], s_m[3]));
-    const uint32_t w[7] = {ctr[2], LM, L, F, R1, ctr[7], 0u};
-    publish_to_host(host, w, seq);
-  }
+  slice_publish_body(ntiles, user_mask, mask2, r1, ctr, host, seq, spec_fail, seg_count);
 }
 void launch_slice_publish(int ntiles, const int32_t* user_mask, const int32_t* mask2, const uint32_t* r1, uint32_t* ctr,
                           uint32_t* host, uint32_t seq, uint32_t* spec_fail, hipStream_t st, const uint32_t* seg_count) {
diff --git a/rtg_slam_amd/csrc/raster_launch.h b/rtg_slam_amd/csrc/raster_launch.h
--- a/rtg_slam_amd/csrc/raster_launch.h
+++ b/rtg_slam_amd/csrc/raster_launch.h
@@ -16,6 +16,11 @@
                              const float* rots, const float* normal_w, Splat* splats, int32_t* radii, uint8_t* clamped, float2* uv,
                              SliceList list, SliceSel sel, size_t max_items, hipStream_t st,
                              RowBands rb = RowBands{nullptr, nullptr, 0u});
+void launch_slice_shade(const RasterParams& p, const float* means, const float* opac, const float* shs, const float* scales,
+                        const float* rots, const float* normal_w, Splat* splats, int32_t* radii, uint8_t* clamped, float2* uv,
+                        SliceSel sel, uint32_t* ids, uint32_t* n_list, const uint32_t* rect_area, uint32_t* gbase,
+                        uint32_t* slot_cursor, RowBands rb, hipStream_t st);
+int slice_shade_chunk();
 void launch_recull_rows(const RasterParams& p, const float* means, const float* scales, const float* rots, uint32_t* tiles_touched,
                         int32_t* radii, int32_t* out_radii, uint32_t* zero_words, int zero_n, uint8_t* zbin, float2* uv,
                         uint32_t* hist, unsigned long long* cover, uint8_t* marks, const float* view_copy, int fail_idx,
diff --git a/rtg_slam_amd/csrc/raster_publish.h b/rtg_slam_amd/csrc/raster_publish.h
--- /dev/null
+++ b/rtg_slam_amd/csrc/raster_publish.h
@@ -0,0 +1,19 @@
+#pragma once
+#include <hip/hip_runtime.h>
+#include <stdint.h>
+
+#include "../../include/rtgs_raster.h"
+#include "raster_common.h"
+
+namespace rtgs {
+
+void publish_defer_request(rtgs_ctx* ctx);
+bool publish_take(rtgs_ctx* ctx, PublishJob* out);
+void publish_put_back(rtgs_ctx* ctx, const PublishJob& job);
+int publish_discharge(rtgs_ctx* ctx);
+void publish_note_in_loss(rtgs_ctx* ctx);
+int loss_sums_signs_publish(const float* color, const float* depth, const int32_t* depth_index, const float* gt_color,
+                            const float* gt_depth, int32_t H, int32_t W, const rtgs_loss_cfg* cfg, void* scratch,
+                            float* loss_out4, const PublishJob& job, bool* job_launched, void* stream);
+
+}
diff --git a/rtg_slam_amd/rasterizer.py b/rtg_slam_amd/rasterizer.py
--- a/rtg_slam_amd/rasterizer.py
+++ b/rtg_slam_amd/rasterizer.py
@@ -86,6 +86,22 @@
         _lib.check(_lib.load().rtgs_raster_tile_gather_stats_ctx(self.ptr, out), "rtgs_raster_tile_gather_stats")
         return dict(gathered=int(out[0]), fell_back_listed=int(out[1]), fell_back_longest=int(out[2]), fell_back_layout=int(out[3]),
                     chunk=int(out[4]), capacity=int(out[5]))
+
+    def set_slice_shade(self, enable: bool):
+        _lib.load().rtgs_raster_set_slice_shade_ctx(self.ptr, int(bool(enable)))
+
+    def slice_shade_stats(self):
+        out = (C.c_int64 * 3)()
+        _lib.check(_lib.load().rtgs_raster_slice_shade_stats_ctx(self.ptr, out), "rtgs_raster_slice_shade_stats")
+        return dict(fused=int(out[0]), separate=int(out[1]), chunk=int(out[2]))
+
+    def set_loss_publish(self, enable: bool):
+        _lib.load().rtgs_raster_set_loss_publish_ctx(self.ptr, int(bool(enable)))
+
+    def loss_publish_stats(self):
+        out = (C.c_int64 * 3)()
+        _lib.check(_lib.load().rtgs_raster_loss_publish_stats_ctx(self.ptr, out), "rtgs_raster_loss_publish_stats")
+        return dict(in_loss=int(out[0]), stand_alone=int(out[1]), wait_fallbacks=int(out[2]))
 
     def set_loss_signs(self, enable: bool):
         _lib.load().rtgs_raster_set_loss_signs_ctx(self.ptr, int(bool(enable)))
```

Result: faster. 3158 units/s (median of 6 runs) (+1.6%).
